# vt-asaplab/vPIN

Hardware: AMD Instinct MI355X
Metric: R1CS constraints/sec, whole Spartan SNARK (sat proof + SPARK evaluation proof; vPIN point-mult + point-add instances) (higher is better)
Workload: dtype u256 (integers mod q and mod p = 2^255-19, 32-bit limbs); 1 GPU; vPIN LeNet trace (layers L1..L7): 12 SNARKs per step; inputs=resident in HBM, parallelism=one trace per rank x 1 rank(s), no collective; 4 stream(s) per rank, table_slot_bytes=128

## Files before the change

include/vpin_hip.h:

```cpp
#ifndef VPIN_HIP_H
#define VPIN_HIP_H
#include <stddef.h>
#include <stdint.h>

#ifdef __cplusplus
extern "C" {
#endif

#define VPIN_OK 0
#define VPIN_EINVAL (-1)
#define VPIN_ENODEV (-2)
#define VPIN_ENOMEM (-3)
#define VPIN_EHIP (-4)
#define VPIN_ESHAPE (-5)
#define VPIN_EVERIFY (-6)

typedef struct vpin_ctx vpin_ctx;
typedef struct vpin_table vpin_table;

const char* vpin_strerror(int code);
const char* vpin_last_error(void);
int vpin_crash_line_set(const char* line, size_t n);
int vpin_abi_version(void);

int vpin_ctx_create(int device, vpin_ctx** out);
int vpin_ctx_create_prio(int device, int priority, vpin_ctx** out);
int vpin_ctx_create_cumask(int device, const uint32_t* cu_mask, uint32_t n_words, vpin_ctx** out);
int vpin_ctx_set_cumask_after_phase1(vpin_ctx* ctx, const uint32_t* cu_mask, uint32_t n_words);
void vpin_ctx_destroy(vpin_ctx* ctx);
void* vpin_ctx_stream(vpin_ctx* ctx);
int vpin_ctx_set_progress_flag(vpin_ctx* ctx, int* flag);
int vpin_ctx_set_shared_device(vpin_ctx* ctx, int on);
unsigned long long vpin_ctx_strip_rows_taken(vpin_ctx* ctx);
unsigned long long vpin_ctx_rlc_shared_sums(vpin_ctx* ctx);
int vpin_ctx_set_rlc_shared_cap(vpin_ctx* ctx, size_t bytes);
int vpin_ctx_set_pool_poison(vpin_ctx* ctx, uint32_t word, int on);
int vpin_ctx_pool_poison_stats(vpin_ctx* ctx, unsigned long long* blocks, unsigned long long* bytes);
unsigned long long vpin_ctx_row_table_rows(vpin_ctx* ctx);
size_t vpin_msm_row_min_scalars(vpin_ctx* ctx, int part_short);
unsigned long long vpin_ctx_pip_row_chunks(vpin_ctx* ctx);
unsigned long long vpin_ctx_witness_redo_ops(vpin_ctx* ctx);
int vpin_ctx_pool_stats(vpin_ctx* ctx, size_t out[3]);
int vpin_driver_alloc_stats(unsigned long long out[2]);
int vpin_ctx_pool_trim(vpin_ctx* ctx);
int vpin_ctx_set_low_memory(vpin_ctx* ctx, int on);
int vpin_ctx_set_expected_proofs(vpin_ctx* ctx, int n);
int vpin_ctx_device_props(vpin_ctx* ctx, int* num_cus, int* clock_khz);
int vpin_ctx_mem_info(vpin_ctx* ctx, size_t* free_bytes, size_t* total_bytes);
int vpin_ctx_sync(vpin_ctx* ctx);

int vpin_host_register(void* p, size_t bytes);
int vpin_host_unregister(void* p);

int vpin_table_upload(vpin_ctx* ctx, const uint8_t* mont32, size_t len, vpin_table** out);
int vpin_table_alloc(vpin_ctx* ctx, size_t len, vpin_table** out);
int vpin_table_wrap(vpin_ctx* ctx, void* device_ptr, size_t len, vpin_table** out);
int vpin_table_clone(vpin_ctx* ctx, const vpin_table* src, vpin_table** out);
void vpin_table_free(vpin_ctx* ctx, vpin_table* t);
size_t vpin_table_len(const vpin_table* t);
void* vpin_table_device_ptr(const vpin_table* t);
int vpin_table_read(vpin_ctx* ctx, const vpin_table* t, size_t off, size_t n, uint8_t* out);
int vpin_table_write(vpin_ctx* ctx, vpin_table* t, size_t off, size_t n, const uint8_t* src);

int vpin_sc_cubic_round(vpin_ctx* ctx, const vpin_table* tau, const vpin_table* Az,
                        const vpin_table* Bz, const vpin_table* Cz, uint8_t out_e0_e2_e3[96]);
int vpin_sc_quad_round(vpin_ctx* ctx, const vpin_table* A, const vpin_table* B,
                       uint8_t out_e0_e2[64]);
int vpin_sc_bind(vpin_ctx* ctx, vpin_table* const* tables, int k, const uint8_t r[32]);
int vpin_sc_cubic_bind_round(vpin_ctx* ctx, vpin_table* tau, vpin_table* Az, vpin_table* Bz,
                             vpin_table* Cz, const uint8_t r[32], uint8_t out_e0_e2_e3[96]);
int vpin_sc_quad_bind_round(vpin_ctx* ctx, vpin_table* A, vpin_table* B, const uint8_t r[32],
                            uint8_t out_e0_e2[64]);

int vpin_eq_table(vpin_ctx* ctx, const uint8_t* r, int ell, vpin_table** out);

int vpin_eq_suffix_tables(vpin_ctx* ctx, const uint8_t* tau, int ell, vpin_table** out);
int vpin_sc_cubic3_round(vpin_ctx* ctx, const vpin_table* pyramid, int ell, int level, vpin_table* Az,
                         vpin_table* Bz, vpin_table* Cz, uint8_t out_S0_S2_S3[96]);
int vpin_sc_cubic3_bind_round(vpin_ctx* ctx, const vpin_table* pyramid, int ell, int level, vpin_table* Az,
                              vpin_table* Bz, vpin_table* Cz, const uint8_t r[32], uint8_t out_S0_S2_S3[96]);
int vpin_sc_cubic3_lead_round(vpin_ctx* ctx, const vpin_table* pyramid, int ell, int level, vpin_table* Az,
                              vpin_table* Bz, vpin_table* Cz, const uint8_t* r, uint8_t out[96]);
int vpin_spark_batched_round(vpin_ctx* ctx, vpin_table* forest, size_t n, int ncirc, int level, size_t len,
                             const vpin_table* E, size_t e_off, const uint8_t* r, int lead, const vpin_table* derefs,
                             const vpin_table* vals, vpin_table* scratch, int first_fold, uint8_t* out);

typedef struct vpin_gens vpin_gens;
int vpin_gens_create(vpin_ctx* ctx, const uint8_t* gens_xyzt, size_t nb, vpin_gens** out);
int vpin_gens_map_stream(vpin_ctx* ctx, const uint8_t* stream64, size_t nb, uint8_t* out_xyzt);
int vpin_gens_shared(vpin_ctx* ctx, const char* label, const uint8_t* gens_xyzt, size_t nb, size_t budget_gb,
                     const vpin_gens** out);
void vpin_gens_shared_clear(void);
size_t vpin_gens_shared_bytes(int device);
void vpin_gens_free(vpin_ctx* ctx, vpin_gens* g);
size_t vpin_gens_count(const vpin_gens* g);
int vpin_gens_layout(const vpin_gens* g, size_t out[6]);
int vpin_gens_row_layout(const vpin_gens* g, size_t out[4]);
int vpin_hyrax_commit_derefs(vpin_ctx* ctx, const vpin_gens* g, const vpin_table* Z, size_t L, size_t N, const uint32_t* col_idx,
                             const uint32_t hot[3], const vpin_table* e_ry, uint8_t* out_compressed);
size_t vpin_gens_entry_bytes(void);
int vpin_hyrax_commit(vpin_ctx* ctx, const vpin_gens* g, const vpin_table* Z, const uint8_t* blinds,
                      size_t L, size_t blind_base, uint8_t* out_compressed );
int vpin_hyrax_commit_rows(vpin_ctx* ctx, const vpin_gens* g, const vpin_table* Z, size_t L, size_t row0, size_t nrows,
                           const uint8_t* blinds, size_t blind_base, uint8_t* out_compressed);
int vpin_hyrax_commit_pippenger(vpin_ctx* ctx, const vpin_gens* g, const vpin_table* Z, const uint8_t* blinds, size_t L,
                                size_t blind_base, int c_bits, uint8_t* out_compressed);
int vpin_hyrax_commit_pair(vpin_ctx* ctx, const vpin_gens* g, const vpin_table* Za, const vpin_table* Zb,
                           const uint8_t* blinds_a, const uint8_t* blinds_b, size_t L, size_t blind_base,
                           uint8_t* out_a, uint8_t* out_b, uint8_t* out_sum);
int vpin_hyrax_commit_pair_split(vpin_ctx* ctx, const vpin_gens* g, const vpin_table* Za, const vpin_table* Zb,
                                 const uint8_t* blinds_a, const uint8_t* blinds_b, size_t L, size_t blind_base,
                                 uint8_t* out_a, uint8_t* out_b, uint8_t* out_sum);
int vpin_gens_msm(vpin_ctx* ctx, const vpin_gens* g, const uint8_t* scalars_mont, size_t rows, size_t ncols,
                  uint8_t* out_compressed , uint8_t* out_xyzt );

int vpin_msm(vpin_ctx* ctx, const uint8_t* scalars_mont, const uint8_t* points_compressed, size_t n, uint8_t* out_compressed,
             uint8_t* out_xyzt);
int vpin_msm_bucket(vpin_ctx* ctx, const uint8_t* scalars_mont, const uint8_t* points_compressed, size_t n, uint8_t* out_compressed,
                    uint8_t* out_xyzt);
int vpin_points_add(vpin_ctx* ctx, const uint8_t* a_compressed, const uint8_t* b_compressed, size_t n, uint8_t* out_compressed);

// ... 511 lines not shown
```

vpin_amd/build.py:

```python
import glob
import os
import shutil
import subprocess
import sys

HERE = os.path.dirname(os.path.abspath(__file__))
CSRC = os.path.join(HERE, "csrc")
LIB_DIR = os.path.join(HERE, "lib")
LIB_PATH = os.path.join(LIB_DIR, "libvpin_hip.so")
ARCH = "gfx950"


def hipcc():
    for cand in (shutil.which("hipcc"), "/opt/rocm/bin/hipcc"):
        if cand and os.path.exists(cand):
            return cand
    raise RuntimeError("hipcc not found: the HIP library cannot be built (no CPU fallback exists)")


def sources():
    return sorted(glob.glob(os.path.join(CSRC, "*.hip")) + glob.glob(os.path.join(CSRC, "*.cpp")))


def deps():
# ... 34 lines not shown
            raise RuntimeError(f"hipcc failed on {src}")
    cmd = [hipcc(), f"--offload-arch={ARCH}", "-shared", "-fPIC", "-fopenmp", "-o", LIB_PATH] + objs
    if verbose:
        print(" ".join(cmd))
    subprocess.check_call(cmd)
    build_cli(verbose)
    build_devtest(force=True, verbose=verbose)
    build_hosttest(force=True, verbose=verbose)
    return LIB_PATH


def build_cli(verbose=False):
    src = os.path.join(CSRC, "cli", "vpin_prove.cpp")
    out_dir = os.path.join(HERE, "bin")
    os.makedirs(out_dir, exist_ok=True)
    out = os.path.join(out_dir, "vpin_prove")
    cmd = [hipcc(), "-O2", "-std=c++17", "-pthread", src, "-o", out, "-L", LIB_DIR, "-lvpin_hip", "-Wl,-rpath,$ORIGIN/../lib"]
    if verbose:
        print(" ".join(cmd))
    subprocess.check_call(cmd)
    return out


DEVTEST_SRC = os.path.join(os.path.dirname(HERE), "tests", "devarith", "devarith.hip")
DEVTEST_LIB = os.path.join(LIB_DIR, "libvpin_devtest.so")


def devtest_up_to_date():
    if not os.path.exists(DEVTEST_LIB):
        return False
    t = os.path.getmtime(DEVTEST_LIB)
    return all(os.path.getmtime(s) <= t for s in [DEVTEST_SRC] + glob.glob(os.path.join(CSRC, "*.h")))


def build_devtest(force=False, verbose=False, out=None, csrc=None):
    if out is None and csrc is None and not force and devtest_up_to_date():
        return DEVTEST_LIB
    if not os.path.exists(LIB_PATH):
        raise RuntimeError("libvpin_hip.so comes first: the harness links to it for make_fq_const")
    os.makedirs(LIB_DIR, exist_ok=True)
    out = out or DEVTEST_LIB
    cmd = [hipcc(), f"--offload-arch={ARCH}", "-O3", "-std=c++17", "-fPIC", "-shared", DEVTEST_SRC, "-o", out,
           "-I", csrc or CSRC, "-L", LIB_DIR, "-lvpin_hip", "-Wl,-rpath,$ORIGIN"]
    cmd += os.environ.get("VPIN_HIPCC_FLAGS", "").split()
    if verbose:
        print(" ".join(cmd))
    subprocess.check_call(cmd)
    return out


HOSTTEST_DIR = os.path.join(os.path.dirname(HERE), "tests", "hostarith")
HOSTTEST_SRC = os.path.join(HOSTTEST_DIR, "hostarith.cpp")
HOSTTEST_MAIN = os.path.join(HOSTTEST_DIR, "hostarith_main.cpp")
HOSTTEST_LIB = os.path.join(LIB_DIR, "libvpin_hosttest.so")
HOSTTEST_FLAGS = ["--offload-host-only", "-O3", "-std=c++17", "-fPIC", "-fopenmp"]


def hosttest_deps():
    return [HOSTTEST_SRC] + glob.glob(os.path.join(CSRC, "*.h")) + glob.glob(os.path.join(CSRC, "host", "*.h"))


def build_hosttest(force=False, verbose=False, out=None, csrc=None):
    if out is None and csrc is None and not force and os.path.exists(HOSTTEST_LIB) and all(
            os.path.getmtime(s) <= os.path.getmtime(HOSTTEST_LIB) for s in hosttest_deps()):
        return HOSTTEST_LIB
    os.makedirs(LIB_DIR, exist_ok=True)
    out = out or HOSTTEST_LIB
    cmd = [hipcc()] + HOSTTEST_FLAGS + ["-shared", HOSTTEST_SRC, "-o", out, "-I", csrc or CSRC]
    if verbose:
        print(" ".join(cmd))
    subprocess.check_call(cmd)
    return out


def build_hosttest_program(out, sanitize="address,undefined", verbose=False):
    cmd = [hipcc()] + HOSTTEST_FLAGS + ["-g", "-fno-omit-frame-pointer", "-Xarch_host", f"-fsanitize={sanitize}", "-fno-sanitize-recover=all",
                                        HOSTTEST_SRC, HOSTTEST_MAIN, "-o", out, "-I", CSRC]
    if verbose:
        print(" ".join(cmd))
    subprocess.check_call(cmd)
    return out


if __name__ == "__main__":
    print(build(force="--force" in sys.argv, verbose=True))
```

vpin_amd/capi.py:

```python
import ctypes as C
import os
import re

import numpy as np

HERE = os.path.dirname(os.path.abspath(__file__))
ROOT = os.path.dirname(HERE)
HEADER = os.path.join(ROOT, "include", "vpin_hip.h")

KERNEL_CLASSES = {
    0: "sc_cubic", 1: "sc_quad", 2: "sc_bind", 3: "sc_cubic_fused", 4: "sc_quad_fused", 5: "eq", 6: "msm", 7: "sc_tail",
    8: "spark_round", 9: "spark_build", 10: "spark_round_big", 11: "msm_rows", 12: "spark_tail",
}
K_COUNT = 16


class VpinError(RuntimeError):
    def __init__(self, code, where):
        self.code = code
        L = lib()
        msg = L.vpin_strerror(code).decode()
        last = L.vpin_last_error().decode()
        super().__init__(f"{where}: {msg} ({code})" + (f" [{last}]" if last else ""))

# ... 713 lines not shown
        cus = sorted(set(int(x) for x in cu_mask))
        words = np.zeros((cus[-1] // 32) + 1, dtype=np.uint32)
        for x in cus:
            words[x // 32] |= np.uint32(1 << (x % 32))
        return words

    def set_cumask_after_phase1(self, cu_mask):
        if cu_mask is None:
            _chk(lib().vpin_ctx_set_cumask_after_phase1(self.h, None, 0), "vpin_ctx_set_cumask_after_phase1")
            return
        words = self._mask_words(cu_mask)
        _chk(lib().vpin_ctx_set_cumask_after_phase1(self.h, words.ctypes.data_as(C.c_void_p), len(words)), "vpin_ctx_set_cumask_after_phase1")

    def close(self):
        if self.h:
            lib().vpin_ctx_destroy(self.h)
            self.h = None

    def __enter__(self):
        return self

    def __exit__(self, *a):
        self.close()

    @property
    def stream(self):
        return lib().vpin_ctx_stream(self.h)

    def sync(self):
        _chk(lib().vpin_ctx_sync(self.h), "vpin_ctx_sync")

    def device_props(self):
        cus, khz = C.c_int(), C.c_int()
        L = lib()
        L.vpin_ctx_device_props.argtypes = [C.c_void_p, C.POINTER(C.c_int), C.POINTER(C.c_int)]
        _chk(L.vpin_ctx_device_props(self.h, C.byref(cus), C.byref(khz)), "vpin_ctx_device_props")
        return cus.value, khz.value * 1e3

    def device_total_bytes(self):
        f, t = C.c_size_t(), C.c_size_t()
        L = lib()
        L.vpin_ctx_mem_info.argtypes = [C.c_void_p, C.POINTER(C.c_size_t), C.POINTER(C.c_size_t)]
        _chk(L.vpin_ctx_mem_info(self.h, C.byref(f), C.byref(t)), "vpin_ctx_mem_info")
        return t.value

    def pool_stats(self):
        L = lib()
        L.vpin_ctx_pool_stats.argtypes = [C.c_void_p, C.POINTER(C.c_size_t * 3)]
        out = (C.c_size_t * 3)()
        _chk(L.vpin_ctx_pool_stats(self.h, C.byref(out)), "vpin_ctx_pool_stats")
        return int(out[0]), int(out[1]), int(out[2])

    @staticmethod
    def crash_line_set(line_bytes):
        L = lib()
        L.vpin_crash_line_set.argtypes = [C.c_char_p, C.c_size_t]
        _chk(L.vpin_crash_line_set(line_bytes if line_bytes else None, len(line_bytes)), "vpin_crash_line_set")

    @staticmethod
    def driver_alloc_stats():
        L = lib()
        L.vpin_driver_alloc_stats.argtypes = [C.POINTER(C.c_ulonglong * 2)]
        out = (C.c_ulonglong * 2)()
        _chk(L.vpin_driver_alloc_stats(C.byref(out)), "vpin_driver_alloc_stats")
        return int(out[0]), int(out[1])

    def pool_trim(self):
        L = lib()
        L.vpin_ctx_pool_trim.argtypes = [C.c_void_p]
        _chk(L.vpin_ctx_pool_trim(self.h), "vpin_ctx_pool_trim")

    def pip_row_chunks(self):
        L = lib()
        L.vpin_ctx_pip_row_chunks.argtypes = [C.c_void_p]
        L.vpin_ctx_pip_row_chunks.restype = C.c_ulonglong
        return int(L.vpin_ctx_pip_row_chunks(self.h))

    def row_table_rows(self):
        L = lib()
        L.vpin_ctx_row_table_rows.argtypes = [C.c_void_p]
        L.vpin_ctx_row_table_rows.restype = C.c_ulonglong
        return int(L.vpin_ctx_row_table_rows(self.h))

    def msm_row_min_scalars(self, part_short=False):
        L = lib()
        L.vpin_msm_row_min_scalars.argtypes = [C.c_void_p, C.c_int]
        L.vpin_msm_row_min_scalars.restype = C.c_size_t
        return int(L.vpin_msm_row_min_scalars(self.h, 1 if part_short else 0))

    def strip_rows_taken(self):
        L = lib()
        L.vpin_ctx_strip_rows_taken.argtypes = [C.c_void_p]
        L.vpin_ctx_strip_rows_taken.restype = C.c_ulonglong
        return int(L.vpin_ctx_strip_rows_taken(self.h))

    def rlc_shared_sums(self):
        L = lib()
        L.vpin_ctx_rlc_shared_sums.argtypes = [C.c_void_p]
        L.vpin_ctx_rlc_shared_sums.restype = C.c_ulonglong
        return int(L.vpin_ctx_rlc_shared_sums(self.h))

    def set_rlc_shared_cap(self, nbytes):
        L = lib()
        L.vpin_ctx_set_rlc_shared_cap.argtypes = [C.c_void_p, C.c_size_t]
        _chk(L.vpin_ctx_set_rlc_shared_cap(self.h, nbytes), "vpin_ctx_set_rlc_shared_cap")

    def set_pool_poison(self, word, on=True):
        L = lib()
        L.vpin_ctx_set_pool_poison.argtypes = [C.c_void_p, C.c_uint32, C.c_int]
        _chk(L.vpin_ctx_set_pool_poison(self.h, word, 1 if on else 0), "vpin_ctx_set_pool_poison")

    def pool_poison_stats(self):
        L = lib()
        L.vpin_ctx_pool_poison_stats.argtypes = [C.c_void_p, C.POINTER(C.c_ulonglong), C.POINTER(C.c_ulonglong)]
        blocks, nbytes = C.c_ulonglong(0), C.c_ulonglong(0)
        _chk(L.vpin_ctx_pool_poison_stats(self.h, C.byref(blocks), C.byref(nbytes)), "vpin_ctx_pool_poison_stats")
        return int(blocks.value), int(nbytes.value)

    def witness_redo_ops(self):
        L = lib()
        L.vpin_ctx_witness_redo_ops.argtypes = [C.c_void_p]
        L.vpin_ctx_witness_redo_ops.restype = C.c_ulonglong
        return int(L.vpin_ctx_witness_redo_ops(self.h))

    def set_shared_device(self, on=True):
        _chk(lib().vpin_ctx_set_shared_device(self.h, 1 if on else 0), "vpin_ctx_set_shared_device")

    def set_low_memory(self, on=True):
        L = lib()
        L.vpin_ctx_set_low_memory.argtypes = [C.c_void_p, C.c_int]
        _chk(L.vpin_ctx_set_low_memory(self.h, 1 if on else 0), "vpin_ctx_set_low_memory")

    def set_expected_proofs(self, n):
        L = lib()
        L.vpin_ctx_set_expected_proofs.argtypes = [C.c_void_p, C.c_int]
        _chk(L.vpin_ctx_set_expected_proofs(self.h, int(n)), "vpin_ctx_set_expected_proofs")

    def gens_map_stream(self, stream):
        L = lib()
        L.vpin_gens_map_stream.argtypes = [C.c_void_p, C.c_void_p, C.c_size_t, C.c_void_p]
        buf = np.frombuffer(bytes(stream), dtype=np.uint8).copy()
        n = buf.size // 64
        out = np.zeros((n, 128), dtype=np.uint8)
        _chk(L.vpin_gens_map_stream(self.h, buf.ctypes.data_as(C.c_void_p), n, out.ctypes.data_as(C.c_void_p)), "vpin_gens_map_stream")
        return out

    def upload(self, arr):
        a = np.ascontiguousarray(arr)
        n = a.nbytes // 32
        h = C.c_void_p()
        _chk(lib().vpin_table_upload(self.h, a.ctypes.data_as(C.c_void_p), n, C.byref(h)), "vpin_table_upload")
        return Table(self, h)

    def alloc(self, n):
        h = C.c_void_p()
        _chk(lib().vpin_table_alloc(self.h, n, C.byref(h)), "vpin_table_alloc")
        return Table(self, h)

    def wrap(self, device_ptr, n):
        h = C.c_void_p()
        _chk(lib().vpin_table_wrap(self.h, C.c_void_p(device_ptr), n, C.byref(h)), "vpin_table_wrap")
        return Table(self, h)

    def eq_table(self, r):
        r = np.ascontiguousarray(r, dtype=np.uint64).reshape(-1, 4)
        h = C.c_void_p()
# ... 749 lines not shown
```

vpin_amd/csrc/capi.hip:

```cpp
#include <chrono>
#include <csignal>
#include <execinfo.h>
#include <fcntl.h>
#include <unistd.h>
#include <cstdio>
#include <cstdlib>
#include <cstring>
#include <thread>

#include "ctx.h"

namespace vpin {

static thread_local std::string g_last_error;

void set_last_error(const char* what, hipError_t e) {
  g_last_error = std::string(what) + ": " + hipGetErrorString(e);
}

void set_last_error_text(const char* text) { g_last_error = text; }

static hipEvent_t get_event(vpin_ctx* c) {
  if (!c->free_events.empty()) {
    hipEvent_t e = c->free_events.back();
    c->free_events.pop_back();
    return e;
  }
  hipEvent_t e = nullptr;
  (void)hipEventCreate(&e);
  return e;
}

static std::mutex g_ctx_mu;
static std::vector<vpin_ctx*> g_live_ctxs;
static void ctx_wait_unpinned(vpin_ctx* c) {
  while (c->pins.load(std::memory_order_acquire) != 0) std::this_thread::yield();
}

void ctx_register(vpin_ctx* c) { std::lock_guard<std::mutex> g(g_ctx_mu); g_live_ctxs.push_back(c); }
void ctx_unregister(vpin_ctx* c) {
  std::lock_guard<std::mutex> g(g_ctx_mu);
  for (size_t i = 0; i < g_live_ctxs.size(); i++)
    if (g_live_ctxs[i] == c) { g_live_ctxs.erase(g_live_ctxs.begin() + (long)i); break; }
}
int live_ctx_count() {
  std::lock_guard<std::mutex> g(g_ctx_mu);
  return (int)g_live_ctxs.size();
}
double host_cpu_quota() {
  static const double q = [] {
    double v = 0.0;
    if (FILE* f = fopen("/sys/fs/cgroup/cpu.max", "r")) {
      char a[32] = {0};
      long per = 0;
      if (fscanf(f, "%31s %ld", a, &per) == 2 && strcmp(a, "max") != 0 && per > 0) v = atof(a) / (double)per;
      fclose(f);
    } else if (FILE* f1 = fopen("/sys/fs/cgroup/cpu/cpu.cfs_quota_us", "r")) {
      long quota = -1, per = 100000;
      if (fscanf(f1, "%ld", &quota) != 1) quota = -1;
      fclose(f1);
      if (FILE* f2 = fopen("/sys/fs/cgroup/cpu/cpu.cfs_period_us", "r")) { if (fscanf(f2, "%ld", &per) != 1) per = 100000; fclose(f2); }
      if (quota > 0 && per > 0) v = (double)quota / (double)per;
    }
    const double hw = (double)std::thread::hardware_concurrency();
    return v > 0.0 && (hw <= 0.0 || v < hw) ? v : (hw > 0.0 ? hw : 1.0);
  }();
  return q;
}
bool ctx_is_live(vpin_ctx* c) {
  std::lock_guard<std::mutex> g(g_ctx_mu);
  for (auto* x : g_live_ctxs) if (x == c) return true;
  return false;
}

static size_t pool_trace_min() {
  static const size_t v = [] { const char* e = getenv("VPIN_POOL_TRACE"); return e ? ((size_t)atol(e) << 20) : (size_t)0; }();
  return v;
}
static double pool_trace_ms() {
  static const auto t0 = std::chrono::steady_clock::now();
  return std::chrono::duration<double, std::milli>(std::chrono::steady_clock::now() - t0).count();
}
static std::atomic<long long> g_in_use{0};
std::atomic<unsigned long long> g_driver_allocs{0}, g_driver_alloc_bytes{0};
void note_driver_alloc(size_t bytes) { g_driver_allocs.fetch_add(1, std::memory_order_relaxed); g_driver_alloc_bytes.fetch_add(bytes, std::memory_order_relaxed); }
static void pool_trace(const char* what, size_t cls, bool fresh, double took_ms = 0.0) {
  if (!pool_trace_min() || cls < pool_trace_min()) return;
  fprintf(stderr, "[pool %10.2f ms] %-7s %9.1f MiB%s  in use %9.1f MiB", pool_trace_ms(), what, (double)cls / 1048576.0,
          fresh ? " (hipMalloc)" : "", (double)g_in_use.load() / 1048576.0);
  if (took_ms > 0.0) fprintf(stderr, "  took %.2f ms", took_ms);
  fputc('\n', stderr);
}

static void pool_release_unlocked(vpin_ctx* c) {
  std::vector<void*> blocks;
  {
    std::lock_guard<std::mutex> g(c->pool_mu);
    for (auto& kv : c->pool_free_lists)
      for (void* p : kv.second) { c->pool_sizes.erase(p); blocks.push_back(p); }
    c->pool_free_lists.clear();
  }
  if (blocks.empty()) return;
  const double t_a = pool_trace_min() ? pool_trace_ms() : 0.0;
  if (c->stream_main) (void)hipStreamSynchronize(c->stream_main);
  if (c->stream_alt) (void)hipStreamSynchronize(c->stream_alt);
  if (!c->stream_main) (void)hipStreamSynchronize(c->stream);
  for (void* p : blocks) (void)hipFree(p);
  if (pool_trace_min())
    fprintf(stderr, "[pool %10.2f ms] release %zu cached blocks of ctx %p to the driver: %.2f ms\n", pool_trace_ms(), blocks.size(), (void*)c,
            pool_trace_ms() - t_a);
}

hipError_t driver_malloc(void** p, size_t bytes) {
  if (bytes >= ((size_t)64 << 20)) {
    size_t free_b = 0, total_b = 0;
    if (hipMemGetInfo(&free_b, &total_b) == hipSuccess && free_b < bytes + ((size_t)256 << 20)) return hipErrorOutOfMemory;
  }
  return hipMalloc(p, bytes);
}

static int pool_poison_fill(vpin_ctx* c, void** out, size_t cls) {
  const hipError_t e = hipMemsetD32Async((hipDeviceptr_t)*out, (int)c->pool_poison_word, cls / 4, c->stream);
  if (e != hipSuccess) {
    set_last_error("pool poison fill", e);
    dev_free(c, *out);
    *out = nullptr;
    return VPIN_EHIP;
  }
  c->pool_poison_blocks++;
  c->pool_poison_bytes += cls;
  return VPIN_OK;
}

int dev_alloc(vpin_ctx* c, size_t bytes, void** out) {
  size_t cls = 256;
  while (cls < bytes) cls <<= 1;
  if (cls > (size_t)1 << 22) cls = (bytes + ((size_t)1 << 20) - 1) & ~(((size_t)1 << 20) - 1);
  size_t hit = 0;
  {
    std::lock_guard<std::mutex> g(c->pool_mu);
    for (auto it = c->pool_free_lists.lower_bound(cls); it != c->pool_free_lists.end(); ++it) {
      if (it->first != cls && (cls < ((size_t)1 << 22) || it->first > 2 * cls)) break;
      if (it->second.empty()) continue;
      *out = it->second.back();
      it->second.pop_back();
      if (pool_trace_min()) { g_in_use += (long long)it->first; pool_trace("alloc", it->first, false); }
      hit = it->first;
      break;
    }
  }
  if (hit) return c->pool_poison ? pool_poison_fill(c, out, hit) : VPIN_OK;
  void* p = nullptr;
  const double t_m = pool_trace_min() ? pool_trace_ms() : 0.0;
  if (driver_malloc(&p, cls) != hipSuccess) {
    (void)hipGetLastError();
    if (pool_trace_min()) fprintf(stderr, "[pool %10.2f ms] hipMalloc of %.1f MiB FAILED: releasing cached blocks\n", pool_trace_ms(), (double)cls / 1048576.0);
    dev_pool_release(c);
    if (driver_malloc(&p, cls) != hipSuccess) {
      (void)hipGetLastError();
      std::vector<vpin_ctx*> others;
      {
        std::lock_guard<std::mutex> g(g_ctx_mu);
        for (auto* x : g_live_ctxs)
          if (x != c && x->device == c->device && x->comm_pub.load(std::memory_order_acquire) == nullptr &&
              x->tail_rounds.load(std::memory_order_acquire) == 0) {
            x->pins.fetch_add(1, std::memory_order_acq_rel);
            others.push_back(x);
          }
      }
      for (auto* x : others) {
        if (x->comm_pub.load(std::memory_order_acquire) == nullptr && x->tail_rounds.load(std::memory_order_acquire) == 0)
          pool_release_unlocked(x);
        x->pins.fetch_sub(1, std::memory_order_acq_rel);
      }
      if (driver_malloc(&p, cls) != hipSuccess) { (void)hipGetLastError(); return VPIN_ENOMEM; }
    }
  }
  note_driver_alloc(cls);
  {
    std::lock_guard<std::mutex> g(c->pool_mu);
    c->pool_sizes[p] = cls;
    *out = p;
    if (pool_trace_min()) { g_in_use += (long long)cls; pool_trace("alloc", cls, true, pool_trace_ms() - t_m); }
  }
  return c->pool_poison ? pool_poison_fill(c, out, cls) : VPIN_OK;
}

void dev_free(vpin_ctx* c, void* p) {
  if (!p) return;
  std::lock_guard<std::mutex> g(c->pool_mu);
  auto it = c->pool_sizes.find(p);
  if (it == c->pool_sizes.end()) { (void)hipFree(p); return; }
  c->pool_free_lists[it->second].push_back(p);
  if (pool_trace_min()) { g_in_use -= (long long)it->second; pool_trace("free", it->second, false); }
}

void dev_pool_release(vpin_ctx* c) { pool_release_unlocked(c); }

void dev_free_owned(vpin_ctx* owner, vpin_ctx* fallback, void* p) {
  if (!p) return;
  vpin_ctx* pool = owner ? owner : fallback;
  bool live = false;
  if (pool) {
    std::lock_guard<std::mutex> g(g_ctx_mu);
    for (auto* x : g_live_ctxs) live = live || x == pool;
    if (live) pool->pins.fetch_add(1, std::memory_order_acq_rel);
  }
  if (live) { dev_free(pool, p); pool->pins.fetch_sub(1, std::memory_order_acq_rel); }
  else if (!owner) (void)hipFree(p);
}

void dev_release_block(vpin_ctx* c, void* p) {
  if (!p) return;
  size_t sz = 0;
  {
    std::lock_guard<std::mutex> g(c->pool_mu);
    auto it = c->pool_sizes.find(p);
    if (it != c->pool_sizes.end()) { sz = it->second; c->pool_sizes.erase(it); }
  }
  const double t_a = pool_trace_min() ? pool_trace_ms() : 0.0;
  (void)hipFree(p);
  if (pool_trace_min()) { g_in_use -= (long long)sz; pool_trace("hipFree", sz, false, pool_trace_ms() - t_a); }
}

static void ctx_switch_stream(vpin_ctx* c, hipStream_t to, int cus, bool masked) {
  if (!to || c->stream == to) return;
  (void)hipEventRecord(c->stream_switch_ev, c->stream);
  (void)hipStreamWaitEvent(to, c->stream_switch_ev, 0);
  c->stream = to;
  c->num_cus = cus;
  c->cu_masked = masked;
}
void ctx_enter_alt(vpin_ctx* c) { if (c && c->stream_alt) ctx_switch_stream(c, c->stream_alt, c->cus_alt, true); }
void ctx_leave_alt(vpin_ctx* c) { if (c && c->stream_alt) ctx_switch_stream(c, c->stream_main, c->cus_main, false); }

ProfScope::ProfScope(vpin_ctx* c, int kclass, double bytes, int also, double units) : ctx(c) {
  if (!c->prof) return;
  ProfRec r;
  r.kclass = kclass;
  r.also = also;
  r.units = units;
  r.bytes = bytes;
  r.start = get_event(c);
  r.stop = get_event(c);
  (void)hipEventRecord(r.start, c->stream);
  c->recs.push_back(r);
  rec = (int)c->recs.size() - 1;
}

ProfScope::~ProfScope() {
  if (rec >= 0) (void)hipEventRecord(ctx->recs[rec].stop, ctx->stream);
}

}

using namespace vpin;

extern "C" {

const char* vpin_strerror(int code) {
  switch (code) {
    case VPIN_OK: return "ok";
    case VPIN_EINVAL: return "invalid argument";
    case VPIN_ENODEV: return "no usable HIP device (this library has no CPU fallback)";
    case VPIN_ENOMEM: return "out of memory";
    case VPIN_EHIP: return "HIP runtime error";
    case VPIN_ESHAPE: return "operand shapes do not match";
    case VPIN_EVERIFY: return "proof rejected by the verifier";
    case VPIN_ECOMM: return "a peer rank failed or timed out";
    default: return "unknown error";
  }
}

const char* vpin_last_error(void) { return g_last_error.c_str(); }

int vpin_abi_version(void) { return 11; }

static int ctx_create(int device, int priority, const uint32_t* cu_mask, uint32_t n_words, vpin_ctx** out);

int vpin_ctx_create(int device, vpin_ctx** out) { return ctx_create(device, 0, nullptr, 0, out); }
int vpin_ctx_create_prio(int device, int priority, vpin_ctx** out) { return ctx_create(device, priority, nullptr, 0, out); }
int vpin_ctx_create_cumask(int device, const uint32_t* cu_mask, uint32_t n_words, vpin_ctx** out) {
  if (!cu_mask || n_words == 0) return VPIN_EINVAL;
  return ctx_create(device, 0, cu_mask, n_words, out);
}

static int ctx_create(int device, int priority, const uint32_t* cu_mask, uint32_t n_words, vpin_ctx** out) {
  if (!out) return VPIN_EINVAL;
  setenv("KMP_BLOCKTIME", "0", 0);
  setenv("OMP_WAIT_POLICY", "PASSIVE", 0);
  setenv("KMP_AFFINITY", "disabled", 0);
  *out = nullptr;
  int n = 0;
  if (hipGetDeviceCount(&n) != hipSuccess || n <= 0) return VPIN_ENODEV;
  if (device < 0 || device >= n) return VPIN_EINVAL;
  VPIN_HIP_TRY(hipSetDevice(device));
  vpin_ctx* c = new (std::nothrow) vpin_ctx();
  if (!c) return VPIN_ENOMEM;
  c->device = device;
  hipDeviceProp_t prop;
  if (hipGetDeviceProperties(&prop, device) == hipSuccess) c->num_cus = prop.multiProcessorCount;
  int lo = 0, hi = 0;
  (void)hipDeviceGetStreamPriorityRange(&lo, &hi);
  int prio = priority < 0 ? hi : priority > 0 ? lo : 0;
  hipError_t e;
  if (cu_mask) {
    int enabled = 0;
    for (uint32_t w = 0; w < n_words; w++) {
      uint32_t bits = cu_mask[w];
      if ((w + 1) * 32 > (uint32_t)c->num_cus) bits &= (w * 32 >= (uint32_t)c->num_cus) ? 0u : ((1u << (c->num_cus - w * 32)) - 1u);
      enabled += __builtin_popcount(bits);
    }
    if (enabled == 0) { delete c; return VPIN_EINVAL; }
    e = hipExtStreamCreateWithCUMask(&c->stream, n_words, cu_mask);
    c->num_cus = enabled;
    c->cu_masked = true;
  } else {
    e = hipStreamCreateWithPriority(&c->stream, hipStreamNonBlocking, prio);
  }
  if (e != hipSuccess) { set_last_error("hipStreamCreate", e); delete c; return VPIN_EHIP; }
  c->stream_main = c->stream;
  c->cus_main = c->num_cus;
  c->partials_cap = (size_t)18 * 4096 * 3;
  if (hipMalloc(&c->d_partials, c->partials_cap * sizeof(fq)) != hipSuccess ||
      hipMalloc(&c->d_out, 8 * sizeof(fq)) != hipSuccess ||
      hipHostMalloc(&c->h_out, 8 * sizeof(fq), hipHostMallocDefault) != hipSuccess) {
    vpin_ctx_destroy(c);
    return VPIN_ENOMEM;
  }
  ctx_register(c);
  *out = c;
  return VPIN_OK;
}

void vpin_ctx_destroy(vpin_ctx* c) {
  if (!c) return;
  (void)hipSetDevice(c->device);
  if (c->stream) (void)hipStreamSynchronize(c->stream);
  ctx_leave_alt(c);
  if (c->prover_cache_free) c->prover_cache_free(c);
  if (c->spark_cache_free) c->spark_cache_free(c);
  if (c->verify_cache_free) c->verify_cache_free(c);
  if (c->h_spark) (void)hipHostFree(c->h_spark);
  if (c->d_spark_cnt) (void)hipFree(c->d_spark_cnt);
  if (c->d_add_count) (void)hipFree(c->d_add_count);
  ctx_unregister(c);
  ctx_wait_unpinned(c);
  dev_pool_release(c);
  if (!c->pool_sizes.empty()) {
    fprintf(stderr, "vpin_ctx_destroy: %zu device block(s) still referenced by live handles are released with the context; "
                    "free tables / instances / decommitments before the context\n", c->pool_sizes.size());
    for (auto& kv : c->pool_sizes) (void)hipFree(kv.first);
    c->pool_sizes.clear();
  }
  for (auto& r : c->recs) { (void)hipEventDestroy(r.start); (void)hipEventDestroy(r.stop); }
  for (auto e : c->free_events) (void)hipEventDestroy(e);
  if (c->d_partials) (void)hipFree(c->d_partials);
  if (c->d_out) (void)hipFree(c->d_out);
  if (c->h_out) (void)hipHostFree(c->h_out);
  if (c->h_bullet) (void)hipHostFree(c->h_bullet);
  if (c->stream_alt) { (void)hipStreamSynchronize(c->stream_alt); (void)hipStreamDestroy(c->stream_alt); }
  if (c->stream_switch_ev) (void)hipEventDestroy(c->stream_switch_ev);
  if (c->stream_main) (void)hipStreamDestroy(c->stream_main);
  delete c;
}

void* vpin_ctx_stream(vpin_ctx* c) { return c ? (void*)c->stream : nullptr; }

int vpin_ctx_set_cumask_after_phase1(vpin_ctx* c, const uint32_t* cu_mask, uint32_t n_words) {
  if (!c || c->cu_masked || c->stream != c->stream_main) return VPIN_EINVAL;
  (void)hipSetDevice(c->device);
  if (c->stream_alt) {
    VPIN_HIP_TRY(hipStreamSynchronize(c->stream_alt));
    (void)hipStreamDestroy(c->stream_alt);
    c->stream_alt = nullptr;
    c->cus_alt = 0;
  }
  if (!cu_mask || n_words == 0) return VPIN_OK;
  int enabled = 0;
  for (uint32_t w = 0; w < n_words; w++) {
    uint32_t bits = cu_mask[w];
    if ((w + 1) * 32 > (uint32_t)c->cus_main) bits &= (w * 32 >= (uint32_t)c->cus_main) ? 0u : ((1u << (c->cus_main - w * 32)) - 1u);
    enabled += __builtin_popcount(bits);
  }
  if (enabled == 0) return VPIN_EINVAL;
  if (!c->stream_switch_ev) VPIN_HIP_TRY(hipEventCreateWithFlags(&c->stream_switch_ev, hipEventDisableTiming));
  VPIN_HIP_TRY(hipExtStreamCreateWithCUMask(&c->stream_alt, n_words, cu_mask));
  c->cus_alt = enabled;
  return VPIN_OK;
}

int vpin_ctx_set_progress_flag(vpin_ctx* c, int* flag) {
  if (!c) return VPIN_EINVAL;
  c->progress_flag = flag;
  return VPIN_OK;
}

unsigned long long vpin_ctx_strip_rows_taken(vpin_ctx* c) { return c ? c->strip_rows_taken : 0ull; }
unsigned long long vpin_ctx_row_table_rows(vpin_ctx* c) { return c ? c->row_table_rows : 0ull; }
unsigned long long vpin_ctx_pip_row_chunks(vpin_ctx* c) { return c ? c->pip_row_chunks : 0ull; }
unsigned long long vpin_ctx_witness_redo_ops(vpin_ctx* c) { return c ? c->witness_redo_ops : 0ull; }

int vpin_ctx_set_pool_poison(vpin_ctx* c, uint32_t word, int on) {
  if (!c) return VPIN_EINVAL;
  c->pool_poison_word = word;
  c->pool_poison = on != 0;
  return VPIN_OK;
}
int vpin_ctx_pool_poison_stats(vpin_ctx* c, unsigned long long* blocks, unsigned long long* bytes) {
  if (!c) return VPIN_EINVAL;
  if (blocks) *blocks = c->pool_poison_blocks;
  if (bytes) *bytes = c->pool_poison_bytes;
  return VPIN_OK;
}

int vpin_host_register(void* p, size_t bytes) {
  if (!p || !bytes) return VPIN_EINVAL;
  VPIN_HIP_TRY(hipHostRegister(p, bytes, hipHostRegisterDefault));
  return VPIN_OK;
}
int vpin_host_unregister(void* p) {
  if (!p) return VPIN_EINVAL;
  VPIN_HIP_TRY(hipHostUnregister(p));
  return VPIN_OK;
}

int vpin_ctx_pool_trim(vpin_ctx* c) {
  if (!c) return VPIN_EINVAL;
  (void)hipSetDevice(c->device);
  dev_pool_release(c);
  return VPIN_OK;
}

int vpin_ctx_pool_stats(vpin_ctx* c, size_t out[3]) {
  if (!c || !out) return VPIN_EINVAL;
  std::lock_guard<std::mutex> g(c->pool_mu);
  size_t total = 0, cached = 0;
  for (auto& kv : c->pool_sizes) total += kv.second;
  for (auto& kv : c->pool_free_lists) cached += kv.first * kv.second.size();
  out[0] = total; out[1] = cached; out[2] = c->pool_sizes.size();
  return VPIN_OK;
}

namespace {
char g_crash_buf[8192];
volatile size_t g_crash_len = 0;
struct sigaction g_crash_old[5];
const int g_crash_sigs[5] = {SIGSEGV, SIGBUS, SIGABRT, SIGFPE, SIGTERM};
void crash_handler(int) {
  const size_t n = g_crash_len;
  size_t off = 0;
  while (off < n) {
    const ssize_t w = write(1, g_crash_buf + off, n - off);
    if (w <= 0) break;
    off += (size_t)w;
  }
  _exit(0);
}
}

namespace {
int g_segv_fd = 2;
void segv_trace_handler(int sig) {
  void* frames[64];
  const int n = backtrace(frames, 64);
  const char msg[] = "[vpin] fatal signal, call stack of the faulting thread:\n";
  (void)!write(g_segv_fd, msg, sizeof msg - 1);
  backtrace_symbols_fd(frames, n, g_segv_fd);
  signal(sig, SIG_DFL);
  raise(sig);
}
struct SegvTraceInit {
  SegvTraceInit() {
    const char* e = getenv("VPIN_SEGV_TRACE");
    if (!e) return;
    if (e[0] == '/' || e[0] == '.' || strchr(e, '/')) {
      const int fd = open(e, O_WRONLY | O_CREAT | O_APPEND, 0644);
      if (fd >= 0) g_segv_fd = fd;
    }
    struct sigaction sa;
    memset(&sa, 0, sizeof sa);
    sa.sa_handler = segv_trace_handler;
// ... 246 lines not shown
```

vpin_amd/csrc/ctx.h:

```cpp
#pragma once
#include <hip/hip_runtime.h>

#include <atomic>
#include <chrono>
#include <cstdio>
#include <cstdlib>
#include <map>
#include <mutex>
#include <string>
#include <unordered_map>
#include <vector>

#include "../../include/vpin_hip.h"
#include "fq_dev.h"

namespace vpin {

void set_last_error(const char* what, hipError_t e);

#define VPIN_HIP_TRY(expr)                         \
  do {                                             \
    hipError_t e_ = (expr);                        \
    if (e_ != hipSuccess) {                        \
      ::vpin::set_last_error(#expr, e_);           \
      return VPIN_EHIP;                            \
    }                                              \
  } while (0)

struct ProfRec {
  int kclass;
  double bytes;
  hipEvent_t start, stop;
  int also = -1;
  double units = 0.0;
};

}

struct vpin_ctx;

struct vpin_table {
  vpin::fq* d = nullptr;
  size_t len = 0;
  size_t cap = 0;
  bool owned = true;
  vpin_ctx* owner = nullptr;
};

struct vpin_gens;

struct vpin_ctx {
  int device = 0;
  hipStream_t stream = nullptr;
  int num_cus = 256;
  bool cu_masked = false;
  hipStream_t stream_main = nullptr, stream_alt = nullptr;
  hipEvent_t stream_switch_ev = nullptr;
  int cus_main = 256, cus_alt = 0;
  vpin::fq* d_partials = nullptr;
  size_t partials_cap = 0;
  vpin::fq* d_out = nullptr;
  vpin::fq* h_out = nullptr;
  bool prof = false;
  bool prof_count_adds = false;
  unsigned long long* d_add_count = nullptr;
  std::vector<vpin::ProfRec> recs;
  std::vector<hipEvent_t> free_events;
  vpin_kstat stats[VPIN_K_COUNT] = {};
  std::mutex pool_mu;
  std::atomic<int> pins{0};
  std::map<size_t, std::vector<void*>> pool_free_lists;
  std::unordered_map<void*, size_t> pool_sizes;
  void* prover_cache = nullptr;
  void (*prover_cache_free)(vpin_ctx*) = nullptr;
  void* spark_cache = nullptr;
  void (*spark_cache_free)(vpin_ctx*) = nullptr;
  void* verify_cache = nullptr;
  void (*verify_cache_free)(vpin_ctx*) = nullptr;
  vpin::fq* h_spark = nullptr;
  uint32_t* d_spark_cnt = nullptr;
  uint32_t spark_seq = 0;
  int round_split = 0, round_split_grid = 0, round_split_ncirc = 0;
  int round_group_ndotp = 0;
  uint32_t tail_seq = 0;
  std::atomic<int> tail_rounds{0};
  vpin::fq tail_sums[3 * 18];
  vpin::fq tail_final[6 * 18];
  unsigned long long pip_row_chunks = 0;
  unsigned long long row_table_rows = 0;
  unsigned long long strip_rows_taken = 0;
  unsigned long long rlc_shared_sums = 0;
  size_t rlc_shared_cap = 0;
  bool pool_poison = false;
  uint32_t pool_poison_word = 0;
  unsigned long long pool_poison_blocks = 0, pool_poison_bytes = 0;
  unsigned long long witness_redo_ops = 0;
  bool low_memory = false;
  bool shared_device = false;
  int expected_proofs = 0;
  double gens_scalars_per_proof = 0.0;
  void* h_bullet = nullptr;
  uint32_t bullet_seq = 0;
  std::atomic<vpin_comm*> comm_pub{nullptr};
  vpin_comm* comm = nullptr;
  volatile int* progress_flag = nullptr;
};

namespace vpin {

struct ProfScope {
  vpin_ctx* ctx;
  int rec = -1;
  ProfScope(vpin_ctx* c, int kclass, double bytes, int also = -1, double units = 0.0);
  ~ProfScope();
};

void ctx_enter_alt(vpin_ctx* c);
void ctx_leave_alt(vpin_ctx* c);
struct AltStreamGuard {
  vpin_ctx* c;
  explicit AltStreamGuard(vpin_ctx* ctx) : c(ctx) {}
  ~AltStreamGuard() { ctx_leave_alt(c); }
};

int dev_alloc(vpin_ctx* c, size_t bytes, void** out);
hipError_t driver_malloc(void** p, size_t bytes);
void note_driver_alloc(size_t bytes);
void dev_free(vpin_ctx* c, void* p);
int live_ctx_count();
double host_cpu_quota();
void dev_free_owned(vpin_ctx* owner, vpin_ctx* fallback, void* p);
void dev_pool_release(vpin_ctx* c);
void dev_release_block(vpin_ctx* c, void* p);

struct DevBuf {
  vpin_ctx* c;
  void* p = nullptr;
  explicit DevBuf(vpin_ctx* ctx) : c(ctx) {}
  ~DevBuf() { if (p) dev_free(c, p); }
  int alloc(size_t bytes) { return dev_alloc(c, bytes, &p); }
  void release() { if (p) { dev_free(c, p); p = nullptr; } }
};

int table_alloc_uninit(vpin_ctx* c, size_t len, vpin_table** out);

struct CommitPairState;
int commit_pair_begin(vpin_ctx* c, const vpin_gens* g, const vpin_table* Za, const vpin_table* Zb, size_t L,
                      CommitPairState** out, size_t row0 = 0, size_t nrows = (size_t)-1, size_t row_step = 1);
int commit_pair_finish(vpin_ctx* c, const vpin_gens* g, CommitPairState* st, const uint8_t* blinds_a, const uint8_t* blinds_b,
                       size_t blind_base, uint8_t* out_a, uint8_t* out_b, uint8_t* out_sum);

int sc_round_launch(vpin_ctx* c, int K, vpin_table* const* tabs, const uint8_t* r);
int sc_round_wait(vpin_ctx* c, int K, uint8_t* out);
int sc_final_claims(vpin_ctx* c, vpin_table* const* tables, int k, const uint8_t r[32], uint8_t* out);
int sc_cubic3_launch(vpin_ctx* c, vpin_table* const* t, const vpin_table* pyramid, int ell, int level, const uint8_t* r,
                     bool lead = false);

int r1cs_multiply_vec_strided(vpin_ctx* c, const vpin_r1cs_dev* d, const vpin_table* z, size_t r0, size_t step, vpin_table** Az,
                              vpin_table** Bz, vpin_table** Cz);
int table_take_strided(vpin_ctx* c, const vpin_table* src, size_t r0, size_t step, vpin_table** out);
int r1cs_eval_table_strided(vpin_ctx* c, const vpin_r1cs_dev* d, const vpin_table* evals_rx, const uint8_t r_abc[96], size_t r0,
                            size_t step, vpin_table** out);

int poly_bound_dist(vpin_ctx* c, const vpin_table* Z, const uint8_t* Lvec, size_t L_size, uint8_t* out_LZ, const fq* z_rows = nullptr);

int slices_bound(vpin_ctx* c, const uint32_t* Z32, int n32, const fq* Z, size_t N, int S, size_t Rs, const uint8_t* Ltop, size_t T,
                 const uint8_t* Rv, fq* d_LZs, uint8_t* ev_out);
int slices_combine(vpin_ctx* c, const fq* d_LZs, int S, size_t Rs, const uint8_t* coef, uint8_t* out_LZ);

inline bool is_pow2(size_t x) { return x && !(x & (x - 1)); }

int hyrax_commit_walk(vpin_ctx* c, const vpin_gens* g, const vpin_table* Z, const uint8_t* blinds, size_t L, size_t blind_base,
                      uint8_t* out_compressed);
int gens_shared_rows(vpin_ctx* c, const char* label, const uint8_t* gens_xyzt, size_t nb, size_t budget_gb, const vpin_gens** out);
int gens_msm_parts_dev(vpin_ctx* c, const vpin_gens* g, const fq* d_scalars, size_t rows, size_t ncols, uint8_t* parts_xyzt);
int hyrax_commit_derefs_hot(vpin_ctx* c, const vpin_gens* g, const vpin_table* Z, size_t L, size_t N, const uint32_t* const col_idx[3],
                            const uint32_t hot[3], const fq* e_ry, uint8_t* out_compressed, size_t row0 = 0, size_t nrows = (size_t)-1,
                            size_t row_step = 1, const fq* z_rows = nullptr);
int hyrax_commit_rows_strided(vpin_ctx* c, const vpin_gens* g, const vpin_table* Z, size_t L, size_t row0, size_t nrows, size_t row_step,
                              uint8_t* out_compressed, const fq* z_rows = nullptr);
size_t gens_msm_parts_scratch_bytes(size_t rows, size_t ncols);
int gens_msm_parts_launch(vpin_ctx* c, const vpin_gens* g, const fq* d_scalars, size_t rows, size_t ncols, void* scratch,
                          uint8_t* parts_xyzt, bool host_mapped = false);

struct ge_niels;
struct ge_ext;
int pip_rows(vpin_ctx* c, const ge_niels* d_gn, const fq* dZ, size_t rows, size_t stride, size_t ncols, const fq* d_extra, int n_extra,
             int cbits, ge_ext* d_points, unsigned long long* d_adds);
int pip_default_bits(size_t n);

struct BulletState;
int bullet_begin(vpin_ctx* c, const uint8_t* x_mont, const uint8_t* a_mont, size_t R, BulletState** out);
int bullet_round_begin(vpin_ctx* c, const vpin_gens* g, BulletState* st, size_t n, uint8_t* parts_xyzt, uint8_t cLR[64]);
int bullet_round_end(vpin_ctx* c);
uint8_t* bullet_pinned(vpin_ctx* c);
int bullet_fold(vpin_ctx* c, BulletState* st, size_t n, const uint8_t u[32], const uint8_t u_inv[32]);
int bullet_finish(vpin_ctx* c, const vpin_gens* g, BulletState* st, uint8_t xhat_ahat[64], uint8_t* parts_xyzt);
void bullet_free(vpin_ctx* c, BulletState* st);
bool bullet_fused(const BulletState* st);
int bullet_step(vpin_ctx* c, const vpin_gens* g, BulletState* st, size_t n, const uint8_t* u_prev, const uint8_t* u_inv_prev,
                uint8_t cLR[64]);
size_t bullet_part_ptrs(vpin_ctx* c, const BulletState* st, size_t n, int row, const uint8_t** out);
int bullet_finish_fused(vpin_ctx* c, const vpin_gens* g, BulletState* st, const uint8_t u[32], const uint8_t u_inv[32],
                        uint8_t xhat_ahat[64]);
int bullet_step_launch(vpin_ctx* c, const vpin_gens* g, const fq* a_prev, const fq* b_prev, fq* a_next, fq* b_next, fq* sj, size_t n,
                       size_t R, bool fold, bool finish, const uint8_t* u, const uint8_t* u_inv, uint8_t* parts_pinned,
                       uint32_t* up_pinned, uint32_t seq, void* dev_parts);

struct TraceLap {
  vpin_ctx* c;
  const char* who;
  bool on;
  std::chrono::steady_clock::time_point t;
  TraceLap(vpin_ctx* ctx, const char* w) : c(ctx), who(w), on(getenv("VPIN_CLI_TRACE") != nullptr), t(std::chrono::steady_clock::now()) {}
  void operator()(const char* what) {
    if (!on) return;
    if (c) (void)hipStreamSynchronize(c->stream);
    auto n = std::chrono::steady_clock::now();
    fprintf(stderr, "[%s] %-22s %9.1f ms\n", who, what, std::chrono::duration<double, std::milli>(n - t).count());
    t = n;
  }
};

}
```

vpin_amd/csrc/host/prover_common.h:

```cpp
#pragma once
#include <omp.h>

#include <chrono>
#include <cstdlib>
#include <cstring>
#include <map>
#include <memory>
#include <mutex>
#include <string>
#include <vector>

#include "../ctx.h"
#include "../comm.h"
#include "curve.h"
#include "transcript.h"

extern "C" {
size_t vpin_gens_msm_parts_count(size_t ncols);
int vpin_gens_msm_parts(vpin_ctx* ctx, const vpin_gens* g, const uint8_t* scalars_mont, size_t rows, size_t ncols,
                        uint8_t* parts_xyzt);
int vpin_poly_bound(vpin_ctx* c, const vpin_table* Z, const uint8_t* Lvec, size_t L_size, uint8_t* out_LZ);
int vpin_gens_map_stream(vpin_ctx* ctx, const uint8_t* stream64, size_t nb, uint8_t* out_xyzt);
void vpin_r1cs_dims(const vpin_r1cs_dev* d, size_t* num_cons, size_t* num_vars, size_t* num_inputs);
}
// ... 374 lines not shown
  };
  size_t n = R;
  static const bool fine = getenv("VPIN_SPARK_TRACE") && atoi(getenv("VPIN_SPARK_TRACE")) >= 3;
  double tb[6] = {0, 0, 0, 0, 0, 0};
  const bool fused = vpin::bullet_fused(bs);
  auto sum_side = [&](int row, size_t nn) {
    const uint8_t* ptrs[256];
    const size_t cnt = vpin::bullet_part_ptrs(c, bs, nn, row, ptrs);
    Point acc = Point::identity();
    for (size_t k = 0; k < cnt; k++) acc = acc + Point::from_xyzt(ptrs[k]);
    return acc;
  };
  Fq u_prev = Fq::zero(), u_inv_prev = Fq::zero();
  for (size_t round = 0; round < lgR; round++) {
    n /= 2;
    Fq cLR[2];
    auto t0 = Clock::now();
    if (fused) rc = vpin::bullet_step(c, pc.dev, bs, n, round ? B(&u_prev) : nullptr, round ? B(&u_inv_prev) : nullptr, B(cLR));
    else rc = vpin::bullet_round_begin(c, pc.dev, bs, n, parts.data(), B(cLR));
    if (rc) return rc;
    auto t1 = Clock::now();
    Point qh[2] = {Point::identity(), Point::identity()};
    pc.fb_gR.mul_acc(qh[0], cLR[0] * r_); pc.fb_h.mul_acc(qh[0], bv1[round]);
    pc.fb_gR.mul_acc(qh[1], cLR[1] * r_); pc.fb_h.mul_acc(qh[1], bv2[round]);
    auto t2 = Clock::now();
    if ((rc = vpin::bullet_round_end(c))) return rc;
    auto t3 = Clock::now();
    Point lr[2] = {(fused ? sum_side(0, n) : sum_parts(parts.data())) + qh[0],
                   (fused ? sum_side(1, n) : sum_parts(parts.data() + np * 128)) + qh[1]};
    auto t4 = Clock::now();
    out.Lvec[round] = compress(lr[0]);
    out.Rvec[round] = compress(lr[1]);
    tr.append_point("L", out.Lvec[round].b);
    tr.append_point("R", out.Rvec[round].b);
    Fq u = tr.challenge_scalar("u"), u_inv = u.invert();
    auto t5 = Clock::now();
    if (fused) { u_prev = u; u_inv_prev = u_inv; }
    else if ((rc = vpin::bullet_fold(c, bs, n, B(&u), B(&u_inv)))) return rc;
    blind_fin = blind_fin + bv1[round] * u * u + bv2[round] * u_inv * u_inv;
    if (fine) {
      auto t6 = Clock::now();
      tb[0] += secs(t0, t1); tb[1] += secs(t1, t2); tb[2] += secs(t2, t3); tb[3] += secs(t3, t4); tb[4] += secs(t4, t5); tb[5] += secs(t5, t6);
    }
  }
  if (fine)
    fprintf(stderr, "[dplog] R=%zu, %zu rounds, us per round: rows+inner products %.1f | host Q,H terms %.1f | wait for the MSM %.1f | "
            "sum %zu parts x2 %.1f | compress x2 + transcript + invert %.1f | fold launch %.1f\n", R, lgR, tb[0] / lgR * 1e6,
            tb[1] / lgR * 1e6, tb[2] / lgR * 1e6, np, tb[3] / lgR * 1e6, tb[4] / lgR * 1e6, tb[5] / lgR * 1e6);
  Fq xa[2];
  if (fused) rc = vpin::bullet_finish_fused(c, pc.dev, bs, B(&u_prev), B(&u_inv_prev), B(xa));
  else rc = vpin::bullet_finish(c, pc.dev, bs, B(xa), parts.data());
  if (rc) return rc;
  const Fq x_hat = xa[0], a_hat = xa[1], y_hat = x_hat * a_hat;
  Point g_hat = fused ? sum_side(0, 0) : sum_parts(parts.data());
  {
    Point p = g_hat.mul(d_);
    pc.fb_h.mul_acc(p, r_delta);
    out.delta = compress(p);
    tr.append_point("delta", out.delta.b);
    Point q = pc.fb_gR.mul(d_ * r_);
    pc.fb_h.mul_acc(q, r_beta);
    out.beta = compress(q);
    tr.append_point("beta", out.beta.b);
  }
  Fq c_ = tr.challenge_scalar("c");
  out.z1 = d_ + c_ * y_hat;
  out.z2 = a_hat * (c_ * blind_fin + r_beta) + r_delta;
  bs_guard.done = true;
  return VPIN_OK;
}

struct TableGuard {
  vpin_ctx* c;
  std::vector<vpin_table*> t;
  explicit TableGuard(vpin_ctx* c_) : c(c_) {}
  ~TableGuard() { for (auto* p : t) vpin_table_free(c, p); }
  vpin_table* add(vpin_table* p) { t.push_back(p); return p; }
};

#if defined(__clang__)
#pragma clang diagnostic pop
#endif

int sat_prove_core(vpin_ctx* c, const vpin_r1cs_dev* dinst, size_t nv, size_t ncons, size_t ni,
                   const vpin_table* d_para, const vpin_table* d_input, const vpin_table* d_vars, const uint8_t* inputs,
                   const uint8_t seed_commit64[64], const uint8_t seed_proof64[64], uint8_t* proof_out, size_t proof_cap,
                   size_t* proof_len, uint8_t* comm_para_out, uint8_t* comm_input_out, uint8_t inst_evals_out[96],
                   uint8_t* rx_out, uint8_t* ry_out, vpin_host::Transcript* tr_out, vpin_host::Transcript* tape_out);

}
```

vpin_amd/csrc/msm.hip:

```cpp
#include <algorithm>
#include <atomic>
#include <cstdlib>
#include <condition_variable>
#include <cstring>
#include <memory>
#include <mutex>
#include <string>
#include <vector>

#include "ctx.h"
#include "fp_dev.h"
#include "fp10_dev.h"
#include "ge_tree_dev.h"
#include "mailbox_dev.h"

#ifndef VPIN_NIELS_SLOT
#define VPIN_NIELS_SLOT 96
#endif
static_assert(VPIN_NIELS_SLOT == 96 || VPIN_NIELS_SLOT == 128, "table entry size");

struct vpin_gens {
  vpin::fp* table = nullptr;
  vpin::fp* table_hi = nullptr;
  int s32 = VPIN_NIELS_SLOT / 32;
// ... 1175 lines not shown
}

static int msm_rows_win(vpin_ctx* c, const vpin_gens* g, const RowArgs& ra, size_t rows, const HotRows& hr, ge_ext* d_points) {
  const RowTable rt = row_view(g);
  const int segn = row_segment(rt.W);
  c->row_table_rows += rows;
  const size_t total = ra.ncols + (size_t)ra.n_extra;
  const size_t most = std::max<size_t>(1, total / ((size_t)segn * 2));
  size_t want = rows >= 768 ? 1 : (768 + rows - 1) / rows;
  if (rows >= 768 && total > (size_t)kSeg) want = std::min<size_t>(8, (total + kSeg - 1) / kSeg);
  const char* ec = getenv("VPIN_MSM_ROW_WIN_CHUNKS");
  const int chunks = ec && atoi(ec) > 0 ? std::min(atoi(ec), 64) : (int)std::max<size_t>(1, std::min<size_t>(64, std::min(want, most)));
  DevBuf parts(c);
  if (parts.alloc(rows * (size_t)chunks * (size_t)rt.W * sizeof(ge_ext))) return VPIN_ENOMEM;
  hipLaunchKernelGGL(msm_rows_win_kernel, dim3((unsigned)rows, (unsigned)chunks), dim3(kMsmBlock), msm_lds_pad(c), c->stream, ra, view(g),
                     rt, hr, segn, (ge_ext*)parts.p);
  hipLaunchKernelGGL(msm_rows_finish_kernel, dim3((unsigned)((rows + 63) / 64)), dim3(64), 0, c->stream, (ge_ext*)parts.p, rows, chunks,
                     rt.W, rt.c, d_points);
  VPIN_HIP_TRY(hipGetLastError());
  return VPIN_OK;
}

static int row_chunks(size_t rows, size_t total, bool hot_kernel) {
  if (hot_kernel) {
    static const int env_chunks = [] { const char* e = getenv("VPIN_MSM_HOT_CHUNKS"); return e ? atoi(e) : 0; }();
    return env_chunks > 0 ? env_chunks : (int)std::max<size_t>(1, std::min<size_t>(8, total / kSeg));
  }
  if (rows < 128) {
    size_t want = (total + kMsmBlock - 1) / kMsmBlock * 4;
    return (int)(want < 1 ? 1 : want > 64 ? 64 : want);
  }
  if (rows >= 768 && total > (size_t)kSeg) {
    static const int env_chunks = [] { const char* e = getenv("VPIN_MSM_ROW_CHUNKS"); return e ? atoi(e) : 0; }();
    return env_chunks > 0 ? env_chunks : (int)std::min<size_t>(8, (total + kSeg - 1) / kSeg);
  }
  if (rows < 768 && total >= 2 * (size_t)kMsmBlock) {
    size_t want = (768 + rows - 1) / rows, most = total / kMsmBlock;
    return std::max(1, (int)(want < most ? want : most));
  }
  return 1;
}

struct StripShape { size_t groups; int strips; uint32_t rows_used; };
static StripShape strip_shape(size_t R, uint32_t eligible, size_t slots, bool cu_masked, size_t min_list) {
  const size_t G = ((size_t)eligible + kMsmBlock - 1) / kMsmBlock;
  size_t bestG = 0;
  int bestS = 0;
  for (int cand = 8; cand <= 64 && (size_t)cand * 128 <= R; cand += 8)
    if (G * (size_t)cand <= slots) { bestG = G; bestS = cand; }
  if (cu_masked)
    for (int cand = 8; cand <= 64 && (size_t)cand * 128 <= R; cand += 8) {
      const size_t g2 = std::min(G, slots / (size_t)cand);
      if (g2 * kMsmBlock >= min_list && g2 * (size_t)cand > bestG * (size_t)bestS) { bestG = g2; bestS = cand; }
    }
  if (const char* eshape = getenv("VPIN_MSM_STRIP_SHAPE")) {
    int eg = 0, esn = 0;
    if (sscanf(eshape, "%d,%d", &eg, &esn) == 2 && eg > 0 && esn > 0 && esn % 8 == 0 && (size_t)esn <= R / 8) {
      if (std::min(G, (size_t)eg) * (size_t)esn <= slots) { bestG = std::min(G, (size_t)eg); bestS = esn; }
      else if (getenv("VPIN_MSM_STRIP_TRACE")) fprintf(stderr, "[strip] VPIN_MSM_STRIP_SHAPE=%d,%d refused: %zu workgroups on %zu slots\n", eg, esn, std::min(G, (size_t)eg) * (size_t)esn, slots);
    }
  }
  return StripShape{bestG, bestS, bestG ? (uint32_t)std::min<size_t>(eligible, bestG * kMsmBlock) : 0u};
}

struct StripTake {
  DevBuf flag, list, parts, sync;
  size_t nrows = 0;
  uint32_t n = 0;
  int S = 16;
  bool uniform_shape = false;
  explicit StripTake(vpin_ctx* c) : flag(c), list(c), parts(c), sync(c) {}
  const uint32_t* d_list() const { return (const uint32_t*)list.p; }
  const uint32_t* d_count() const { return (const uint32_t*)list.p + nrows; }
};

static int strip_take(vpin_ctx* c, const vpin_gens* g, const RowArgs& ra, size_t nrows, const HotRows& hr, StripTake& st) {
  const char* es = getenv("VPIN_MSM_STRIP");
  const char* em = getenv("VPIN_MSM_STRIP_MIN");
  const size_t R = ra.ncols;
  const int env_strip = es ? atoi(es) : -1;
  const size_t min_rows = em ? (size_t)atol(em) : 8192, min_list = em ? (size_t)1 : 4096, min_R = em ? (size_t)64 : 4096;
  st.S = env_strip > 0 ? env_strip : 16;
  st.nrows = nrows;
  if (!(env_strip != 0 && (env_strip > 0 || (!c->shared_device && c->comm == nullptr)) && nrows >= min_rows && R >= min_R && R <= g->split &&
        st.S % 8 == 0 && (size_t)st.S <= R / 8))
    return VPIN_OK;
  if (st.flag.alloc(nrows) || st.list.alloc((nrows + 1) * sizeof(uint32_t))) return VPIN_ENOMEM;
  uint32_t* d_list = (uint32_t*)st.list.p;
  uint32_t* d_count = d_list + nrows;
  uint32_t n_strip = 0;
  hipLaunchKernelGGL(strip_classify_kernel, dim3((unsigned)nrows), dim3(kMsmBlock), 0, c->stream, ra, hr, (uint8_t*)st.flag.p);
  hipLaunchKernelGGL(strip_list_kernel, dim3(1), dim3(1024), 0, c->stream, (const uint8_t*)st.flag.p, nrows, d_list, d_count);
  VPIN_HIP_TRY(hipMemcpyAsync(&n_strip, d_count, sizeof n_strip, hipMemcpyDeviceToHost, c->stream));
  VPIN_HIP_TRY(hipStreamSynchronize(c->stream));
  if (n_strip < min_list) n_strip = 0;
  if (n_strip && env_strip < 0) {
    const size_t slots = (size_t)c->num_cus * (c->shared_device ? 1 : 3);
    const StripShape shape = strip_shape(R, n_strip, slots, c->cu_masked, min_list);
    if (shape.rows_used && shape.rows_used < n_strip)
      hipLaunchKernelGGL(strip_trim_kernel, dim3((n_strip - shape.rows_used + 255) / 256), dim3(256), 0, c->stream, (const uint32_t*)d_list,
                         d_count, shape.rows_used, n_strip, (uint8_t*)st.flag.p);
    if (getenv("VPIN_MSM_STRIP_TRACE")) fprintf(stderr, "[strip] %zu rows: %u eligible, %u taken as %zu groups x %d strips on %zu slots\n", nrows, n_strip, shape.rows_used, shape.groups, shape.strips, slots);
    n_strip = shape.rows_used;
    if (n_strip) {
      st.S = shape.strips;
      st.uniform_shape = true;
    }
  }
  if (n_strip && st.parts.alloc((size_t)n_strip * (size_t)st.S * sizeof(ge_ext))) return VPIN_ENOMEM;
  st.n = n_strip;
  return VPIN_OK;
}
static int strip_launch(vpin_ctx* c, const vpin_gens* g, const RowArgs& ra, const HotRows& hr, StripTake& st, unsigned pad) {
  c->strip_rows_taken += st.n;
  const unsigned groups = (unsigned)((st.n + kMsmBlock - 1) / kMsmBlock);
  const size_t per = (ra.ncols + (size_t)st.S - 1) / (size_t)st.S;
  const char* el = getenv("VPIN_MSM_STRIP_LAG");
  const int lag = el ? atoi(el) : 1;
  uint32_t* d_sync = nullptr;
  if (lag > 0 && st.uniform_shape) {
    if (st.sync.alloc((size_t)st.S * (per + 1) * sizeof(uint32_t))) return VPIN_ENOMEM;
    d_sync = (uint32_t*)st.sync.p;
    VPIN_HIP_TRY(hipMemsetAsync(d_sync, 0, (size_t)st.S * (per + 1) * sizeof(uint32_t), c->stream));
  }
  hipLaunchKernelGGL(msm_strip_kernel, dim3(groups * (unsigned)st.S), dim3(kMsmBlock), pad, c->stream, ra, view(g), hr, st.d_list(),
                     st.d_count(), st.S, (ge_ext*)st.parts.p, d_sync, lag);
  return VPIN_OK;
}

struct RowPolicy {
  bool walk_only = false;
  bool part_short = false;
  bool may_strip = false;
};

static int msm_rows_launch(vpin_ctx* c, const vpin_gens* g, const RowArgs& ra, size_t rows, const HotRows& hr, const RowPolicy& pol,
                           ge_ext* d_points) {
  const size_t total = ra.ncols + (size_t)ra.n_extra;
  const int chunks = row_chunks(rows, total, pol.may_strip);
  const bool strip_asked = pol.may_strip && (getenv("VPIN_MSM_STRIP") || getenv("VPIN_MSM_STRIP_MIN"));
  const bool use_row = !pol.walk_only && !strip_asked && row_table_use(c, g, rows, ra.ncols, ra.n_extra, ra.extra_base0, pol.part_short);
  const bool as_rows = pol.may_strip || rows >= 128;
  if (c->prof_count_adds && c->d_add_count && as_rows)
    hipLaunchKernelGGL(msm_count_adds_kernel, dim3((unsigned)rows), dim3(kMsmBlock), 0, c->stream, ra, view(g), hr, use_row ? g->c_row : 0,
                       use_row ? g->W_row : 0, c->d_add_count);
  const double bytes = 32.0 * (double)rows * (double)total;
  if (use_row) {
    ProfScope ps(c, VPIN_K_MSM, bytes, as_rows ? VPIN_K_MSM_ROWS : -1);
    return msm_rows_win(c, g, ra, rows, hr, d_points);
  }
  DevBuf parts(c);
  ge_ext* dst = d_points;
  if (chunks > 1) {
    if (parts.alloc(rows * (size_t)chunks * sizeof(ge_ext))) return VPIN_ENOMEM;
    dst = (ge_ext*)parts.p;
  }
  StripTake st(c);
  if (pol.may_strip)
    if (const int rc = strip_take(c, g, ra, rows, hr, st)) return rc;
  {
    ProfScope ps(c, VPIN_K_MSM, bytes, as_rows ? VPIN_K_MSM_ROWS : -1);
    const unsigned pad = msm_lds_pad(c);
    const dim3 grid((unsigned)rows, (unsigned)chunks);
    if (st.n)
      if (const int rc = strip_launch(c, g, ra, hr, st, pad)) return rc;
    if (pol.may_strip)
      hipLaunchKernelGGL(msm_rows_hot_kernel, grid, dim3(kMsmBlock), pad, c->stream, ra, view(g), hr, dst,
                         st.n ? (const uint8_t*)st.flag.p : (const uint8_t*)nullptr);
    else
      hipLaunchKernelGGL(msm_rows_kernel, grid, dim3(kMsmBlock), pad, c->stream, ra, view(g), dst);
    if (chunks > 1)
      hipLaunchKernelGGL(ge_sum_chunks_kernel, dim3((unsigned)((rows + 63) / 64)), dim3(64), 0, c->stream, (const ge_ext*)dst, rows, chunks,
                         d_points);
    if (st.n)
      hipLaunchKernelGGL(strip_combine_kernel, dim3((st.n + 63) / 64), dim3(64), 0, c->stream, (const ge_ext*)st.parts.p, st.d_list(),
                         st.d_count(), st.S, d_points);
  }
  VPIN_HIP_TRY(hipGetLastError());
  return VPIN_OK;
}

static int msm_rows(vpin_ctx* c, const vpin_gens* g, const fq* dZ, size_t rows, size_t stride, size_t ncols,
                    const fq* d_extra, int n_extra, size_t extra_base0, ge_ext* d_points, bool walk_only = false,
                    bool part_short = false) {
  if (const int pm = pip_mode())
    if (n_extra <= 1 && ncols + (size_t)n_extra <= 32768)
      return msm_rows_pip(c, g, dZ, rows, stride, ncols, d_extra, n_extra, extra_base0, pm < 0 ? 0 : pm, d_points);
  return msm_rows_launch(c, g, RowArgs{dZ, stride, ncols, d_extra, n_extra, extra_base0, 0, 1, 0}, rows, HotRows{},
                         RowPolicy{walk_only, part_short, false}, d_points);
}

static int compress_to_host(vpin_ctx* c, const ge_ext* d_pts, size_t n, uint8_t* out0, uint8_t* out1 = nullptr, uint8_t* out2 = nullptr) {
  uint8_t* const outs[3] = {out0, out1, out2};
  const size_t k = out2 ? 3 : out1 ? 2 : 1, per = n / k * 32;
  DevBuf dout(c);
  if (dout.alloc(n * 32)) return VPIN_ENOMEM;
  hipLaunchKernelGGL(ge_compress_kernel, dim3((unsigned)((n + 63) / 64)), dim3(64), 0, c->stream, d_pts, n, (fp*)dout.p, (fp*)nullptr);
  VPIN_HIP_TRY(hipGetLastError());
  for (size_t i = 0; i < k; i++) VPIN_HIP_TRY(hipMemcpyAsync(outs[i], (uint8_t*)dout.p + i * per, per, hipMemcpyDeviceToHost, c->stream));
  VPIN_HIP_TRY(hipStreamSynchronize(c->stream));
  return VPIN_OK;
}

static int commit_rows(vpin_ctx* c, const vpin_gens* g, const fq* z, size_t rows, size_t stride, size_t R, const uint8_t* blinds,
                       size_t blind_base, bool buckets, int c_bits, uint8_t* out_compressed, bool walk_only = false) {
  (void)hipSetDevice(c->device);
  const int n_extra = blinds ? 1 : 0;
  DevBuf dbl(c), dpts(c);
  if ((blinds && dbl.alloc(rows * 32)) || dpts.alloc(rows * sizeof(ge_ext))) return VPIN_ENOMEM;
  if (blinds) VPIN_HIP_TRY(hipMemcpyAsync(dbl.p, blinds, rows * 32, hipMemcpyHostToDevice, c->stream));
  const int rc = buckets ? msm_rows_pip(c, g, z, rows, stride, R, (const fq*)dbl.p, n_extra, blind_base, c_bits, (ge_ext*)dpts.p)
                         : msm_rows(c, g, z, rows, stride, R, (const fq*)dbl.p, n_extra, blind_base, (ge_ext*)dpts.p, walk_only);
  if (rc) return rc;
  return compress_to_host(c, (const ge_ext*)dpts.p, rows, out_compressed);
}

int vpin_hyrax_commit(vpin_ctx* c, const vpin_gens* g, const vpin_table* Z, const uint8_t* blinds, size_t L,
                      size_t blind_base, uint8_t* out_compressed) {
  if (!c || !g || !Z || !Z->d || !blinds || !out_compressed || L == 0) return VPIN_EINVAL;
  if (Z->len % L != 0) return VPIN_ESHAPE;
  const size_t R = Z->len / L;
  if (R > g->nb || blind_base >= g->nb) return VPIN_ESHAPE;
  return commit_rows(c, g, Z->d, L, R, R, blinds, blind_base, false, 0, out_compressed);
}

int vpin_hyrax_commit_pippenger(vpin_ctx* c, const vpin_gens* g, const vpin_table* Z, const uint8_t* blinds, size_t L,
                                size_t blind_base, int c_bits, uint8_t* out_compressed) {
  if (!c || !g || !Z || !Z->d || !out_compressed || L == 0) return VPIN_EINVAL;
  if (Z->len % L != 0) return VPIN_ESHAPE;
  const size_t R = Z->len / L;
  if (R > g->nb || (blinds && blind_base >= g->nb)) return VPIN_ESHAPE;
  return commit_rows(c, g, Z->d, L, R, R, blinds, blind_base, true, c_bits, out_compressed);
}

int vpin_hyrax_commit_rows(vpin_ctx* c, const vpin_gens* g, const vpin_table* Z, size_t L, size_t row0, size_t nrows,
                           const uint8_t* blinds, size_t blind_base, uint8_t* out_compressed) {
  if (!c || !g || !Z || !Z->d || !out_compressed || L == 0 || nrows == 0) return VPIN_EINVAL;
  if (Z->len % L != 0 || row0 + nrows > L) return VPIN_ESHAPE;
  const size_t R = Z->len / L;
  if (R > g->nb || (blinds && blind_base >= g->nb)) return VPIN_ESHAPE;
  return commit_rows(c, g, Z->d + row0 * R, nrows, R, R, blinds, blind_base, false, 0, out_compressed);
}

}

namespace vpin {

int hyrax_commit_derefs_hot(vpin_ctx* c, const vpin_gens* g, const vpin_table* Z, size_t L, size_t N, const uint32_t* const col_idx[3],
                            const uint32_t hot[3], const fq* e_ry, uint8_t* out_compressed, size_t row0, size_t nrows, size_t row_step,
                            const fq* z_rows) {
  if (!c || !g || !Z || (!Z->d && !z_rows) || !col_idx || !hot || !e_ry || !out_compressed || L == 0 || Z->len % L) return VPIN_EINVAL;
  const size_t R = Z->len / L;
  if (R > g->nb || N % R || Z->len < 6 * N) return VPIN_ESHAPE;
  const fq* zbase = z_rows ? z_rows : (const fq*)Z->d;
  const int z_compact = z_rows ? 1 : 0;
  if (nrows == (size_t)-1) { row0 = 0; nrows = L; row_step = 1; }
  if (row_step == 0 || (nrows && row0 + (nrows - 1) * row_step >= L)) return VPIN_ESHAPE;
  if (nrows == 0) return VPIN_OK;
  if (pip_mode()) return hyrax_commit_rows_strided(c, g, Z, L, row0, nrows, row_step, out_compressed, z_rows);
  (void)hipSetDevice(c->device);
  DevBuf dpts(c), dT(c);
  if (dpts.alloc(nrows * sizeof(ge_ext))) return VPIN_ENOMEM;
  HotRows hr{};
  hr.row0 = 3 * (N / R);
  hr.rows_per_vec = N / R;
  uint32_t distinct[3];
  int nd = 0;
  for (int m = 0; m < 3; m++) {
    hr.idx[m] = col_idx[m];
    hr.hot[m] = hot[m];
    if (hot[m] == 0xffffffffu) continue;
    bool seen = false;
    for (int k = 0; k < nd; k++) seen = seen || distinct[k] == hot[m];
    if (!seen) distinct[nd++] = hot[m];
  }
  if (nd && dT.alloc((size_t)nd * R * sizeof(ge_cached))) return VPIN_ENOMEM;
  for (int k = 0; k < nd; k++) {
    ge_cached* Tk = (ge_cached*)dT.p + (size_t)k * R;
    hipLaunchKernelGGL(scalar_times_bases_kernel, dim3((unsigned)((R + 63) / 64)), dim3(64), 0, c->stream, e_ry + distinct[k], R, view(g), Tk);
    for (int m = 0; m < 3; m++)
      if (hot[m] == distinct[k]) hr.T[m] = Tk;
  }
  if (const int rc = msm_rows_launch(c, g, RowArgs{zbase, R, R, nullptr, 0, 0, row0, row_step, z_compact}, nrows, hr,
                                     RowPolicy{false, false, true}, (ge_ext*)dpts.p))
    return rc;
  return compress_to_host(c, (const ge_ext*)dpts.p, nrows, out_compressed);
}

int hyrax_commit_walk(vpin_ctx* c, const vpin_gens* g, const vpin_table* Z, const uint8_t* blinds, size_t L, size_t blind_base,
                      uint8_t* out_compressed) {
  if (!c || !g || !Z || !Z->d || !blinds || !out_compressed || L == 0) return VPIN_EINVAL;
  if (Z->len % L != 0) return VPIN_ESHAPE;
  const size_t R = Z->len / L;
  if (R > g->nb || blind_base >= g->nb) return VPIN_ESHAPE;
  return commit_rows(c, g, Z->d, L, R, R, blinds, blind_base, false, 0, out_compressed, true);
}

int gens_shared_rows(vpin_ctx* c, const char* label, const uint8_t* gens_xyzt, size_t nb, size_t budget_gb, const vpin_gens** out) {
  return gens_shared_impl(c, label, gens_xyzt, nb, budget_gb, true, out);
}

int hyrax_commit_rows_strided(vpin_ctx* c, const vpin_gens* g, const vpin_table* Z, size_t L, size_t row0, size_t nrows, size_t row_step,
                              uint8_t* out_compressed, const fq* z_rows) {
  if (!c || !g || !Z || (!Z->d && !z_rows) || !out_compressed || L == 0 || row_step == 0) return VPIN_EINVAL;
  if (nrows == 0) return VPIN_OK;
  if (Z->len % L != 0 || row0 + (nrows - 1) * row_step >= L) return VPIN_ESHAPE;
  const size_t R = Z->len / L;
  if (R > g->nb) return VPIN_ESHAPE;
  if (z_rows) return commit_rows(c, g, z_rows, nrows, R, R, nullptr, 0, false, 0, out_compressed);
  return commit_rows(c, g, Z->d + row0 * R, nrows, row_step * R, R, nullptr, 0, false, 0, out_compressed);
}

}

extern "C" {

int vpin_hyrax_commit_derefs(vpin_ctx* c, const vpin_gens* g, const vpin_table* Z, size_t L, size_t N, const uint32_t* col_idx,
                             const uint32_t hot[3], const vpin_table* e_ry, uint8_t* out_compressed) {
  if (!c || !g || !Z || !Z->d || !col_idx || !hot || !e_ry || !e_ry->d || !out_compressed || L == 0 || N == 0) return VPIN_EINVAL;
  for (size_t i = 0; i < 3 * N; i++)
    if (col_idx[i] >= e_ry->len) return VPIN_ESHAPE;
  for (int m = 0; m < 3; m++)
    if (hot[m] != 0xffffffffu && hot[m] >= e_ry->len) return VPIN_ESHAPE;
  (void)hipSetDevice(c->device);
  DevBuf didx(c);
  if (didx.alloc(3 * N * sizeof(uint32_t))) return VPIN_ENOMEM;
  VPIN_HIP_TRY(hipMemcpyAsync(didx.p, col_idx, 3 * N * sizeof(uint32_t), hipMemcpyHostToDevice, c->stream));
  const uint32_t* const idx[3] = {(const uint32_t*)didx.p, (const uint32_t*)didx.p + N, (const uint32_t*)didx.p + 2 * N};
  return vpin::hyrax_commit_derefs_hot(c, g, Z, L, N, idx, hot, (const fq*)e_ry->d, out_compressed);
}

int vpin_hyrax_commit_pair(vpin_ctx* c, const vpin_gens* g, const vpin_table* Za, const vpin_table* Zb,
                           const uint8_t* blinds_a, const uint8_t* blinds_b, size_t L, size_t blind_base,
                           uint8_t* out_a, uint8_t* out_b, uint8_t* out_sum) {
  if (!c || !g || !Za || !Zb || !blinds_a || !blinds_b || !out_a || !out_b || !out_sum || L == 0) return VPIN_EINVAL;
  if (Za->len != Zb->len || Za->len % L != 0) return VPIN_ESHAPE;
  size_t R = Za->len / L;
  if (R > g->nb || blind_base >= g->nb) return VPIN_ESHAPE;
  (void)hipSetDevice(c->device);
  DevBuf dbl(c), dpts(c);
  if (dbl.alloc(2 * L * 32) || dpts.alloc(3 * L * sizeof(ge_ext))) return VPIN_ENOMEM;
  VPIN_HIP_TRY(hipMemcpyAsync(dbl.p, blinds_a, L * 32, hipMemcpyHostToDevice, c->stream));
  VPIN_HIP_TRY(hipMemcpyAsync((uint8_t*)dbl.p + L * 32, blinds_b, L * 32, hipMemcpyHostToDevice, c->stream));
  ge_ext* pts = (ge_ext*)dpts.p;
  int rc = msm_rows(c, g, Za->d, L, R, R, (const fq*)dbl.p, 1, blind_base, pts);
  if (rc) return rc;
  rc = msm_rows(c, g, Zb->d, L, R, R, (const fq*)dbl.p + L, 1, blind_base, pts + L);
  if (rc) return rc;
  hipLaunchKernelGGL(ge_add_rows_kernel, dim3((unsigned)((L + 63) / 64)), dim3(64), 0, c->stream, pts, pts + L, L, pts + 2 * L);
  return compress_to_host(c, pts, 3 * L, out_a, out_b, out_sum);
}

constexpr size_t kMaxParts = 128;
static inline int wide_q(size_t ncols) { return ncols >= 8192 ? 4 : 1; }
static inline size_t raw_parts(size_t ncols) { const size_t per = (size_t)kWideScalars * wide_q(ncols); return (ncols + per - 1) / per; }
size_t vpin_gens_msm_parts_count(size_t ncols) { size_t n = raw_parts(ncols); return n < kMaxParts ? n : kMaxParts; }

int vpin_gens_msm_parts(vpin_ctx* c, const vpin_gens* g, const uint8_t* scalars_mont, size_t rows, size_t ncols,
                        uint8_t* parts_xyzt) {
  if (!c || !g || !scalars_mont || !parts_xyzt || rows == 0 || ncols == 0) return VPIN_EINVAL;
  if (ncols > g->nb) return VPIN_ESHAPE;
  (void)hipSetDevice(c->device);
  DevBuf ds(c);
  if (ds.alloc(rows * ncols * 32)) return VPIN_ENOMEM;
  VPIN_HIP_TRY(hipMemcpyAsync(ds.p, scalars_mont, rows * ncols * 32, hipMemcpyHostToDevice, c->stream));
  return vpin::gens_msm_parts_dev(c, g, (const fq*)ds.p, rows, ncols, parts_xyzt);
}

}

namespace vpin {
struct CommitPairState {
  DevBuf pts;
  size_t L = 0;
  explicit CommitPairState(vpin_ctx* c) : pts(c) {}
};

int commit_pair_begin(vpin_ctx* c, const vpin_gens* g, const vpin_table* Za, const vpin_table* Zb, size_t L_all,
                      CommitPairState** out, size_t row0, size_t nrows, size_t row_step) {
  if (!c || !g || !Za || !Zb || !out || L_all == 0) return VPIN_EINVAL;
  if (Za->len != Zb->len || Za->len % L_all != 0) return VPIN_ESHAPE;
  size_t R = Za->len / L_all;
  if (R > g->nb) return VPIN_ESHAPE;
  if (nrows == (size_t)-1) { row0 = 0; nrows = L_all; row_step = 1; }
  if (nrows == 0 || row_step == 0 || row0 + (nrows - 1) * row_step >= L_all) return VPIN_ESHAPE;
  const size_t L = nrows;
  (void)hipSetDevice(c->device);
  CommitPairState* st = new (std::nothrow) CommitPairState(c);
  if (!st) return VPIN_ENOMEM;
  st->L = L;
  if (st->pts.alloc(5 * L * sizeof(ge_ext))) { delete st; return VPIN_ENOMEM; }
  ge_ext* pts = (ge_ext*)st->pts.p;
  int rc = msm_rows(c, g, Za->d + row0 * R, L, row_step * R, R, nullptr, 0, 0, pts, false, true);
// ... 135 lines not shown
```

vpin_amd/csrc/prover.cpp:

```cpp
#include "host/proof_sizes.h"
#include "host/prover_common.h"

namespace {

using namespace vpin_host;
using namespace vpin_prover;


struct SatGens {
  size_t ell = 0, L = 0, R = 0, nb = 0;
  std::vector<Point> g;
  FixedBase fb[5];
  const vpin_gens* dev = nullptr;
  PcGens pc;
  Mcg gens_1, gens_3, gens_4;
};

struct ProverCache {
  std::map<size_t, std::unique_ptr<SatGens>> by_nv;
};

static void cache_free(vpin_ctx* c) {
  auto* pc = static_cast<ProverCache*>(c->prover_cache);
  if (!pc) return;
// ... 369 lines not shown
  if (rc) return rc;
  struct Guard { vpin_ctx* c; vpin::BulletState* s; ~Guard() { (void)hipStreamSynchronize(c->stream); vpin::bullet_free(c, s); } } guard{c, bs};
  const bool fused = !classic && vpin::bullet_fused(bs);
  if (!classic && !fused) return VPIN_ESHAPE;
  const size_t lgR = log2z(R), np = vpin_gens_msm_parts_count(R);
  auto sum_side = [&](int row, size_t nn) {
    const uint8_t* ptrs[256];
    const size_t cnt = vpin::bullet_part_ptrs(c, bs, nn, row, ptrs);
    Point acc = Point::identity();
    for (size_t k = 0; k < cnt; k++) acc = acc + Point::from_xyzt(ptrs[k]);
    return acc;
  };
  std::vector<uint8_t> parts(2 * np * 128);
  const Fq* u = reinterpret_cast<const Fq*>(u_mont);
  Fq u_prev = Fq::zero(), ui_prev = Fq::zero();
  size_t n = R;
  for (size_t k = 0; k < lgR; k++) {
    n /= 2;
    if (fused) rc = vpin::bullet_step(c, g, bs, n, k ? B(&u_prev) : nullptr, k ? B(&ui_prev) : nullptr, cLR_out + 64 * k);
    else rc = vpin::bullet_round_begin(c, g, bs, n, parts.data(), cLR_out + 64 * k);
    if (rc) return rc;
    if ((rc = vpin::bullet_round_end(c))) return rc;
    for (int row = 0; row < 2; row++) {
      Point acc = Point::identity();
      if (fused) acc = sum_side(row, n);
      else
        for (size_t p = 0; p < np; p++) acc = acc + Point::from_xyzt(parts.data() + ((size_t)row * np + p) * 128);
      acc.compress(LR_out + 64 * k + 32 * row);
    }
    u_prev = u[k];
    ui_prev = u[k].invert();
    if (!fused && (rc = vpin::bullet_fold(c, bs, n, B(&u_prev), B(&ui_prev)))) return rc;
  }
  Point ghat = Point::identity();
  if (fused) {
    if ((rc = vpin::bullet_finish_fused(c, g, bs, B(&u_prev), B(&ui_prev), xhat_ahat_out))) return rc;
    ghat = sum_side(0, 0);
  } else {
    if ((rc = vpin::bullet_finish(c, g, bs, xhat_ahat_out, parts.data()))) return rc;
    for (size_t p = 0; p < np; p++) ghat = ghat + Point::from_xyzt(parts.data() + p * 128);
  }
  ghat.compress(ghat_out);
  return VPIN_OK;
}

void vpin_sat_last_timings(double out[8]) { memcpy(out, g_timings, sizeof g_timings); }

size_t vpin_sat_proof_max_bytes(size_t num_cons, size_t num_vars) { return vpin_sizes::sat_proof_max_bytes(num_cons, num_vars); }

}

namespace vpin_prover {

static int dist_fingerprint_check(vpin_ctx* c, size_t nv, size_t ncons, size_t ni, const uint8_t seed_commit64[64],
                                  const uint8_t seed_proof64[64]) {
  vpin_comm* cm = c->comm;
  auto fnv = [](const uint8_t* p, size_t n) { uint64_t h = 0xcbf29ce484222325ull; for (size_t i = 0; i < n; i++) { h ^= p[i]; h *= 0x100000001b3ull; } return h; };
  auto env_num = [](const char* name, long dflt) { const char* e = getenv(name); return e ? atol(e) : dflt; };
  uint64_t fp[9] = {
      (uint64_t)nv, (uint64_t)ncons, (uint64_t)ni, fnv(seed_commit64, 64), fnv(seed_proof64, 64),
      (uint64_t)(getenv("VPIN_DIST_NO_SAT_SPLIT") != nullptr), (uint64_t)(getenv("VPIN_DIST_BY_CIRCUIT") != nullptr),
      (uint64_t)env_num("VPIN_SPARK_TAIL_PAIRS", 1024), (uint64_t)(getenv("VPIN_BULLET_CLASSIC") != nullptr)};
  std::vector<uint64_t> all((size_t)cm->world * 9);
  int rc = vpin::comm_allgather_ctx(c, fp, all.data(), sizeof fp, "fingerprint");
  if (rc) return rc;
  static const char* what[9] = {"num_vars", "num_cons", "num_inputs", "seed_commit", "seed_proof", "VPIN_DIST_NO_SAT_SPLIT",
                                "VPIN_DIST_BY_CIRCUIT", "VPIN_SPARK_TAIL_PAIRS", "VPIN_BULLET_CLASSIC"};
  for (int r = 0; r < cm->world; r++)
    for (int k = 0; k < 9; k++)
      if (all[(size_t)r * 9 + k] != fp[k]) {
        char msg[200];
        snprintf(msg, sizeof msg, "collective proof: rank %d and rank %d differ in %s (%llu vs %llu)", cm->rank, r, what[k],
                 (unsigned long long)fp[k], (unsigned long long)all[(size_t)r * 9 + k]);
        vpin::set_last_error(msg, hipErrorUnknown);
        return VPIN_ECOMM;
      }
  return VPIN_OK;
}

int sat_prove_core(vpin_ctx* c, const vpin_r1cs_dev* dinst, size_t nv, size_t ncons, size_t ni,
                   const vpin_table* d_para, const vpin_table* d_input, const vpin_table* d_vars, const uint8_t* inputs,
                   const uint8_t seed_commit64[64], const uint8_t seed_proof64[64], uint8_t* proof_out, size_t proof_cap,
                   size_t* proof_len, uint8_t* comm_para_out, uint8_t* comm_input_out, uint8_t inst_evals_out[96],
                   uint8_t* rx_out, uint8_t* ry_out, vpin_host::Transcript* tr_out, vpin_host::Transcript* tape_out) {
  auto t_begin = Clock::now();
  memset(g_timings, 0, sizeof g_timings);
  (void)hipSetDevice(c->device);

  SatGens* sg = nullptr;
  auto t0 = Clock::now();
  int rc = get_gens(c, nv, &sg);
  if (rc) return rc;
  g_timings[5] = secs(t0, Clock::now());
  const size_t L = sg->L, R = sg->R;
  TableGuard tg(c);

  t0 = Clock::now();
  vpin_comm* cm = (c->comm && c->comm->world > 1) ? c->comm : nullptr;
  if (cm && (rc = dist_fingerprint_check(c, nv, ncons, ni, seed_commit64, seed_proof64))) return rc;
  const size_t nrows = cm ? vpin::comm_strided_count(L, cm->rank, cm->world) : L;
  vpin::CommitPairState* cps = nullptr;
  if (nrows && (rc = vpin::commit_pair_begin(c, sg->dev, d_para, d_input, L, &cps, cm ? (size_t)cm->rank : 0, nrows, cm ? (size_t)cm->world : 1)))
    return rc;
  const uint8_t two = 2;
  Transcript tape1 = make_tape(&two, 1, seed_commit64);
  std::vector<Fq> blind_para = tape1.challenge_vector("poly_blinds", L);
  std::vector<Fq> blind_input = tape1.challenge_vector("poly_blinds", L);
  std::vector<Fq> blind_vars(L);
  for (size_t i = 0; i < L; i++) blind_vars[i] = blind_para[i] + blind_input[i];
  std::vector<CG> comm_vars(L);
  if (!cm) {
    rc = vpin::commit_pair_finish(c, sg->dev, cps, B(blind_para.data()), B(blind_input.data()), R + 1, comm_para_out,
                                  comm_input_out, comm_vars[0].b);
    if (rc) return rc;
  } else {
    const size_t pmax = vpin::comm_block_max(L, cm->world);
    std::vector<uint8_t> mine(3 * pmax * 32, 0), all((size_t)cm->world * 3 * pmax * 32);
    if (nrows) {
      std::vector<Fq> bp(nrows), bi(nrows);
      for (size_t k = 0; k < nrows; k++) { bp[k] = blind_para[cm->rank + k * cm->world]; bi[k] = blind_input[cm->rank + k * cm->world]; }
      if ((rc = vpin::commit_pair_finish(c, sg->dev, cps, B(bp.data()), B(bi.data()), R + 1, mine.data(), mine.data() + pmax * 32,
                                         mine.data() + 2 * pmax * 32)))
        return rc;
    }
    if ((rc = vpin::comm_allgather_ctx(c, mine.data(), all.data(), mine.size(), "witness_commit"))) return rc;
    for (int r = 0; r < cm->world; r++) {
      const size_t n = vpin::comm_strided_count(L, r, cm->world);
      const uint8_t* blk = all.data() + (size_t)r * 3 * pmax * 32;
      for (size_t k = 0; k < n; k++) {
        const size_t row = (size_t)r + k * (size_t)cm->world;
        memcpy(comm_para_out + row * 32, blk + k * 32, 32);
        memcpy(comm_input_out + row * 32, blk + pmax * 32 + k * 32, 32);
        memcpy(comm_vars[row].b, blk + 2 * pmax * 32 + k * 32, 32);
      }
    }
  }
  g_timings[0] = secs(t0, Clock::now());

  Transcript tr("snark_example");
  Transcript tape = make_tape(reinterpret_cast<const uint8_t*>("proof"), 5, seed_proof64);
  tr.append_protocol_name("Spartan SNARK proof");
  tr.append_protocol_name("R1CS proof");
  tr.append_message("poly_commitment", "poly_commitment_begin");
  for (size_t i = 0; i < L; i++) tr.append_point("poly_commitment_share", comm_vars[i].b);
  tr.append_message("poly_commitment", "poly_commitment_end");

  t0 = Clock::now();
  const size_t zl = 2 * nv;
  vpin_table* d_z = nullptr;
  if ((rc = vpin_r1cs_build_z(c, dinst, d_vars, inputs, &d_z))) return rc;
  tg.add(d_z);
  const int nrx = (int)log2z(ncons), nry = (int)log2z(zl);
  std::vector<Fq> tau = tr.challenge_vector("challenge_tau", nrx);
  int lw = 0;
  if (cm && (cm->world & (cm->world - 1)) == 0) {
    const int l = (int)log2z((size_t)cm->world);
    static const bool off = getenv("VPIN_DIST_NO_SAT_SPLIT") != nullptr;
    if (!off && nrx - l >= 12 && nry - l >= 12) lw = l;
  }
  const size_t wstep = (size_t)1 << lw, wrank = lw ? (size_t)cm->rank : 0;
  vpin_table* d_pyr = nullptr;
  if ((rc = vpin_eq_suffix_tables(c, B(tau.data()), nrx - lw, &d_pyr))) return rc;
  tg.add(d_pyr);
  const Fq one = Fq::one();
  vpin_table* d_abc[3] = {nullptr, nullptr, nullptr};
  auto t_spmv = Clock::now();
  if (lw) rc = vpin::r1cs_multiply_vec_strided(c, dinst, d_z, wrank, wstep, &d_abc[0], &d_abc[1], &d_abc[2]);
  else rc = vpin_r1cs_multiply_vec(c, dinst, d_z, &d_abc[0], &d_abc[1], &d_abc[2]);
  if (rc) return rc;
  for (int m = 0; m < 3; m++) tg.add(d_abc[m]);
  g_timings[6] += secs(t_spmv, Clock::now());
  ZkSc sc1, sc2;
  std::vector<Fq> rx, ry;
  Fq claims1[4], blind_post1;
  vpin_table* tabs1[3] = {d_abc[0], d_abc[1], d_abc[2]};
  rc = zk_sumcheck(c, 4, tabs1, Fq::zero(), Fq::zero(), nrx, sg->gens_1, sg->gens_4, tr, tape, sc1, rx, claims1, blind_post1,
                   &tau, d_pyr, lw);
  if (rc) return rc;
  if ((rc = vpin::comm_mark(c, "sat_phase1_rest"))) return rc;
  vpin::ctx_enter_alt(c);
  if (c->progress_flag) *c->progress_flag = 1;
  g_timings[1] = secs(t0, Clock::now());

  const Fq tau_claim = claims1[0], Az_claim = claims1[1], Bz_claim = claims1[2], Cz_claim = claims1[3];
  Fq Az_blind = tape.challenge_scalar("Az_blind"), Bz_blind = tape.challenge_scalar("Bz_blind"),
     Cz_blind = tape.challenge_scalar("Cz_blind"), prod_blind = tape.challenge_scalar("prod_Az_Bz_blind");
  KnowProof pok_Cz;
  CG comm_Cz = knowledge_prove(pok_Cz, sg->gens_1, tr, tape, Cz_claim, Cz_blind);
  ProdProof pprod;
  CG comm_Az, comm_Bz, comm_prod;
  product_prove(pprod, sg->gens_1, tr, tape, Az_claim, Az_blind, Bz_claim, Bz_blind, Az_claim * Bz_claim, prod_blind, comm_Az,
                comm_Bz, comm_prod);
  tr.append_point("comm_Az_claim", comm_Az.b);
  tr.append_point("comm_Bz_claim", comm_Bz.b);
  tr.append_point("comm_Cz_claim", comm_Cz.b);
  tr.append_point("comm_prod_Az_Bz_claims", comm_prod.b);
  Fq blind_expected1 = tau_claim * (prod_blind - Cz_blind);
  Fq claim_post1 = (Az_claim * Bz_claim - Cz_claim) * tau_claim;
  EqProof eq1;
  equality_prove(eq1, sg->gens_1, tr, tape, claim_post1, blind_expected1, claim_post1, blind_post1);

  t0 = Clock::now();
  Fq r_A = tr.challenge_scalar("challenege_Az"), r_B = tr.challenge_scalar("challenege_Bz"),
     r_C = tr.challenge_scalar("challenege_Cz");
  Fq claim2 = r_A * Az_claim + r_B * Bz_claim + r_C * Cz_claim;
  Fq blind_claim2 = r_A * Az_blind + r_B * Bz_blind + r_C * Cz_blind;
  vpin_table *d_eq_rx = nullptr, *d_eabc = nullptr;
  if ((rc = vpin_eq_table(c, B(rx.data()), nrx, &d_eq_rx))) return rc;
  tg.add(d_eq_rx);
  t_spmv = Clock::now();
  {
    Fq rabc[3] = {r_A, r_B, r_C};
    if (lw) rc = vpin::r1cs_eval_table_strided(c, dinst, d_eq_rx, B(rabc), wrank, wstep, &d_eabc);
    else rc = vpin_r1cs_eval_table(c, dinst, d_eq_rx, B(rabc), &d_eabc);
    if (rc) return rc;
    tg.add(d_eabc);
  }
  g_timings[6] += secs(t_spmv, Clock::now());
  Fq claims2[2], blind_post2;
  vpin_table* d_z2 = d_z;
  if (lw) {
    if ((rc = vpin::table_take_strided(c, d_z, wrank, wstep, &d_z2))) return rc;
    tg.add(d_z2);
  }
  vpin_table* tabs2[2] = {d_z2, d_eabc};
  rc = zk_sumcheck(c, 2, tabs2, claim2, blind_claim2, nry, sg->gens_1, sg->gens_3, tr, tape, sc2, ry, claims2, blind_post2, nullptr,
                   nullptr, lw);
  if (rc) return rc;
  if ((rc = vpin::comm_mark(c, "sat_phase2_rest"))) return rc;
  g_timings[2] = secs(t0, Clock::now());

  t0 = Clock::now();
  const size_t left = sg->ell / 2, right = sg->ell - left;
  std::vector<Fq> Lv(L), Rv(R), LZ(R);
  host_eq(ry.data() + 1, left, Lv.data());
  host_eq(ry.data() + 1 + left, right, Rv.data());
  if (cm) rc = vpin::poly_bound_dist(c, d_vars, B(Lv.data()), L, B(LZ.data()));
  else rc = vpin_poly_bound(c, d_vars, B(Lv.data()), L, B(LZ.data()));
  if (rc) return rc;
  Fq eval_vars_at_ry = Fq::zero();
  for (size_t i = 0; i < R; i++) eval_vars_at_ry = eval_vars_at_ry + LZ[i] * Rv[i];
  Fq blind_eval = tape.challenge_scalar("blind_eval");
  tr.append_protocol_name("polynomial evaluation proof");
  Fq LZ_blind = Fq::zero();
  for (size_t i = 0; i < L; i++) LZ_blind = LZ_blind + blind_vars[i] * Lv[i];

  DpLog pe;
  if ((rc = dplog_prove(c, sg->pc, tr, tape, LZ, LZ_blind, Rv, eval_vars_at_ry, blind_eval, pe))) return rc;
  g_timings[3] = secs(t0, Clock::now());

  Fq blind_eval_Z = (one - ry[0]) * blind_eval;
  Fq blind_expected2 = claims2[1] * blind_eval_Z;
  Fq claim_post2 = claims2[0] * claims2[1];
  EqProof eq2;
  equality_prove(eq2, sg->gens_1, tr, tape, claim_post2, blind_expected2, claim_post2, blind_post2);

  t0 = Clock::now();
  Fq ie[3];
  {
    vpin_table* d_eq_ry = nullptr;
    if ((rc = vpin_eq_table(c, B(ry.data()), nry, &d_eq_ry))) return rc;
    tg.add(d_eq_ry);
    if ((rc = vpin_r1cs_evaluate(c, dinst, d_eq_rx, d_eq_ry, B(ie)))) return rc;
  }
  tr.append_scalar("Ar_claim", ie[0]);
  tr.append_scalar("Br_claim", ie[1]);
  tr.append_scalar("Cr_claim", ie[2]);
  memcpy(inst_evals_out, ie, 96);
  g_timings[7] = secs(t0, Clock::now());

  Writer w;
  w.u64(L);
  for (auto& cg : comm_vars) w.point(cg);
  write_zksc(w, sc1);
  w.point(comm_Az); w.point(comm_Bz); w.point(comm_Cz); w.point(comm_prod);
  w.point(pok_Cz.alpha); w.scalar(pok_Cz.z1); w.scalar(pok_Cz.z2);
  w.point(pprod.alpha); w.point(pprod.beta); w.point(pprod.delta);
  for (int i = 0; i < 5; i++) w.scalar(pprod.z[i]);
  w.point(eq1.alpha); w.scalar(eq1.z);
  write_zksc(w, sc2);
  w.point(pe.Cy);
  write_dplog(w, pe);
  w.point(eq2.alpha); w.scalar(eq2.z);
  if (w.buf.size() > proof_cap) return VPIN_ESHAPE;
  memcpy(proof_out, w.buf.data(), w.buf.size());
  *proof_len = w.buf.size();
  if (rx_out) memcpy(rx_out, rx.data(), rx.size() * 32);
  if (ry_out) memcpy(ry_out, ry.data(), ry.size() * 32);
  if ((rc = vpin::comm_mark(c, "sat_replicated"))) return rc;
  if (tr_out) *tr_out = tr;
  if (tape_out) *tape_out = tape;
  g_timings[4] = secs(t_begin, Clock::now());
  static const bool trace_on = getenv("VPIN_SPARK_TRACE") && atoi(getenv("VPIN_SPARK_TRACE")) >= 2;
  if (trace_on)
    fprintf(stderr, "[sat] 2^%d: polycommit %.3f  phase 1 %.3f  phase 2 %.3f  polyeval %.3f  inst.evaluate %.3f  (sparse products %.3f)  total %.3f ms\n",
            nrx, 1e3 * g_timings[0], 1e3 * g_timings[1], 1e3 * g_timings[2], 1e3 * g_timings[3], 1e3 * g_timings[7],
            1e3 * g_timings[6], 1e3 * g_timings[4]);
  return VPIN_OK;
}

}

extern "C" {

int vpin_sat_prepare(vpin_ctx* c, size_t num_vars) {
  if (!c || !vpin::is_pow2(num_vars)) return VPIN_EINVAL;
  SatGens* sg = nullptr;
  return get_gens(c, num_vars, &sg);
}

int vpin_sat_prove_resident(vpin_ctx* c, const vpin_r1cs_dev* dinst, const vpin_table* vars_para, const vpin_table* vars_input,
                            const vpin_table* vars, const uint8_t* inputs, const uint8_t seed_commit64[64],
// ... 63 lines not shown
```

vpin_amd/csrc/spark.cpp:

```cpp
#include <cstdio>

#include "host/proof_sizes.h"
#include "host/prover_common.h"
#include "gadget_dev.h"
#include "spark_dev.h"

namespace {

using namespace vpin_host;
using namespace vpin_prover;

static bool spark_trace() { static const bool on = getenv("VPIN_SPARK_TRACE") != nullptr; return on; }
struct TraceSpan {
  const char* name; Clock::time_point t0;
  explicit TraceSpan(const char* n) : name(n), t0(Clock::now()) {}
  ~TraceSpan() { if (spark_trace()) fprintf(stderr, "[spark] %-28s %8.3f ms\n", name, secs(t0, Clock::now()) * 1e3); }
};


struct SparkGens {
  std::vector<Point> g;
  std::map<size_t, std::unique_ptr<PcGens>> views;
};

static void spark_cache_free(vpin_ctx* c) {
  auto* sg = static_cast<SparkGens*>(c->spark_cache);
  if (!sg) return;
  delete sg;
  c->spark_cache = nullptr;
}

static size_t spark_budget_gb(vpin_ctx* c) {
  if (c->expected_proofs > 0) return (size_t)24;
  static const size_t gb = [c] {
    const char* e = getenv("VPIN_SPARK_GENS_BUDGET_GB");
    if (e && atoi(e) > 0) return (size_t)atoi(e);
    size_t free_b = 0, total_b = 0;
    (void)hipSetDevice(c->device);
    if (hipMemGetInfo(&free_b, &total_b) != hipSuccess) return (size_t)24;
    return free_b >= ((size_t)200 << 30) ? (size_t)80 : (size_t)24;
  }();
  return gb;
}

static int get_view(vpin_ctx* c, size_t ell, const PcGens** out) {
  if (!c->spark_cache) { c->spark_cache = new SparkGens(); c->spark_cache_free = spark_cache_free; }
  auto* sg = static_cast<SparkGens*>(c->spark_cache);
  auto it = sg->views.find(ell);
  if (it == sg->views.end()) {
    const size_t left = ell / 2, R = (size_t)1 << (ell - left), nb = R + 2;
    vpin::TraceLap lap(nullptr, "spark get_view");
    if (sg->g.size() < nb) derive_gens(sg->g, nb, "gens_r1cs_eval", c);
    lap("derive_gens (host)");
    std::unique_ptr<PcGens> v(new PcGens());
    v->ell = ell; v->L = (size_t)1 << left; v->R = R;
    int rc = vpin::gens_shared_rows(c, "gens_r1cs_eval", nullptr, nb, 0, &v->dev);
    if (rc == VPIN_EINVAL) {
      std::vector<uint8_t> xyzt(128 * nb);
#pragma omp parallel for schedule(static) num_threads(host_threads())
      for (long i = 0; i < (long)nb; i++) sg->g[i].to_xyzt(xyzt.data() + 128 * (size_t)i);
      c->gens_scalars_per_proof = (double)((size_t)1 << ell) * 0.375;
      rc = vpin::gens_shared_rows(c, "gens_r1cs_eval", xyzt.data(), nb, spark_budget_gb(c), &v->dev);
    }
    if (rc) return rc;
    lap("device table");
#pragma omp parallel for schedule(static, 1) num_threads(2)
    for (int k = 0; k < 2; k++) {
      if (k == 0) v->fb_gR = FixedBase(sg->g[R]);
      else v->fb_h = FixedBase(sg->g[R + 1]);
    }
    lap("fixed bases (host)");
    v->bind_views();
    it = sg->views.emplace(ell, std::move(v)).first;
  }
  *out = it->second.get();
  return VPIN_OK;
}

using Shape = vpin_sizes::SparkShape;

static Shape shape_of(size_t num_cons, size_t num_vars, const size_t nnz[3]) { return vpin_sizes::spark_shape(num_cons, num_vars, nnz); }

static int commit_noblind(vpin_ctx* c, const PcGens* pc, const vpin_table* Z, std::vector<CG>& out, bool short_scalars = false) {
  std::vector<uint8_t> zeros(pc->L * 32, 0);
  out.resize(pc->L);
  if (short_scalars) return vpin::hyrax_commit_walk(c, pc->dev, Z, zeros.data(), pc->L, pc->R + 1, out[0].b);
  return vpin_hyrax_commit(c, pc->dev, Z, zeros.data(), pc->L, pc->R + 1, out[0].b);
}

static void append_polycomm(Transcript& tr, const char* label, const std::vector<CG>& C) {
  tr.append_message(label, "poly_commitment_begin");
  for (auto& p : C) tr.append_point("poly_commitment_share", p.b);
  tr.append_message(label, "poly_commitment_end");
}

static void w_scalars(Writer& w, const Fq* v, size_t n) { w.u64(n); for (size_t i = 0; i < n; i++) w.scalar(v[i]); }

static int polyeval_prove_plain(vpin_ctx* c, const PcGens& pc, const vpin_table* Z, const std::vector<Fq>& r, const Fq& Zr,
                                Transcript& tr, Transcript& tape, DpLog& out, const vpin::fq* z_rows = nullptr,
                                const std::vector<Fq>* lz_pre = nullptr, const std::vector<Fq>* rv_pre = nullptr) {
  if (r.size() != pc.ell || (!(lz_pre && rv_pre) && (!Z || Z->len != ((size_t)1 << pc.ell)))) return VPIN_ESHAPE;
  tr.append_protocol_name("polynomial evaluation proof");
  const size_t left = pc.ell / 2, right = pc.ell - left;
  if (lz_pre && rv_pre) {
    if (lz_pre->size() != pc.R || rv_pre->size() != pc.R) return VPIN_ESHAPE;
    TraceSpan ts("  dplog");
    return dplog_prove(c, pc, tr, tape, *lz_pre, Fq::zero(), *rv_pre, Zr, Fq::zero(), out);
  }
  std::vector<Fq> Lv(pc.L), Rv(pc.R), LZ(pc.R);
  host_eq(r.data(), left, Lv.data());
  host_eq(r.data() + left, right, Rv.data());
  int rc;
  {
    TraceSpan ts("  poly_bound");
    if (c->comm && c->comm->world > 1) rc = vpin::poly_bound_dist(c, Z, B(Lv.data()), pc.L, B(LZ.data()), z_rows);
    else rc = vpin_poly_bound(c, Z, B(Lv.data()), pc.L, B(LZ.data()));
  }
  if (rc) return rc;
  if ((rc = vpin::comm_mark(c, "hash_poly_bound"))) return rc;
  TraceSpan ts("  dplog");
  return dplog_prove(c, pc, tr, tape, LZ, Fq::zero(), Rv, Zr, Fq::zero(), out);
}

struct SlicePass {
  vpin::DevBuf lzs;
  std::vector<Fq> Rv;
  int used = 0, nbits = 0;
  bool on = false;
  explicit SlicePass(vpin_ctx* c) : lzs(c) {}
  static bool fits(const PcGens& pc, int nbits, const std::vector<Fq>& rand) {
    const bool off = getenv("VPIN_HASH_TWO_PASS") != nullptr;
    return !off && pc.ell / 2 >= (size_t)nbits && rand.size() + (size_t)nbits == pc.ell;
  }
  int run(vpin_ctx* c, const PcGens& pc, const uint32_t* table32, int n32, const vpin::fq* table, int nbits_, int used_,
          const std::vector<Fq>& rand, Fq* ev) {
    nbits = nbits_; used = used_;
    const size_t left = pc.ell / 2, T = pc.L >> nbits, N = (size_t)1 << rand.size();
    std::vector<Fq> Ltop(T);
    host_eq(rand.data(), left - (size_t)nbits, Ltop.data());
    Rv.resize(pc.R);
    host_eq(rand.data() + (left - (size_t)nbits), pc.ell - left, Rv.data());
    if (lzs.alloc((size_t)used * pc.R * 32)) return VPIN_ENOMEM;
    int rc = vpin::slices_bound(c, table32, n32, table, N, used, pc.R, B(Ltop.data()), T, B(Rv.data()), (vpin::fq*)lzs.p, B(ev));
    on = rc == VPIN_OK;
    return rc;
  }
  int combine(vpin_ctx* c, const PcGens& pc, const std::vector<Fq>& ch, std::vector<Fq>& LZ) {
    std::vector<Fq> coef((size_t)1 << nbits);
    host_eq(ch.data(), (size_t)nbits, coef.data());
    LZ.resize(pc.R);
    return vpin::slices_combine(c, (const vpin::fq*)lzs.p, used, pc.R, B(coef.data()), B(LZ.data()));
  }
};

struct DistPlan {
  vpin_comm* cm = nullptr;
  int rank = 0, world = 1;
  int owner_ops[12], owner_dotp[6], owner_mem[4];
  std::vector<std::vector<int>> ops_of, dotp_of, mem_of;
  int max_ops_inst = 0, max_mem_inst = 0;
  int lw = 0;
};

static void make_plan(int world, int owner_ops[12], int owner_dotp[6], int owner_mem[4]) {
  std::vector<long> load(world, 0);
  auto least = [&](const std::vector<long>& key2) {
    int best = 0;
    for (int r = 1; r < world; r++)
      if (load[r] < load[best] || (load[r] == load[best] && key2[r] < key2[best])) best = r;
    return best;
  };
// ... 397 lines not shown
        const Fq* res = reinterpret_cast<const Fq*>(c->h_spark);
        for (int t = 0; t < npc; t++) {
          cl[t] = res[4 * t] + rl * (res[4 * t + 1] - res[4 * t]);
          cr[t] = res[4 * t + 2] + rl * (res[4 * t + 3] - res[4 * t + 2]);
        }
        if (with_dotp) {
          const Fq* q = reinterpret_cast<const Fq*>(c->h_spark) + 64;
          for (int i = 0; i < 6; i++)
            for (int t = 0; t < 3; t++) dp[3 * i + t] = q[6 * i + 2 * t] + rl * (q[6 * i + 2 * t + 1] - q[6 * i + 2 * t]);
        }
      }
    }

    for (int t = 0; t < npc; t++) {
      tr.append_scalar("claim_prod_left", cl[t]);
      tr.append_scalar("claim_prod_right", cr[t]);
    }
    if (with_dotp) {
      for (int t = 0; t < 3; t++) out.dotp[t].resize(6);
      for (int i = 0; i < 6; i++) {
        for (int t = 0; t < 3; t++) out.dotp[t][i] = dp[3 * i + t];
        tr.append_scalar("claim_dotp_left", out.dotp[0][i]);
        tr.append_scalar("claim_dotp_right", out.dotp[1][i]);
        tr.append_scalar("claim_dotp_weight", out.dotp[2][i]);
      }
    }
    Fq r_layer = tr.challenge_scalar("challenge_r_layer");
    for (int t = 0; t < npc; t++) claims[t] = cl[t] + r_layer * (cr[t] - cl[t]);
    out.claims_left[o] = cl;
    out.claims_right[o] = cr;
    std::vector<Fq> ext;
    ext.reserve(k + 1);
    ext.push_back(r_layer);
    ext.insert(ext.end(), r.begin(), r.end());
    rand.swap(ext);
    if (fine) { auto t = Clock::now(); t_epi += secs(tl0, t); tl0 = t; }
  }
  if (fine)
    fprintf(stderr, "[spark]   forest of %d x 2^%d: setup %.3f  first result %.3f  later results %.3f  host per-round math %.3f  epilogue %.3f ms\n",
            npc, num_layers, t_setup * 1e3, t_first * 1e3, t_rounds * 1e3, t_host * 1e3, t_epi * 1e3);
  return VPIN_OK;
}

static thread_local double g_spark_timings[8];

static int dist_pick(vpin_ctx* c, const DistPlan& pl, const Fq* mine, size_t cnt, const int* owner, Fq* out, const char* tag) {
  std::vector<Fq> all(cnt * (size_t)pl.world);
  int rc = vpin::comm_allgather_ctx(c, mine, all.data(), cnt * 32, tag);
  if (rc) return rc;
  for (size_t i = 0; i < cnt; i++) out[i] = all[cnt * (size_t)owner[i] + i];
  return VPIN_OK;
}

struct SparkProof {
  vpin_ctx* c;
  const vpin_spark_decomm* d;
  const std::vector<Fq>&rx, &ry;
  const Fq* evals;
  Transcript &tr, &tape;
  const size_t N, M, lgN, lgM;
  const PcGens *g_ops = nullptr, *g_mem = nullptr, *g_derefs = nullptr;
  TableGuard tg;
  DistPlan plan;
  const DistPlan* dz = nullptr;
  bool st = false;
  vpin::SparkLeaves leaves;
  size_t Nf = 0, Mf = 0;
  bool defer_mem = false;
  vpin_table *mem_rx = nullptr, *mem_ry = nullptr, *comb = nullptr;
  vpin_table comb_shape;
  vpin::DevBuf b_cloc, b_crows, b_vloc, b_ops, b_mem, b_scr;
  vpin::fq* comb_rows = nullptr;
  const vpin::fq *derefs = nullptr, *vals = nullptr;
  std::vector<CG> comm_derefs;
  vpin::HashParams hash;
  vpin::SparkForest f_ops, f_mem;
  Fq pl[2][8];
  DotpCtx dotp;
  Fq dotp_left[3], dotp_right[3];
  Batched pf_ops, pf_mem;
  std::vector<Fq> rand_ops, rand_mem;
  Fq ev_derefs[6], ev_ops[15], ev_mem[2];
  DpLog pe_derefs, pe_ops, pe_mem;

  SparkProof(vpin_ctx* c_, const vpin_spark_decomm* d_, const std::vector<Fq>& rx_, const std::vector<Fq>& ry_, const Fq* evals_,
             Transcript& tr_, Transcript& tape_)
      : c(c_), d(d_), rx(rx_), ry(ry_), evals(evals_), tr(tr_), tape(tape_), N(d_->N), M(d_->M), lgN(log2z(d_->N)), lgM(log2z(d_->M)),
        tg(c_), b_cloc(c_), b_crows(c_), b_vloc(c_), b_ops(c_), b_mem(c_), b_scr(c_) {}
  bool by_circuit() const { return dz && !st; }
};

static int split_plan(SparkProof& S) {
  vpin_ctx* c = S.c;
  if (!(c->comm && c->comm->world > 1)) return VPIN_OK;
  if (c->comm->world > 12) return VPIN_EINVAL;
  plan_init(S.plan, c->comm);
  S.dz = &S.plan;
  static const bool by_circuit = getenv("VPIN_DIST_BY_CIRCUIT") != nullptr;
  const size_t Wz = (size_t)S.plan.world;
  if (!by_circuit && (Wz & (Wz - 1)) == 0 && Wz <= 16 && S.N / Wz >= 4096 && S.M / Wz >= 4096 && S.g_derefs->L >= Wz)
    S.plan.lw = (int)log2z(Wz);
  S.st = S.plan.lw > 0;
  if (S.st) { S.leaves.r0 = (size_t)S.plan.rank; S.leaves.step = Wz; }
  return VPIN_OK;
}

static int stage_derefs(SparkProof& S) {
  vpin_ctx* c = S.c;
  const vpin_spark_decomm* d = S.d;
  const DistPlan* dz = S.dz;
  const PcGens* g_derefs = S.g_derefs;
  const size_t N = S.N;
  int rc;
  S.tr.append_protocol_name("Sparse polynomial evaluation proof");
  const size_t nm = std::max(d->nx, d->ny);
  std::vector<Fq> rx_ext(nm, Fq::zero()), ry_ext(nm, Fq::zero());
  std::copy(S.rx.begin(), S.rx.end(), rx_ext.begin() + (nm - d->nx));
  std::copy(S.ry.begin(), S.ry.end(), ry_ext.begin() + (nm - d->ny));
  if ((rc = vpin_eq_table(c, B(rx_ext.data()), (int)nm, &S.mem_rx))) return rc;
  S.tg.add(S.mem_rx);
  if ((rc = vpin_eq_table(c, B(ry_ext.data()), (int)nm, &S.mem_ry))) return rc;
  S.tg.add(S.mem_ry);
  const vpin::fq *mem_rx = S.mem_rx->d, *mem_ry = S.mem_ry->d;
  S.Nf = N / S.leaves.step; S.Mf = S.M / S.leaves.step;
  if (S.st) {
    S.comb_shape.d = nullptr; S.comb_shape.len = S.comb_shape.cap = 8 * N; S.comb_shape.owned = false;
    S.comb = &S.comb_shape;
    const size_t Nl = S.Nf, nrows_loc = vpin::comm_strided_count(g_derefs->L, dz->rank, dz->world);
    if (S.b_cloc.alloc(6 * Nl * 32) || S.b_crows.alloc(std::max<size_t>(1, nrows_loc) * g_derefs->R * 32) || S.b_vloc.alloc(3 * Nl * 32)) return VPIN_ENOMEM;
    S.comb_rows = (vpin::fq*)S.b_crows.p;
    if ((rc = vpin::spark_gather_derefs(c, d, S.leaves, mem_rx, mem_ry, (vpin::fq*)S.b_cloc.p, S.comb_rows, g_derefs->R, nrows_loc))) return rc;
    for (int m = 0; m < 3; m++)
      if ((rc = vpin::spark_take_strided(c, d->vals + (size_t)m * N, Nl, S.leaves.r0, S.leaves.step, (vpin::fq*)S.b_vloc.p + (size_t)m * Nl))) return rc;
    S.derefs = (const vpin::fq*)S.b_cloc.p; S.vals = (const vpin::fq*)S.b_vloc.p;
  } else {
    if ((rc = vpin::table_alloc_uninit(c, 8 * N, &S.comb))) return rc;
    S.tg.add(S.comb);
    if ((rc = vpin::spark_gather_derefs(c, d, S.leaves, mem_rx, mem_ry, S.comb->d))) return rc;
    S.derefs = S.comb->d; S.vals = d->vals;
  }
  if ((rc = vpin::comm_mark(c, "derefs_gather"))) return rc;
  std::vector<CG>& comm_derefs = S.comm_derefs;
  const bool hot = d->hot_col[0] != 0xffffffffu || d->hot_col[1] != 0xffffffffu || d->hot_col[2] != 0xffffffffu;
  const uint32_t* col_idx[3] = {d->idx + 6 * N, d->idx + 7 * N, d->idx + 8 * N};
  if (dz) {
    const size_t L = g_derefs->L, pmax = vpin::comm_block_max(L, dz->world);
    const size_t nrows = vpin::comm_strided_count(L, dz->rank, dz->world);
    std::vector<uint8_t> mine(pmax * 32, 0), all(pmax * 32 * (size_t)dz->world);
    if (nrows) {
      if (hot)
        rc = vpin::hyrax_commit_derefs_hot(c, g_derefs->dev, S.comb, L, N, col_idx, d->hot_col, mem_ry, mine.data(), (size_t)dz->rank,
                                           nrows, (size_t)dz->world, S.comb_rows);
      else
        rc = vpin::hyrax_commit_rows_strided(c, g_derefs->dev, S.comb, L, (size_t)dz->rank, nrows, (size_t)dz->world, mine.data(), S.comb_rows);
      if (rc) return rc;
    }
    if ((rc = vpin::comm_allgather_ctx(c, mine.data(), all.data(), mine.size(), "derefs_commit"))) return rc;
    comm_derefs.resize(L);
    for (int r = 0; r < dz->world; r++) {
      const size_t n = vpin::comm_strided_count(L, r, dz->world);
      for (size_t k = 0; k < n; k++) memcpy(comm_derefs[(size_t)r + k * (size_t)dz->world].b, all.data() + ((size_t)r * pmax + k) * 32, 32);
    }
  } else if (hot) {
    comm_derefs.resize(g_derefs->L);
    if ((rc = vpin::hyrax_commit_derefs_hot(c, g_derefs->dev, S.comb, g_derefs->L, N, col_idx, d->hot_col, mem_ry, comm_derefs[0].b))) return rc;
  } else if ((rc = commit_noblind(c, g_derefs, S.comb, comm_derefs))) {
    return rc;
  }
  S.tr.append_message("derefs_commitment", "begin_derefs_commitment");
  append_polycomm(S.tr, "comm_poly_row_col_ops_val", comm_derefs);
  S.tr.append_message("derefs_commitment", "end_derefs_commitment");
  return VPIN_OK;
}

static vpin::HashParams make_hash(const Fq& r_hash, const Fq& gamma) {
  const Fq r2 = r_hash * r_hash, r2_boost = r2 * Fq::r2();
  vpin::HashParams hp;
  memcpy(hp.r.v, B(&r_hash), 32); memcpy(hp.r2.v, B(&r2), 32); memcpy(hp.r2_boost.v, B(&r2_boost), 32); memcpy(hp.gamma.v, B(&gamma), 32);
  return hp;
}

static int stage_network(SparkProof& S) {
  vpin_ctx* c = S.c;
  const DistPlan* dz = S.dz;
  int rc;
  std::vector<Fq> r_mem_check = S.tr.challenge_vector("challenge_r_hash", 2);
  S.hash = make_hash(r_mem_check[0], r_mem_check[1]);
  vpin::SparkLeaves lv_ops = S.leaves, lv_mem = S.leaves;
  int nl_ops = 12, nl_mem = 4;
  size_t nl_dotp = 6;
  if (S.by_circuit()) {
    const auto &ops = dz->ops_of[dz->rank], &mem = dz->mem_of[dz->rank];
    lv_ops.ncirc = nl_ops = (int)ops.size(); lv_mem.ncirc = nl_mem = (int)mem.size();
    std::copy(ops.begin(), ops.end(), lv_ops.ids);
    std::copy(mem.begin(), mem.end(), lv_mem.ids);
    nl_dotp = dz->dotp_of[dz->rank].size();
  }
// ... 202 lines not shown
  const size_t N = S.N, M = S.M;
  const std::vector<Fq>&rand_ops = S.rand_ops, &rand_mem = S.rand_mem;
  int rc;
  S.tr.append_protocol_name("Sparse polynomial hash layer proof");
  vpin_table *eq_ops = nullptr, *eq_mem = nullptr;
  const bool one_pass = !dz && SlicePass::fits(*S.g_derefs, 3, rand_ops) && SlicePass::fits(*S.g_ops, 4, rand_ops) &&
                        SlicePass::fits(*S.g_mem, 1, rand_mem);
  SlicePass sp_derefs(c), sp_ops(c), sp_mem(c);
  vpin_table *comb_ops = nullptr, *comb_mem = nullptr;
  if (!one_pass && dz) {
    auto* dm = const_cast<vpin_spark_decomm*>(d);
    dm->comb_unpooled = true;
    if ((rc = vpin::spark_comb_tables(c, dm))) return rc;
    comb_ops = dm->comb_ops; comb_mem = dm->comb_mem;
  } else if (!one_pass) {
    if ((rc = vpin::spark_comb_make(c, d, &comb_ops, &comb_mem))) return rc;
    S.tg.add(comb_ops); S.tg.add(comb_mem);
  }
  if (!one_pass) {
    TraceSpan ts("hash: eq tables");
    const int lwz = S.st ? dz->lw : 0;
    if ((rc = vpin_eq_table(c, B(rand_ops.data()), (int)S.lgN - lwz, &eq_ops))) return rc;
    S.tg.add(eq_ops);
    if ((rc = vpin_eq_table(c, B(rand_mem.data()), (int)S.lgM - lwz, &eq_mem))) return rc;
    S.tg.add(eq_mem);
  }
  if ((rc = vpin::comm_mark(c, "hash_eq_tables"))) return rc;
  const Fq* hs = reinterpret_cast<const Fq*>(c->h_spark);
  if (dz) {
    if ((rc = hash_slice_evals_dist(S, comb_ops, comb_mem, eq_ops, eq_mem))) return rc;
  } else if (one_pass) {
    TraceSpan ts("hash: derefs slices (one pass)");
    if ((rc = sp_derefs.run(c, *S.g_derefs, nullptr, 0, S.derefs, 3, 6, rand_ops, S.ev_derefs))) return rc;
  } else {
    TraceSpan ts("hash: derefs slice evals");
    if ((rc = vpin::spark_slice_evals(c, S.derefs, N, 6, eq_ops->d))) return rc;
    for (int i = 0; i < 6; i++) S.ev_derefs[i] = hs[3 * i];
  }
  S.tr.append_protocol_name("Derefs evaluation proof");
  std::vector<Fq> e8(8, Fq::zero());
  std::copy(S.ev_derefs, S.ev_derefs + 6, e8.begin());
  if ((rc = prove_joint(S, *S.g_derefs, S.comb, sp_derefs, e8, 3, rand_ops,
                        {"evals_ops_val", "challenge_combine_n_to_one", "joint_claim_eval", "hash: polyeval derefs"}, S.comb_rows, S.pe_derefs)))
    return rc;
  if (one_pass) {
    TraceSpan ts("hash: ops+mem slices (one pass)");
    if ((rc = sp_ops.run(c, *S.g_ops, d->idx, 12, d->vals, 4, 15, rand_ops, S.ev_ops))) return rc;
    if ((rc = sp_mem.run(c, *S.g_mem, d->idx + 12 * N, 2, nullptr, 1, 2, rand_mem, S.ev_mem))) return rc;
  } else if (!dz) {
    TraceSpan ts("hash: ops+mem slice evals");
    if ((rc = vpin::spark_slice_evals(c, comb_ops->d, N, 15, eq_ops->d))) return rc;
    for (int i = 0; i < 15; i++) S.ev_ops[i] = hs[3 * i];
    if ((rc = vpin::spark_slice_evals(c, comb_mem->d, M, 2, eq_mem->d))) return rc;
    for (int i = 0; i < 2; i++) S.ev_mem[i] = hs[3 * i];
  }
  std::vector<Fq> e16(16, Fq::zero());
  std::copy(S.ev_ops, S.ev_ops + 15, e16.begin());
  if ((rc = prove_joint(S, *S.g_ops, comb_ops, sp_ops, e16, 4, rand_ops,
                        {"claim_evals_ops", "challenge_combine_n_to_one", "joint_claim_eval_ops", "hash: polyeval ops"}, nullptr, S.pe_ops)))
    return rc;
  return prove_joint(S, *S.g_mem, comb_mem, sp_mem, {S.ev_mem[0], S.ev_mem[1]}, 1, rand_mem,
                     {"claim_evals_mem", "challenge_combine_two_to_one", "joint_claim_eval_mem", "hash: polyeval mem"}, nullptr, S.pe_mem);
}

static void write_proof(const SparkProof& S, Writer& w) {
  const auto& pl = S.pl;
  w.u64(S.comm_derefs.size());
  for (auto& p : S.comm_derefs) w.point(p);
  for (int s = 0; s < 2; s++) { w.scalar(pl[s][0]); w_scalars(w, &pl[s][1], 3); w_scalars(w, &pl[s][4], 3); w.scalar(pl[s][7]); }
  w_scalars(w, S.dotp_left, 3);
  w_scalars(w, S.dotp_right, 3);
  write_batched(w, S.pf_mem);
  write_batched(w, S.pf_ops);
  w_scalars(w, &S.ev_ops[0], 3); w_scalars(w, &S.ev_ops[3], 3); w.scalar(S.ev_mem[0]);
  w_scalars(w, &S.ev_ops[6], 3); w_scalars(w, &S.ev_ops[9], 3); w.scalar(S.ev_mem[1]);
  w_scalars(w, &S.ev_ops[12], 3);
  w_scalars(w, &S.ev_derefs[0], 3); w_scalars(w, &S.ev_derefs[3], 3);
  write_dplog(w, S.pe_ops);
  write_dplog(w, S.pe_mem);
  write_dplog(w, S.pe_derefs);
}

static int spark_prove(vpin_ctx* c, const vpin_spark_decomm* d, const std::vector<Fq>& rx, const std::vector<Fq>& ry,
                       const Fq evals[3], Transcript& tr, Transcript& tape, Writer& w) {
  if (d->N < 4 || d->M < 4 || rx.size() != d->nx || ry.size() != d->ny) return VPIN_ESHAPE;
  int rc;
  SparkProof S(c, d, rx, ry, evals, tr, tape);
  const Shape sh{d->nx, d->ny, S.N, S.M, S.lgN + 4, std::max(d->nx, d->ny) + 1, S.lgN + 3};
  if ((rc = get_view(c, std::max(sh.v_ops, sh.v_mem), &S.g_ops)) || (rc = get_view(c, sh.v_ops, &S.g_ops)) ||
      (rc = get_view(c, sh.v_mem, &S.g_mem)) || (rc = get_view(c, sh.v_derefs, &S.g_derefs)))
    return rc;
  auto t0 = Clock::now();
  auto lap = [&](int slot) { g_spark_timings[slot] = secs(t0, Clock::now()); t0 = Clock::now(); };
  if ((rc = split_plan(S)) || (rc = stage_derefs(S))) return rc;
  lap(1);
  if (c->progress_flag) *c->progress_flag = 2;
  if ((rc = stage_network(S))) return rc;
  lap(2);
  if ((rc = stage_product(S))) return rc;
  lap(3);
  if ((rc = stage_hash(S))) return rc;
  lap(4);
  write_proof(S, w);
  return VPIN_OK;
}

}

extern "C" {

size_t vpin_spark_comm_bytes(const vpin_r1cs* inst) {
  return inst ? vpin_sizes::spark_comm_bytes(inst->num_cons, inst->num_vars, inst->nnz) : 0;
}

size_t vpin_snark_proof_max_bytes(const vpin_r1cs* inst) {
  return inst ? vpin_sizes::snark_proof_max_bytes(inst->num_cons, inst->num_vars, inst->nnz) : 0;
}

int vpin_spark_prepare(vpin_ctx* c, size_t num_cons, size_t num_vars, size_t max_nnz) {
  if (!c || !vpin::is_pow2(num_cons) || !vpin::is_pow2(num_vars) || max_nnz == 0) return VPIN_EINVAL;
  (void)hipSetDevice(c->device);
  const size_t nnz[3] = {max_nnz, max_nnz, max_nnz};
  const Shape s = shape_of(num_cons, num_vars, nnz);
  const PcGens* g = nullptr;
  int rc = get_view(c, std::max(s.v_ops, s.v_mem), &g);
  if (!rc) {
    auto* sg = static_cast<SparkGens*>(c->spark_cache);
    std::vector<size_t> idx;
    for (size_t ell : {s.v_ops, s.v_mem, s.v_derefs}) {
      const size_t R = (size_t)1 << (ell - ell / 2);
      if (R + 1 < sg->g.size()) { idx.push_back(R); idx.push_back(R + 1); }
    }
#pragma omp parallel for schedule(dynamic, 1) num_threads(host_threads())
    for (long k = 0; k < (long)idx.size(); k++) { FixedBase warm(sg->g[idx[(size_t)k]]); (void)warm; }
  }
  if (!rc) rc = get_view(c, s.v_ops, &g);
  if (!rc) rc = get_view(c, s.v_mem, &g);
  if (!rc) rc = get_view(c, s.v_derefs, &g);
  return rc;
}

int vpin_spark_gens_view(vpin_ctx* c, size_t ell, const vpin_gens** out, size_t* L, size_t* R) {
  if (!c || !out || !L || !R || ell < 2 || ell > 40) return VPIN_EINVAL;
  (void)hipSetDevice(c->device);
  const PcGens* g = nullptr;
  int rc = get_view(c, ell, &g);
  if (rc) return rc;
  *out = g->dev; *L = g->L; *R = g->R;
  return VPIN_OK;
}

int vpin_dist_plan(int world, int owner_ops[12], int owner_dotp[6], int owner_mem[4]) {
  if (world < 1 || world > 12 || !owner_ops || !owner_dotp || !owner_mem) return VPIN_EINVAL;
  make_plan(world, owner_ops, owner_dotp, owner_mem);
  return VPIN_OK;
}

void vpin_spark_decomm_hot_cols(const vpin_spark_decomm* d, uint32_t out[3]) {
  for (int m = 0; m < 3; m++) out[m] = d ? d->hot_col[m] : 0xffffffffu;
}

void vpin_spark_decomm_free(vpin_ctx* c, vpin_spark_decomm* d) {
  if (!d) return;
  if (c) {
    (void)hipSetDevice(c->device);
    if (d->idx) vpin::dev_free(c, d->idx);
    if (d->vals) vpin::dev_free(c, d->vals);
    if (d->comb_ops) vpin_table_free(c, d->comb_ops);
    if (d->comb_mem) vpin_table_free(c, d->comb_mem);
  }
  delete d;
}

static int encode_commit(vpin_ctx* c, const Shape& s, std::unique_ptr<vpin_spark_decomm>& d, vpin::TraceLap& lap, size_t num_cons,
// ... 111 lines not shown
  if (!g || !g->r1cs) return 0;
  vpin_r1cs r{};
  r.num_cons = g->r1cs->num_cons; r.num_vars = g->r1cs->num_vars; r.num_inputs = g->num_inputs;
  for (int m = 0; m < 3; m++) r.nnz[m] = g->nnz[m];
  return vpin_spark_comm_bytes(&r);
}

size_t vpin_dev_instance_proof_max_bytes(const vpin_dev_instance* g) {
  if (!g || !g->r1cs) return 0;
  vpin_r1cs r{};
  r.num_cons = g->r1cs->num_cons; r.num_vars = g->r1cs->num_vars; r.num_inputs = g->num_inputs;
  for (int m = 0; m < 3; m++) r.nnz[m] = g->nnz[m];
  return vpin_snark_proof_max_bytes(&r);
}

int vpin_poly_slices_bound(vpin_ctx* c, const vpin_table* Z, int nbits, int used, const uint8_t* r, size_t r_len, const uint8_t* ch,
                           uint8_t* evals_out, uint8_t* LZ_out) {
  if (!c || !Z || !Z->d || nbits < 0 || nbits > 4 || used < 1 || used > (1 << nbits) || !r || !evals_out) return VPIN_EINVAL;
  const size_t ell = r_len + (size_t)nbits;
  if (Z->len != ((size_t)1 << ell) || ell / 2 < (size_t)nbits) return VPIN_ESHAPE;
  PcGens pc;
  pc.ell = ell; pc.L = (size_t)1 << (ell / 2); pc.R = (size_t)1 << (ell - ell / 2);
  std::vector<Fq> rand(r_len);
  memcpy(rand.data(), r, r_len * 32);
  SlicePass sp(c);
  std::vector<Fq> ev((size_t)used);
  int rc = sp.run(c, pc, nullptr, 0, Z->d, nbits, used, rand, ev.data());
  if (rc) return rc;
  memcpy(evals_out, ev.data(), (size_t)used * 32);
  if (ch && LZ_out) {
    std::vector<Fq> chv((size_t)nbits), LZ;
    memcpy(chv.data(), ch, (size_t)nbits * 32);
    if ((rc = sp.combine(c, pc, chv, LZ))) return rc;
    memcpy(LZ_out, LZ.data(), pc.R * 32);
  }
  return VPIN_OK;
}

int vpin_poly_slices_bound_u32(vpin_ctx* c, const uint32_t* slices_u32, int n32, const vpin_table* Zfq, int nbits, int used,
                               const uint8_t* r, size_t r_len, const uint8_t* ch, uint8_t* evals_out, uint8_t* LZ_out) {
  if (!c || !slices_u32 || n32 < 1 || nbits < 0 || nbits > 4 || used < n32 || used > (1 << nbits) || !r || !evals_out) return VPIN_EINVAL;
  const size_t ell = r_len + (size_t)nbits, N = (size_t)1 << r_len;
  if (ell / 2 < (size_t)nbits || (used > n32 && (!Zfq || !Zfq->d || Zfq->len < (size_t)(used - n32) * N))) return VPIN_ESHAPE;
  PcGens pc;
  pc.ell = ell; pc.L = (size_t)1 << (ell / 2); pc.R = (size_t)1 << (ell - ell / 2);
  (void)hipSetDevice(c->device);
  vpin::DevBuf b32(c);
  if (b32.alloc((size_t)n32 * N * 4)) return VPIN_ENOMEM;
  if (hipMemcpyAsync(b32.p, slices_u32, (size_t)n32 * N * 4, hipMemcpyHostToDevice, c->stream) != hipSuccess) return VPIN_EHIP;
  std::vector<Fq> rand(r_len);
  memcpy(rand.data(), r, r_len * 32);
  SlicePass sp(c);
  std::vector<Fq> ev((size_t)used);
  int rc = sp.run(c, pc, (const uint32_t*)b32.p, n32, used > n32 ? Zfq->d : nullptr, nbits, used, rand, ev.data());
  if (rc) return rc;
  memcpy(evals_out, ev.data(), (size_t)used * 32);
  if (ch && LZ_out) {
    std::vector<Fq> chv((size_t)nbits), LZ;
    memcpy(chv.data(), ch, (size_t)nbits * 32);
    if ((rc = sp.combine(c, pc, chv, LZ))) return rc;
    memcpy(LZ_out, LZ.data(), pc.R * 32);
  }
  return VPIN_OK;
}

int vpin_snark_prove_resident(vpin_ctx* c, const vpin_r1cs_dev* dinst, const vpin_spark_decomm* decomm,
                              const vpin_table* vars_para, const vpin_table* vars_input, const vpin_table* vars,
                              const uint8_t* inputs, const uint8_t seed_commit64[64], const uint8_t seed_proof64[64],
                              uint8_t* proof_out, size_t proof_cap, size_t* proof_len, uint8_t* comm_para_out,
                              uint8_t* comm_input_out) {
  if (!c || !dinst || !decomm || !vars_para || !vars_input || !vars || !seed_commit64 || !seed_proof64 || !proof_out ||
      !proof_len || !comm_para_out || !comm_input_out)
    return VPIN_EINVAL;
  size_t nv, ncons, ni;
  vpin_r1cs_dims(dinst, &ncons, &nv, &ni);
  if (vars_para->len != nv || vars_input->len != nv || vars->len != nv || (ni && !inputs)) return VPIN_ESHAPE;
  if (decomm->num_cons != ncons || decomm->num_vars != nv || decomm->num_inputs != ni) return VPIN_ESHAPE;
  auto t0 = Clock::now();
  vpin::AltStreamGuard alt_guard(c);
  Transcript tr("snark_example"), tape("snark_example");
  uint8_t ie[96];
  std::vector<Fq> rx(log2z(ncons)), ry(log2z(2 * nv));
  size_t sat_len = 0;
  int rc = sat_prove_core(c, dinst, nv, ncons, ni, vars_para, vars_input, vars, inputs, seed_commit64, seed_proof64, proof_out,
                          proof_cap, &sat_len, comm_para_out, comm_input_out, ie, B(rx.data()), B(ry.data()), &tr, &tape);
  if (rc) return vpin::comm_leave(c->comm, rc);
  if (c->progress_flag) *c->progress_flag = 1;
  g_spark_timings[5] = secs(t0, Clock::now());
  Writer w;
  w.bytes(ie, 96);
  Fq evals[3];
  memcpy(evals, ie, 96);
  if ((rc = spark_prove(c, decomm, rx, ry, evals, tr, tape, w))) return vpin::comm_leave(c->comm, rc);
  if (sat_len + w.buf.size() > proof_cap) return VPIN_ESHAPE;
  memcpy(proof_out + sat_len, w.buf.data(), w.buf.size());
  *proof_len = sat_len + w.buf.size();
  g_spark_timings[6] = secs(t0, Clock::now());
  return VPIN_OK;
}

int vpin_snark_prove(vpin_ctx* c, const vpin_r1cs* inst, const uint8_t* vars_para, const uint8_t* vars_input,
                     const uint8_t* vars, const uint8_t* inputs, const uint8_t seed_commit64[64], const uint8_t seed_proof64[64],
                     uint8_t* proof_out, size_t proof_cap, size_t* proof_len, uint8_t* comm_out, size_t comm_cap, size_t* comm_len,
                     uint8_t* comm_para_out, uint8_t* comm_input_out) {
  if (!c || !inst || !vars_para || !vars_input || !vars) return VPIN_EINVAL;
  const size_t nv = inst->num_vars;
  if (!vpin::is_pow2(nv) || !vpin::is_pow2(inst->num_cons) || inst->num_inputs >= nv) return VPIN_ESHAPE;
  vpin_r1cs_dev* dinst = nullptr;
  vpin_spark_decomm* decomm = nullptr;
  const bool trace = getenv("VPIN_CLI_TRACE") != nullptr;
  auto t0 = std::chrono::steady_clock::now();
  auto lap = [&](const char* what) {
    if (!trace) return;
    (void)hipStreamSynchronize(c->stream);
    auto t1 = std::chrono::steady_clock::now();
    fprintf(stderr, "[vpin_snark_prove] %-18s %9.1f ms\n", what, std::chrono::duration<double, std::milli>(t1 - t0).count());
    t0 = t1;
  };
  int rc = vpin_r1cs_upload(c, inst, &dinst);
  if (rc) return rc;
  lap("r1cs_upload");
  TableGuard tg(c);
  vpin_table *d_para = nullptr, *d_input = nullptr, *d_vars = nullptr;
  rc = vpin_spark_encode(c, inst, &decomm, comm_out, comm_cap, comm_len);
  lap("spark_encode");
  if (!rc) rc = vpin_table_upload(c, vars_para, nv, &d_para);
  if (!rc) { tg.add(d_para); rc = vpin_table_upload(c, vars_input, nv, &d_input); }
  if (!rc) { tg.add(d_input); rc = vpin_table_upload(c, vars, nv, &d_vars); }
  lap("witness_upload");
  if (!rc) {
    tg.add(d_vars);
    rc = vpin_snark_prove_resident(c, dinst, decomm, d_para, d_input, d_vars, inputs, seed_commit64, seed_proof64, proof_out,
                                   proof_cap, proof_len, comm_para_out, comm_input_out);
  }
  lap("prove_resident");
  vpin_spark_decomm_free(c, decomm);
  vpin_r1cs_free(c, dinst);
  return rc;
}

int vpin_snark_prove_dev(vpin_ctx* c, const vpin_dev_instance* g, const uint8_t seed_commit64[64], const uint8_t seed_proof64[64],
                         uint8_t* proof_out, size_t proof_cap, size_t* proof_len, uint8_t* comm_out, size_t comm_cap,
                         size_t* comm_len, uint8_t* comm_para_out, uint8_t* comm_input_out) {
  if (!c || !g || !g->r1cs) return VPIN_EINVAL;
  vpin_spark_decomm* decomm = nullptr;
  vpin::TraceLap lap(c, "vpin_snark_prove_dev");
  int rc = vpin_spark_encode_dev(c, g, &decomm, comm_out, comm_cap, comm_len);
  lap("spark_encode_dev");
  if (!rc)
    rc = vpin_snark_prove_resident(c, g->r1cs, decomm, g->vars_para, g->vars_input, g->vars, g->num_inputs ? g->inputs : nullptr,
                                   seed_commit64, seed_proof64, proof_out, proof_cap, proof_len, comm_para_out, comm_input_out);
  lap("prove_resident");
  vpin_spark_decomm_free(c, decomm);
  return rc;
}

void vpin_spark_last_timings(double out[8]) { memcpy(out, g_spark_timings, sizeof g_spark_timings); }

}
```

vpin_amd/csrc/spark.hip:

```cpp
#include <chrono>
#include <cstdlib>

#include "mailbox_dev.h"
#include "sc_dev.h"
#include "spark_dev.h"

namespace vpin {

__device__ __forceinline__ fq fq_r2() {
  fq r;
  r.v[0] = 0x449c0f01u; r.v[1] = 0xa40611e3u; r.v[2] = 0x68859347u; r.v[3] = 0xd00e1ba7u;
  r.v[4] = 0x17f5be65u; r.v[5] = 0xceec73d2u; r.v[6] = 0x7c309a3du; r.v[7] = 0x0399411bu;
  return r;
}
__device__ __forceinline__ fq fq_raw_u32(uint32_t x) {
  fq r = fq_zero();
  r.v[0] = x;
  return r;
}

__global__ __launch_bounds__(kBlock) void u32_to_fq_kernel(const uint32_t* __restrict__ src, fq* __restrict__ dst, size_t n) {
  const fq r2 = fq_r2();
  for (size_t i = (size_t)blockIdx.x * kBlock + threadIdx.x; i < n; i += (size_t)gridDim.x * kBlock) {
    uint32_t x = src[i];
    fq_store(dst + i, x ? fq_mul(fq_raw_u32(x), r2) : fq_zero());
  }
}

template <bool kStrided>
__device__ __forceinline__ size_t leaf_index(const SparkLeaves& lv, size_t k) {
  if constexpr (kStrided) return lv.r0 + k * lv.step;
  return k;
}

template <bool kStrided>
__global__ __launch_bounds__(kBlock) void gather_derefs_kernel(const uint32_t* __restrict__ idx, size_t N,
                                                               const fq* __restrict__ mem_rx, const fq* __restrict__ mem_ry,
                                                               fq* __restrict__ comb, SparkLeaves lv) {
  const int s = blockIdx.y;
  const size_t n = kStrided ? N / lv.step : N;
  fq* dst = comb + (size_t)s * n;
  if (!kStrided && s >= 6) {
    for (size_t i = (size_t)blockIdx.x * kBlock + threadIdx.x; i < n; i += (size_t)gridDim.x * kBlock) fq_store(dst + i, fq_zero());
    return;
  }
  const uint32_t* a = idx + (size_t)(s < 3 ? s : 3 + s) * N;
  const fq* mem = s < 3 ? mem_rx : mem_ry;
  for (size_t k = (size_t)blockIdx.x * kBlock + threadIdx.x; k < n; k += (size_t)gridDim.x * kBlock)
    fq_store(dst + k, fq_load(mem + a[leaf_index<kStrided>(lv, k)]));
}

__device__ __forceinline__ fq ops_leaf(const HashParams& hp, const fq& val, uint32_t addr, uint32_t ts) {
  fq h = fq_sub(fq_mul(val, hp.r), hp.gamma);
  if (addr) h = fq_add(h, fq_mul(fq_raw_u32(addr), fq_r2()));
  if (ts) h = fq_add(h, fq_mul(fq_raw_u32(ts), hp.r2_boost));
  return h;
}
__device__ __forceinline__ fq ops_leaf_write(const HashParams& hp, const fq& read) { return fq_add(read, hp.r2); }
__device__ __forceinline__ fq mem_leaf_init(const HashParams& hp, const fq& val, size_t addr) {
  fq h = fq_sub(fq_mul(val, hp.r), hp.gamma);
  if (addr) h = fq_add(h, fq_mul(fq_raw_u32((uint32_t)addr), fq_r2()));
  return h;
}
__device__ __forceinline__ fq mem_leaf_audit(const HashParams& hp, fq init, uint32_t ts) {
  if (ts) init = fq_add(init, fq_mul(fq_raw_u32(ts), hp.r2_boost));
  return init;
}

template <bool kStrided>
__global__ __launch_bounds__(kBlock) void hash_ops_kernel(const uint32_t* __restrict__ idx, const fq* __restrict__ derefs, size_t N,
                                                          HashParams hp, fq* __restrict__ forest, SparkLeaves lv) {
  const int side = blockIdx.y / 3, m = blockIdx.y % 3;
  const size_t n = kStrided ? N / lv.step : N;
  const uint32_t* addr = idx + (size_t)(side * 6 + m) * N;
  const uint32_t* ts = idx + (size_t)(side * 6 + 3 + m) * N;
  const fq* val = derefs + (size_t)(side * 3 + m) * n;
  fq* rd = forest + (size_t)(side * 6 + m) * 2 * n;
  fq* wr = forest + (size_t)(side * 6 + 3 + m) * 2 * n;
  for (size_t k = (size_t)blockIdx.x * kBlock + threadIdx.x; k < n; k += (size_t)gridDim.x * kBlock) {
    const size_t i = leaf_index<kStrided>(lv, k);
    const fq h = ops_leaf(hp, fq_load(val + k), addr[i], ts[i]);
    fq_store(rd + k, h);
    fq_store(wr + k, ops_leaf_write(hp, h));
  }
}

template <bool kStrided>
__global__ __launch_bounds__(kBlock) void hash_mem_kernel(const uint32_t* __restrict__ audit_ts, const fq* __restrict__ mem_rx,
                                                          const fq* __restrict__ mem_ry, size_t M, HashParams hp,
                                                          fq* __restrict__ forest, SparkLeaves lv) {
  const int side = blockIdx.y;
  const size_t n = kStrided ? M / lv.step : M;
  const fq* mem = side ? mem_ry : mem_rx;
  const uint32_t* ts = audit_ts + (size_t)side * M;
  fq* init = forest + (size_t)(2 * side) * 2 * n;
  fq* audit = forest + (size_t)(2 * side + 1) * 2 * n;
  for (size_t k = (size_t)blockIdx.x * kBlock + threadIdx.x; k < n; k += (size_t)gridDim.x * kBlock) {
    const size_t i = leaf_index<kStrided>(lv, k);
    const fq h = mem_leaf_init(hp, fq_load(mem + i), i);
    fq_store(init + k, h);
    fq_store(audit + k, mem_leaf_audit(hp, h, ts[i]));
  }
}

__global__ __launch_bounds__(kBlock) void hash_ops_sub_kernel(const uint32_t* __restrict__ idx, const fq* __restrict__ derefs, size_t N,
                                                              HashParams hp, fq* __restrict__ forest, SparkLeaves lv) {
  const int g = lv.ids[blockIdx.y], side = g / 6, kind = (g % 6) / 3, m = g % 3;
  const uint32_t* addr = idx + (size_t)(side * 6 + m) * N;
  const uint32_t* ts = idx + (size_t)(side * 6 + 3 + m) * N;
  const fq* val = derefs + (size_t)(side * 3 + m) * N;
  fq* leaf = forest + (size_t)blockIdx.y * 2 * N;
  for (size_t i = (size_t)blockIdx.x * kBlock + threadIdx.x; i < N; i += (size_t)gridDim.x * kBlock) {
    const fq h = ops_leaf(hp, fq_load(val + i), addr[i], ts[i]);
    fq_store(leaf + i, kind ? ops_leaf_write(hp, h) : h);
  }
}

__global__ __launch_bounds__(kBlock) void hash_mem_sub_kernel(const uint32_t* __restrict__ audit_ts, const fq* __restrict__ mem_rx,
                                                              const fq* __restrict__ mem_ry, size_t M, HashParams hp,
                                                              fq* __restrict__ forest, SparkLeaves lv) {
  const int g = lv.ids[blockIdx.y], side = g / 2, kind = g % 2;
  const fq* mem = side ? mem_ry : mem_rx;
// ... 417 lines not shown
  return VPIN_OK;
}

int spark_comb_tables(vpin_ctx* c, vpin_spark_decomm* d) {
  if (!d) return VPIN_EINVAL;
  std::lock_guard<std::mutex> g(d->comb_mu);
  if (d->comb_ops && d->comb_mem) return VPIN_OK;
  spark_comb_release(c, d, false);
  int rc = spark_comb_make(c, d, &d->comb_ops, &d->comb_mem, !d->comb_unpooled);
  if (!rc && hipStreamSynchronize(c->stream) != hipSuccess) rc = VPIN_EHIP;
  if (rc) spark_comb_release(c, d, false);
  return rc;
}

void spark_comb_release(vpin_ctx* c, vpin_spark_decomm* d, bool to_driver) {
  if (!d) return;
  for (vpin_table** t : {&d->comb_ops, &d->comb_mem}) {
    if (!*t) continue;
    if (to_driver && (*t)->owned && (*t)->owner == c) {
      dev_release_block(c, (*t)->d);
      delete *t;
    } else {
      vpin_table_free(c, *t);
    }
    *t = nullptr;
  }
}

__global__ __launch_bounds__(kBlock) void count_cols_kernel(const uint32_t* __restrict__ idx, size_t N, uint32_t v0, uint32_t v1,
                                                            unsigned long long* __restrict__ cnt) {
  const int m = blockIdx.y;
  const uint32_t* a = idx + (size_t)(6 + m) * N;
  unsigned n0 = 0, n1 = 0;
  for (size_t i = (size_t)blockIdx.x * kBlock + threadIdx.x; i < N; i += (size_t)gridDim.x * kBlock) {
    const uint32_t x = a[i];
    n0 += x == v0;
    n1 += x == v1;
  }
  __shared__ unsigned sh[2][kBlock];
  sh[0][threadIdx.x] = n0;
  sh[1][threadIdx.x] = n1;
  __syncthreads();
  for (int st = kBlock / 2; st >= 1; st >>= 1) {
    if ((int)threadIdx.x < st) { sh[0][threadIdx.x] += sh[0][threadIdx.x + st]; sh[1][threadIdx.x] += sh[1][threadIdx.x + st]; }
    __syncthreads();
  }
  if (threadIdx.x == 0) {
    if (sh[0][0]) atomicAdd(&cnt[2 * m], (unsigned long long)sh[0][0]);
    if (sh[1][0]) atomicAdd(&cnt[2 * m + 1], (unsigned long long)sh[1][0]);
  }
}

int spark_find_hot_cols(vpin_ctx* c, vpin_spark_decomm* d) {
  if (!c || !d || !d->idx || d->N == 0) return VPIN_EINVAL;
  for (int m = 0; m < 3; m++) d->hot_col[m] = 0xffffffffu;
  if (d->N < ((size_t)1 << 20)) return VPIN_OK;
  (void)hipSetDevice(c->device);
  DevBuf cnt(c);
  if (cnt.alloc(6 * sizeof(unsigned long long))) return VPIN_ENOMEM;
  VPIN_HIP_TRY(hipMemsetAsync(cnt.p, 0, 6 * sizeof(unsigned long long), c->stream));
  const uint32_t v0 = (uint32_t)d->num_vars, v1 = (uint32_t)d->num_vars + 1;
  hipLaunchKernelGGL(count_cols_kernel, dim3(grid_for(d->N), 3), dim3(kBlock), 0, c->stream, (const uint32_t*)d->idx, d->N, v0, v1,
                     (unsigned long long*)cnt.p);
  VPIN_HIP_TRY(hipGetLastError());
  unsigned long long h[6];
  VPIN_HIP_TRY(hipMemcpyAsync(h, cnt.p, sizeof h, hipMemcpyDeviceToHost, c->stream));
  VPIN_HIP_TRY(hipStreamSynchronize(c->stream));
  for (int m = 0; m < 3; m++) {
    const int k = h[2 * m + 1] > h[2 * m] ? 1 : 0;
    if (h[2 * m + k] >= d->N / 64) d->hot_col[m] = k ? v1 : v0;
  }
  return VPIN_OK;
}

int spark_gather_derefs(vpin_ctx* c, const vpin_spark_decomm* d, const SparkLeaves& lv, const fq* mem_rx, const fq* mem_ry, fq* comb,
                        fq* comb_rows, size_t R, size_t nrows_loc) {
  const bool strided = lv.step > 1;
  if (!c || !d || !mem_rx || !mem_ry || !comb || lv.ncirc || lv.step == 0 || lv.r0 >= lv.step || d->N % lv.step) return VPIN_EINVAL;
  if (strided && (!comb_rows || R == 0 || d->N % R)) return VPIN_EINVAL;
  (void)hipSetDevice(c->device);
  ProfScope ps(c, VPIN_K_SPARK_BUILD, strided ? (double)d->N * 6 * 68.0 + (double)nrows_loc * R * 68.0 : (double)d->N * (6 * 68.0 + 2 * 32.0));
  const dim3 grid(grid_for(d->N / lv.step), strided ? 6 : 8);
  if (strided)
    hipLaunchKernelGGL(gather_derefs_kernel<true>, grid, dim3(kBlock), 0, c->stream, (const uint32_t*)d->idx, d->N, mem_rx, mem_ry, comb, lv);
  else
    hipLaunchKernelGGL(gather_derefs_kernel<false>, grid, dim3(kBlock), 0, c->stream, (const uint32_t*)d->idx, d->N, mem_rx, mem_ry, comb, lv);
  if (strided && nrows_loc)
    hipLaunchKernelGGL(gather_derefs_rows_kernel, dim3(grid_for(nrows_loc * R)), dim3(kBlock), 0, c->stream, (const uint32_t*)d->idx, d->N,
                       R, mem_rx, mem_ry, comb_rows, lv.r0, lv.step, nrows_loc);
  VPIN_HIP_TRY(hipGetLastError());
  return VPIN_OK;
}

static int build_levels(vpin_ctx* c, SparkForest* f) {
  const size_t n2 = 2 * f->n;
  size_t h = f->n / 2;
  int l = 0;
  while (h > (size_t)kTopBlock) {
    if (h / 4 > (size_t)kTopBlock) {
      hipLaunchKernelGGL(tree_level3_kernel, dim3(grid_for(h / 4), f->ncirc), dim3(kBlock), 0, c->stream, f->base, f->stride(),
                         f->level_off(l), f->level_off(l + 1), f->level_off(l + 2), f->level_off(l + 3), h);
      h >>= 3;
      l += 3;
      continue;
    }
    hipLaunchKernelGGL(tree_level_kernel, dim3(grid_for(h), f->ncirc), dim3(kBlock), 0, c->stream, f->base, f->stride(),
                       f->level_off(l), f->level_off(l + 1), h);
    h >>= 1;
    l++;
  }
  if (h >= 1) hipLaunchKernelGGL(tree_top_kernel, dim3(f->ncirc), dim3(kTopBlock), 0, c->stream, f->base, f->stride(), n2, h);
  VPIN_HIP_TRY(hipGetLastError());
  return VPIN_OK;
}

static int check_forest(const vpin_ctx* c, const vpin_spark_decomm* d, const SparkLeaves& lv, const SparkInputs& in, const SparkForest* f,
                        bool is_mem) {
  const int all = is_mem ? 4 : 12;
  if (!c || !d || !f || !f->base || lv.step == 0 || lv.r0 >= lv.step || (lv.ncirc && lv.step > 1)) return VPIN_EINVAL;
  if (is_mem ? (!in.mem_rx || !in.mem_ry) : !in.derefs) return VPIN_EINVAL;
  if (lv.ncirc < 0 || lv.ncirc > all) return VPIN_EINVAL;
  for (int j = 0; j < lv.ncirc; j++)
    if (lv.ids[j] < 0 || lv.ids[j] >= all) return VPIN_EINVAL;
  if (f->n * lv.step != (is_mem ? d->M : d->N) || f->ncirc != (lv.ncirc ? lv.ncirc : all) || f->n < 2) return VPIN_ESHAPE;
  return VPIN_OK;
}

static double forest_bytes(const SparkLeaves& lv, const SparkForest* f, bool is_mem) {
  if (lv.ncirc) return (double)f->n * f->ncirc * (is_mem ? (36.0 + 32.0 + 64.0) : (8.0 + 32.0 + 32.0 + 64.0));
  return (double)f->n * (is_mem ? (2 * 36.0 + 4 * 32.0 + 4 * 64.0) : (6 * (8.0 + 32.0) + 12 * 32.0 + 12 * 64.0));
}

static void launch_leaves(vpin_ctx* c, const vpin_spark_decomm* d, const HashParams& hp, const SparkLeaves& lv, const SparkInputs& in,
                          SparkForest* f, bool is_mem) {
  const uint32_t* idx = d->idx;
  const uint32_t* audit_ts = d->idx + 12 * d->N;
  const dim3 paired(grid_for(f->n), is_mem ? 2 : 6), each(grid_for(f->n), f->ncirc), block(kBlock);
  if (is_mem) {
    if (lv.ncirc) hipLaunchKernelGGL(hash_mem_sub_kernel, each, block, 0, c->stream, audit_ts, in.mem_rx, in.mem_ry, d->M, hp, f->base, lv);
    else if (lv.step > 1) hipLaunchKernelGGL(hash_mem_kernel<true>, paired, block, 0, c->stream, audit_ts, in.mem_rx, in.mem_ry, d->M, hp, f->base, lv);
    else hipLaunchKernelGGL(hash_mem_kernel<false>, paired, block, 0, c->stream, audit_ts, in.mem_rx, in.mem_ry, d->M, hp, f->base, lv);
  } else {
    if (lv.ncirc) hipLaunchKernelGGL(hash_ops_sub_kernel, each, block, 0, c->stream, idx, in.derefs, d->N, hp, f->base, lv);
    else if (lv.step > 1) hipLaunchKernelGGL(hash_ops_kernel<true>, paired, block, 0, c->stream, idx, in.derefs, d->N, hp, f->base, lv);
    else hipLaunchKernelGGL(hash_ops_kernel<false>, paired, block, 0, c->stream, idx, in.derefs, d->N, hp, f->base, lv);
  }
}

int spark_build_forest(vpin_ctx* c, const vpin_spark_decomm* d, const HashParams& hp, const SparkLeaves& lv, const SparkInputs& in,
                       SparkForest* f, bool is_mem) {
  int rc = check_forest(c, d, lv, in, f, is_mem);
  if (rc) return rc;
  (void)hipSetDevice(c->device);
  ProfScope ps(c, VPIN_K_SPARK_BUILD, forest_bytes(lv, f, is_mem));
  launch_leaves(c, d, hp, lv, in, f, is_mem);
  VPIN_HIP_TRY(hipGetLastError());
  return build_levels(c, f);
}

int spark_build_forests(vpin_ctx* c, const vpin_spark_decomm* d, const HashParams& hp, const SparkLeaves& lv, const SparkInputs& in,
                        SparkForest* ops, SparkForest* mem) {
  int rc = check_forest(c, d, lv, in, ops, false);
  if (!rc) rc = check_forest(c, d, lv, in, mem, true);
  if (rc) return rc;
  (void)hipSetDevice(c->device);
  ProfScope ps(c, VPIN_K_SPARK_BUILD, forest_bytes(lv, ops, false) + forest_bytes(lv, mem, true));
  launch_leaves(c, d, hp, lv, in, ops, false);
  launch_leaves(c, d, hp, lv, in, mem, true);
  VPIN_HIP_TRY(hipGetLastError());
  rc = build_levels(c, ops);
  if (!rc) rc = build_levels(c, mem);
  return rc;
// ... 627 lines not shown
```

vpin_amd/csrc/spark_dev.h:

```cpp
#pragma once
#include <mutex>

#include "ctx.h"

struct vpin_spark_decomm {
  size_t num_cons = 0, num_vars = 0, num_inputs = 0;
  size_t nx = 0, ny = 0, N = 0, M = 0;
  uint32_t* idx = nullptr;
  vpin::fq* vals = nullptr;
  vpin_table* comb_ops = nullptr;
  vpin_table* comb_mem = nullptr;
  std::mutex comb_mu;
  bool comb_unpooled = false;
  uint32_t hot_col[3] = {0xffffffffu, 0xffffffffu, 0xffffffffu};
};

namespace vpin {

constexpr size_t kSparkPinned = 8192;
constexpr int kSparkMaxInst = 18;
constexpr size_t kSparkHostTop = 32;

int spark_pinned(vpin_ctx* c);

int spark_trace_timestamps(vpin_ctx* c, const uint32_t* addr, size_t n, size_t M, uint32_t* ts, uint32_t* audit);
int spark_check_bounds(vpin_ctx* c, const uint32_t* a, size_t nnz, uint32_t limit, uint32_t* d_bad);

int spark_u32_to_fq(vpin_ctx* c, const uint32_t* src, fq* dst, size_t n);
int spark_comb_tables(vpin_ctx* c, vpin_spark_decomm* d);
int spark_comb_make(vpin_ctx* c, const vpin_spark_decomm* d, vpin_table** ops, vpin_table** mem, bool pooled = true);
void spark_comb_release(vpin_ctx* c, vpin_spark_decomm* d, bool to_driver = false);

struct SparkLeaves {
  size_t r0 = 0, step = 1;
  int ncirc = 0;
  int ids[12] = {};
};

int spark_gather_derefs(vpin_ctx* c, const vpin_spark_decomm* d, const SparkLeaves& lv, const fq* mem_rx, const fq* mem_ry, fq* comb,
                        fq* comb_rows = nullptr, size_t R = 0, size_t nrows_loc = 0);
int spark_find_hot_cols(vpin_ctx* c, vpin_spark_decomm* d);

struct SparkForest {
  fq* base = nullptr;
  size_t n = 0;
  int ncirc = 0;
  size_t stride() const { return 2 * n; }
  size_t level_off(int l) const { return 2 * n - ((2 * n) >> l); }
};

struct HashParams { fq r, r2, r2_boost, gamma; };
struct SparkInputs { const fq* derefs; const fq* mem_rx; const fq* mem_ry; };

int spark_build_forest(vpin_ctx* c, const vpin_spark_decomm* d, const HashParams& hp, const SparkLeaves& lv, const SparkInputs& in,
                       SparkForest* f, bool is_mem);
int spark_build_forests(vpin_ctx* c, const vpin_spark_decomm* d, const HashParams& hp, const SparkLeaves& lv, const SparkInputs& in,
                        SparkForest* ops, SparkForest* mem);
int spark_mem_roots(vpin_ctx* c, const vpin_spark_decomm* d, const HashParams& hp, const fq* mem_rx, const fq* mem_ry);

int spark_fetch_tops(vpin_ctx* c, const SparkForest* f, size_t cnt);

int spark_prod_round(vpin_ctx* c, const SparkForest* f, int level, size_t len, const fq* E, const uint8_t* r, int ndotp,
                     bool lead = false);

int spark_dotp_round(vpin_ctx* c, size_t N, const fq* vals, const fq* comb_derefs, fq* scratch, size_t len, bool first_fold,
                     const uint8_t* r, const int* halves = nullptr, int ndotp = 6);

int spark_wait_flag(vpin_ctx* c);

int spark_collect(vpin_ctx* c, const SparkForest* f, int level, const vpin_spark_decomm* d, const fq* comb_derefs,
                  const fq* scratch, bool with_dotp, bool folded);

int spark_triple_sums(vpin_ctx* c, const fq* comb_derefs, const fq* vals, size_t N, const int* halves = nullptr, int nh = 6);

size_t spark_tail_pairs();
int spark_tail_launch(vpin_ctx* c, const SparkForest* f, int level, int k, int j0, size_t len0, const fq* pyr, const uint8_t* r_prev,
                      size_t N, const fq* vals, const fq* comb_derefs, fq* scratch, const int* halves = nullptr, int ndotp = 6);
int spark_tail_wait(vpin_ctx* c, int idx, int ninst, int ncirc);
void spark_tail_reply(vpin_ctx* c, int idx, const uint8_t r[32]);
void spark_tail_end(vpin_ctx* c);
void spark_tail_abort(vpin_ctx* c);
const fq* spark_tail_sums(vpin_ctx* c);
const fq* spark_tail_final(vpin_ctx* c);

int spark_wait(vpin_ctx* c);

int spark_slice_evals(vpin_ctx* c, const fq* table, size_t len, int nslices, const fq* eq, size_t r0 = 0, size_t step = 1);

int spark_take_strided(vpin_ctx* c, const fq* src, size_t nloc, size_t r0, size_t step, fq* dst);

}
```

Before: 80.22 million constraints/s.

## Overlap SPARK derefs gather and commitment with sat sumcheck via side stream

Adds hooks into the satisfiability prover so that once rx is known, the SPARK derefs for the row slices are gathered and their Hyrax commitment launched on a separate side stream. The ry slices follow when ry is known. Device frees issued on the side stream are parked in a deferred-free list until the side stream is joined, and the commitment path skips its host sync. The SPARK prover then reuses these precomputed derefs and commitments instead of recomputing them serially. The cost is extra streams, pinned buffers and deferred memory release, and the side work now competes with the sat sumcheck for CUs.

Result: slower. 79.31 million constraints/s (-1.1%).

```diff
diff --git a/include/vpin_hip.h b/include/vpin_hip.h
--- a/include/vpin_hip.h
+++ b/include/vpin_hip.h
@@ -37,6 +37,8 @@
 int vpin_ctx_set_pool_poison(vpin_ctx* ctx, uint32_t word, int on);
 int vpin_ctx_pool_poison_stats(vpin_ctx* ctx, unsigned long long* blocks, unsigned long long* bytes);
 unsigned long long vpin_ctx_row_table_rows(vpin_ctx* ctx);
+unsigned long long vpin_ctx_early_derefs_rows(vpin_ctx* ctx);
+int vpin_ctx_stream_mask(vpin_ctx* ctx, int which, uint32_t* words, uint32_t cap);
 size_t vpin_msm_row_min_scalars(vpin_ctx* ctx, int part_short);
 unsigned long long vpin_ctx_pip_row_chunks(vpin_ctx* ctx);
 unsigned long long vpin_ctx_witness_redo_ops(vpin_ctx* ctx);
diff --git a/vpin_amd/build.py b/vpin_amd/build.py
--- a/vpin_amd/build.py
+++ b/vpin_amd/build.py
@@ -140,5 +140,17 @@
     return out
 
 
+DEFERRED_FREE_MAIN = os.path.join(os.path.dirname(HERE), "tests", "deferred_free", "deferred_free_main.cpp")
+
+
+def build_deferred_free_program(out, sanitize="address,undefined", verbose=False):
+    cmd = [hipcc(), "--offload-host-only", "-O1", "-std=c++17", "-g", "-fno-omit-frame-pointer", "-pthread", "-Xarch_host",
+           f"-fsanitize={sanitize}", "-fno-sanitize-recover=all", DEFERRED_FREE_MAIN, "-o", out, "-I", CSRC]
+    if verbose:
+        print(" ".join(cmd))
+    subprocess.check_call(cmd)
+    return out
+
+
 if __name__ == "__main__":
     print(build(force="--force" in sys.argv, verbose=True))
diff --git a/vpin_amd/capi.py b/vpin_amd/capi.py
--- a/vpin_amd/capi.py
+++ b/vpin_amd/capi.py
@@ -819,6 +819,22 @@
         L.vpin_ctx_row_table_rows.restype = C.c_ulonglong
         return int(L.vpin_ctx_row_table_rows(self.h))
 
+    def early_derefs_rows(self):
+        L = lib()
+        L.vpin_ctx_early_derefs_rows.argtypes = [C.c_void_p]
+        L.vpin_ctx_early_derefs_rows.restype = C.c_ulonglong
+        return int(L.vpin_ctx_early_derefs_rows(self.h))
+
+    def stream_mask(self, which):
+        L = lib()
+        L.vpin_ctx_stream_mask.argtypes = [C.c_void_p, C.c_int, C.POINTER(C.c_uint32), C.c_uint32]
+        L.vpin_ctx_stream_mask.restype = C.c_int
+        buf = (C.c_uint32 * 32)()
+        n = int(L.vpin_ctx_stream_mask(self.h, int(which), buf, 32))
+        if n < 0 and n != -100:
+            raise VpinError(n, "vpin_ctx_stream_mask")
+        return None if n < 0 else [int(buf[i]) for i in range(min(n, 32))]
+
     def msm_row_min_scalars(self, part_short=False):
         L = lib()
         L.vpin_msm_row_min_scalars.argtypes = [C.c_void_p, C.c_int]
diff --git a/vpin_amd/csrc/capi.hip b/vpin_amd/csrc/capi.hip
--- a/vpin_amd/csrc/capi.hip
+++ b/vpin_amd/csrc/capi.hip
@@ -104,6 +104,7 @@
   const double t_a = pool_trace_min() ? pool_trace_ms() : 0.0;
   if (c->stream_main) (void)hipStreamSynchronize(c->stream_main);
   if (c->stream_alt) (void)hipStreamSynchronize(c->stream_alt);
+  if (c->stream_side) (void)hipStreamSynchronize(c->stream_side);
   if (!c->stream_main) (void)hipStreamSynchronize(c->stream);
   for (void* p : blocks) (void)hipFree(p);
   if (pool_trace_min())
@@ -186,8 +187,13 @@
   return c->pool_poison ? pool_poison_fill(c, out, cls) : VPIN_OK;
 }
 
+static void dev_free_now(vpin_ctx* c, void* p);
 void dev_free(vpin_ctx* c, void* p) {
   if (!p) return;
+  if (c->defer_free) { c->defer_free->park(p); return; }
+  dev_free_now(c, p);
+}
+static void dev_free_now(vpin_ctx* c, void* p) {
   std::lock_guard<std::mutex> g(c->pool_mu);
   auto it = c->pool_sizes.find(p);
   if (it == c->pool_sizes.end()) { (void)hipFree(p); return; }
@@ -233,6 +239,55 @@
 }
 void ctx_enter_alt(vpin_ctx* c) { if (c && c->stream_alt) ctx_switch_stream(c, c->stream_alt, c->cus_alt, true); }
 void ctx_leave_alt(vpin_ctx* c) { if (c && c->stream_alt) ctx_switch_stream(c, c->stream_main, c->cus_main, false); }
+
+int side_stream_get(vpin_ctx* c) {
+  const std::vector<uint32_t>& want = (c->stream_alt && c->stream == c->stream_alt) ? c->mask_alt : c->mask_main;
+  if (c->side_made && c->side_mask == want) return VPIN_OK;
+  (void)hipSetDevice(c->device);
+  if (c->side_made) {
+    VPIN_HIP_TRY(hipStreamSynchronize(c->stream_side));
+    (void)hipStreamDestroy(c->stream_side);
+    c->stream_side = nullptr;
+    c->side_made = false;
+  }
+  if (!c->side_ev) VPIN_HIP_TRY(hipEventCreateWithFlags(&c->side_ev, hipEventDisableTiming));
+  if (want.empty()) VPIN_HIP_TRY(hipStreamCreateWithPriority(&c->stream_side, hipStreamNonBlocking, c->stream_prio));
+  else VPIN_HIP_TRY(hipExtStreamCreateWithCUMask(&c->stream_side, (uint32_t)want.size(), want.data()));
+  c->side_mask = want;
+  c->side_made = true;
+  return VPIN_OK;
+}
+
+void* side_pinned(vpin_ctx* c, size_t bytes) {
+  if (bytes <= c->h_side_cap) return c->h_side;
+  (void)hipSetDevice(c->device);
+  if (c->h_side) { (void)hipHostFree(c->h_side); c->h_side = nullptr; c->h_side_cap = 0; }
+  size_t cap = 4096;
+  while (cap < bytes) cap <<= 1;
+  if (hipHostMalloc(&c->h_side, cap, hipHostMallocDefault) != hipSuccess) { (void)hipGetLastError(); c->h_side = nullptr; return nullptr; }
+  c->h_side_cap = cap;
+  return c->h_side;
+}
+
+SideScope::SideScope(vpin_ctx* ctx, DeferredFree* list) : c(ctx), rc(VPIN_EHIP) {
+  if (c->defer_free || (rc = side_stream_get(c))) { if (rc == VPIN_OK) rc = VPIN_EINVAL; return; }
+  if (hipEventRecord(c->side_ev, c->stream) != hipSuccess || hipStreamWaitEvent(c->stream_side, c->side_ev, 0) != hipSuccess) {
+    set_last_error("side stream: event", hipGetLastError());
+    rc = VPIN_EHIP;
+    return;
+  }
+  back = c->stream;
+  c->stream = c->stream_side;
+  c->defer_free = list;
+}
+SideScope::~SideScope() {
+  if (!back) return;
+  c->stream = back;
+  c->defer_free = nullptr;
+}
+void side_wait(vpin_ctx* c) {
+  if (c && c->side_made) { (void)hipSetDevice(c->device); (void)hipStreamSynchronize(c->stream_side); }
+}
 
 ProfScope::ProfScope(vpin_ctx* c, int kclass, double bytes, int also, double units) : ctx(c) {
   if (!c->prof) return;
@@ -315,8 +370,10 @@
     e = hipExtStreamCreateWithCUMask(&c->stream, n_words, cu_mask);
     c->num_cus = enabled;
     c->cu_masked = true;
+    c->mask_main.assign(cu_mask, cu_mask + n_words);
   } else {
     e = hipStreamCreateWithPriority(&c->stream, hipStreamNonBlocking, prio);
+    c->stream_prio = prio;
   }
   if (e != hipSuccess) { set_last_error("hipStreamCreate", e); delete c; return VPIN_EHIP; }
   c->stream_main = c->stream;
@@ -360,6 +417,9 @@
   if (c->h_out) (void)hipHostFree(c->h_out);
   if (c->h_bullet) (void)hipHostFree(c->h_bullet);
   if (c->stream_alt) { (void)hipStreamSynchronize(c->stream_alt); (void)hipStreamDestroy(c->stream_alt); }
+  if (c->stream_side) { (void)hipStreamSynchronize(c->stream_side); (void)hipStreamDestroy(c->stream_side); }
+  if (c->side_ev) (void)hipEventDestroy(c->side_ev);
+  if (c->h_side) (void)hipHostFree(c->h_side);
   if (c->stream_switch_ev) (void)hipEventDestroy(c->stream_switch_ev);
   if (c->stream_main) (void)hipStreamDestroy(c->stream_main);
   delete c;
@@ -375,6 +435,7 @@
     (void)hipStreamDestroy(c->stream_alt);
     c->stream_alt = nullptr;
     c->cus_alt = 0;
+    c->mask_alt.clear();
   }
   if (!cu_mask || n_words == 0) return VPIN_OK;
   int enabled = 0;
@@ -387,6 +448,7 @@
   if (!c->stream_switch_ev) VPIN_HIP_TRY(hipEventCreateWithFlags(&c->stream_switch_ev, hipEventDisableTiming));
   VPIN_HIP_TRY(hipExtStreamCreateWithCUMask(&c->stream_alt, n_words, cu_mask));
   c->cus_alt = enabled;
+  c->mask_alt.assign(cu_mask, cu_mask + n_words);
   return VPIN_OK;
 }
 
@@ -398,6 +460,15 @@
 
 unsigned long long vpin_ctx_strip_rows_taken(vpin_ctx* c) { return c ? c->strip_rows_taken : 0ull; }
 unsigned long long vpin_ctx_row_table_rows(vpin_ctx* c) { return c ? c->row_table_rows : 0ull; }
+unsigned long long vpin_ctx_early_derefs_rows(vpin_ctx* c) { return c ? c->early_derefs_rows : 0ull; }
+int vpin_ctx_stream_mask(vpin_ctx* c, int which, uint32_t* words, uint32_t cap) {
+  if (!c || which < 0 || which > 2 || (cap && !words)) return VPIN_EINVAL;
+  if (which == 0 && !c->side_made) return -100;
+  if (which == 2 && !c->stream_alt) return -100;
+  const std::vector<uint32_t>& m = which == 0 ? c->side_mask : which == 1 ? c->mask_main : c->mask_alt;
+  for (size_t i = 0; i < m.size() && i < cap; i++) words[i] = m[i];
+  return (int)m.size();
+}
 unsigned long long vpin_ctx_pip_row_chunks(vpin_ctx* c) { return c ? c->pip_row_chunks : 0ull; }
 unsigned long long vpin_ctx_witness_redo_ops(vpin_ctx* c) { return c ? c->witness_redo_ops : 0ull; }
 
diff --git a/vpin_amd/csrc/ctx.h b/vpin_amd/csrc/ctx.h
--- a/vpin_amd/csrc/ctx.h
+++ b/vpin_amd/csrc/ctx.h
@@ -13,6 +13,7 @@
 
 #include "../../include/vpin_hip.h"
 #include "fq_dev.h"
+#include "host/deferred_free.h"
 
 namespace vpin {
 
@@ -57,6 +58,15 @@
   hipStream_t stream_main = nullptr, stream_alt = nullptr;
   hipEvent_t stream_switch_ev = nullptr;
   int cus_main = 256, cus_alt = 0;
+  hipStream_t stream_side = nullptr;
+  hipEvent_t side_ev = nullptr;
+  bool side_made = false;
+  int stream_prio = 0;
+  std::vector<uint32_t> mask_main, mask_alt, side_mask;
+  vpin::DeferredFree* defer_free = nullptr;
+  void* h_side = nullptr;
+  size_t h_side_cap = 0;
+  unsigned long long early_derefs_rows = 0;
   vpin::fq* d_partials = nullptr;
   size_t partials_cap = 0;
   vpin::fq* d_out = nullptr;
@@ -123,6 +133,20 @@
   ~AltStreamGuard() { ctx_leave_alt(c); }
 };
 
+int side_stream_get(vpin_ctx* c);
+void* side_pinned(vpin_ctx* c, size_t bytes);
+struct SideScope {
+  vpin_ctx* c;
+  hipStream_t back = nullptr;
+  int rc;
+  SideScope(vpin_ctx* ctx, DeferredFree* list);
+  ~SideScope();
+  SideScope(const SideScope&) = delete;
+  SideScope& operator=(const SideScope&) = delete;
+  bool ok() const { return rc == VPIN_OK; }
+};
+void side_wait(vpin_ctx* c);
+
 int dev_alloc(vpin_ctx* c, size_t bytes, void** out);
 hipError_t driver_malloc(void** p, size_t bytes);
 void note_driver_alloc(size_t bytes);
@@ -176,9 +200,9 @@
 int gens_msm_parts_dev(vpin_ctx* c, const vpin_gens* g, const fq* d_scalars, size_t rows, size_t ncols, uint8_t* parts_xyzt);
 int hyrax_commit_derefs_hot(vpin_ctx* c, const vpin_gens* g, const vpin_table* Z, size_t L, size_t N, const uint32_t* const col_idx[3],
                             const uint32_t hot[3], const fq* e_ry, uint8_t* out_compressed, size_t row0 = 0, size_t nrows = (size_t)-1,
-                            size_t row_step = 1, const fq* z_rows = nullptr);
+                            size_t row_step = 1, const fq* z_rows = nullptr, bool no_wait = false);
 int hyrax_commit_rows_strided(vpin_ctx* c, const vpin_gens* g, const vpin_table* Z, size_t L, size_t row0, size_t nrows, size_t row_step,
-                              uint8_t* out_compressed, const fq* z_rows = nullptr);
+                              uint8_t* out_compressed, const fq* z_rows = nullptr, bool no_wait = false);
 size_t gens_msm_parts_scratch_bytes(size_t rows, size_t ncols);
 int gens_msm_parts_launch(vpin_ctx* c, const vpin_gens* g, const fq* d_scalars, size_t rows, size_t ncols, void* scratch,
                           uint8_t* parts_xyzt, bool host_mapped = false);
diff --git a/vpin_amd/csrc/host/deferred_free.h b/vpin_amd/csrc/host/deferred_free.h
--- /dev/null
+++ b/vpin_amd/csrc/host/deferred_free.h
@@ -0,0 +1,51 @@
+#pragma once
+#include <cstddef>
+#include <mutex>
+#include <vector>
+
+namespace vpin {
+
+struct DeferredFree {
+  std::vector<void*> blocks;
+  void (*release)(void* owner, void* block) = nullptr;
+  void* owner = nullptr;
+  size_t parked = 0, released = 0;
+  std::mutex mu;
+
+  void park(void* p) {
+    if (!p) return;
+    std::lock_guard<std::mutex> g(mu);
+    blocks.push_back(p);
+    parked++;
+  }
+  void release_all() {
+    std::vector<void*> out;
+    {
+      std::lock_guard<std::mutex> g(mu);
+      out.swap(blocks);
+    }
+    for (void* p : out) {
+      if (release) release(owner, p);
+      released++;
+    }
+  }
+};
+
+struct DeferredJoin {
+  DeferredFree* list;
+  void (*wait)(void* arg);
+  void* arg;
+  bool joined = false;
+  DeferredJoin(DeferredFree* l, void (*w)(void*), void* a) : list(l), wait(w), arg(a) {}
+  DeferredJoin(const DeferredJoin&) = delete;
+  DeferredJoin& operator=(const DeferredJoin&) = delete;
+  void join() {
+    if (joined) return;
+    joined = true;
+    if (wait) wait(arg);
+    if (list) list->release_all();
+  }
+  ~DeferredJoin() { join(); }
+};
+
+}
diff --git a/vpin_amd/csrc/host/prover_common.h b/vpin_amd/csrc/host/prover_common.h
--- a/vpin_amd/csrc/host/prover_common.h
+++ b/vpin_amd/csrc/host/prover_common.h
@@ -480,10 +480,17 @@
 #pragma clang diagnostic pop
 #endif
 
+struct SatHooks {
+  virtual int on_rx(const std::vector<Fq>& rx) = 0;
+  virtual int on_ry(const std::vector<Fq>& ry) = 0;
+  virtual ~SatHooks() {}
+};
+
 int sat_prove_core(vpin_ctx* c, const vpin_r1cs_dev* dinst, size_t nv, size_t ncons, size_t ni,
                    const vpin_table* d_para, const vpin_table* d_input, const vpin_table* d_vars, const uint8_t* inputs,
                    const uint8_t seed_commit64[64], const uint8_t seed_proof64[64], uint8_t* proof_out, size_t proof_cap,
                    size_t* proof_len, uint8_t* comm_para_out, uint8_t* comm_input_out, uint8_t inst_evals_out[96],
-                   uint8_t* rx_out, uint8_t* ry_out, vpin_host::Transcript* tr_out, vpin_host::Transcript* tape_out);
-
-}
+                   uint8_t* rx_out, uint8_t* ry_out, vpin_host::Transcript* tr_out, vpin_host::Transcript* tape_out,
+                   SatHooks* hooks = nullptr);
+
+}
diff --git a/vpin_amd/csrc/msm.hip b/vpin_amd/csrc/msm.hip
--- a/vpin_amd/csrc/msm.hip
+++ b/vpin_amd/csrc/msm.hip
@@ -1281,7 +1281,7 @@
   const size_t min_rows = em ? (size_t)atol(em) : 8192, min_list = em ? (size_t)1 : 4096, min_R = em ? (size_t)64 : 4096;
   st.S = env_strip > 0 ? env_strip : 16;
   st.nrows = nrows;
-  if (!(env_strip != 0 && (env_strip > 0 || (!c->shared_device && c->comm == nullptr)) && nrows >= min_rows && R >= min_R && R <= g->split &&
+  if (!(env_strip != 0 && !c->defer_free && (env_strip > 0 || (!c->shared_device && c->comm == nullptr)) && nrows >= min_rows && R >= min_R && R <= g->split &&
         st.S % 8 == 0 && (size_t)st.S <= R / 8))
     return VPIN_OK;
   if (st.flag.alloc(nrows) || st.list.alloc((nrows + 1) * sizeof(uint32_t))) return VPIN_ENOMEM;
@@ -1389,7 +1389,8 @@
                          RowPolicy{walk_only, part_short, false}, d_points);
 }
 
-static int compress_to_host(vpin_ctx* c, const ge_ext* d_pts, size_t n, uint8_t* out0, uint8_t* out1 = nullptr, uint8_t* out2 = nullptr) {
+static int compress_to_host(vpin_ctx* c, const ge_ext* d_pts, size_t n, uint8_t* out0, uint8_t* out1 = nullptr, uint8_t* out2 = nullptr,
+                            bool no_wait = false) {
   uint8_t* const outs[3] = {out0, out1, out2};
   const size_t k = out2 ? 3 : out1 ? 2 : 1, per = n / k * 32;
   DevBuf dout(c);
@@ -1397,12 +1398,12 @@
   hipLaunchKernelGGL(ge_compress_kernel, dim3((unsigned)((n + 63) / 64)), dim3(64), 0, c->stream, d_pts, n, (fp*)dout.p, (fp*)nullptr);
   VPIN_HIP_TRY(hipGetLastError());
   for (size_t i = 0; i < k; i++) VPIN_HIP_TRY(hipMemcpyAsync(outs[i], (uint8_t*)dout.p + i * per, per, hipMemcpyDeviceToHost, c->stream));
-  VPIN_HIP_TRY(hipStreamSynchronize(c->stream));
+  if (!no_wait) VPIN_HIP_TRY(hipStreamSynchronize(c->stream));
   return VPIN_OK;
 }
 
 static int commit_rows(vpin_ctx* c, const vpin_gens* g, const fq* z, size_t rows, size_t stride, size_t R, const uint8_t* blinds,
-                       size_t blind_base, bool buckets, int c_bits, uint8_t* out_compressed, bool walk_only = false) {
+                       size_t blind_base, bool buckets, int c_bits, uint8_t* out_compressed, bool walk_only = false, bool no_wait = false) {
   (void)hipSetDevice(c->device);
   const int n_extra = blinds ? 1 : 0;
   DevBuf dbl(c), dpts(c);
@@ -1411,7 +1412,7 @@
   const int rc = buckets ? msm_rows_pip(c, g, z, rows, stride, R, (const fq*)dbl.p, n_extra, blind_base, c_bits, (ge_ext*)dpts.p)
                          : msm_rows(c, g, z, rows, stride, R, (const fq*)dbl.p, n_extra, blind_base, (ge_ext*)dpts.p, walk_only);
   if (rc) return rc;
-  return compress_to_host(c, (const ge_ext*)dpts.p, rows, out_compressed);
+  return compress_to_host(c, (const ge_ext*)dpts.p, rows, out_compressed, nullptr, nullptr, no_wait);
 }
 
 int vpin_hyrax_commit(vpin_ctx* c, const vpin_gens* g, const vpin_table* Z, const uint8_t* blinds, size_t L,
@@ -1447,8 +1448,8 @@
 
 int hyrax_commit_derefs_hot(vpin_ctx* c, const vpin_gens* g, const vpin_table* Z, size_t L, size_t N, const uint32_t* const col_idx[3],
                             const uint32_t hot[3], const fq* e_ry, uint8_t* out_compressed, size_t row0, size_t nrows, size_t row_step,
-                            const fq* z_rows) {
-  if (!c || !g || !Z || (!Z->d && !z_rows) || !col_idx || !hot || !e_ry || !out_compressed || L == 0 || Z->len % L) return VPIN_EINVAL;
+                            const fq* z_rows, bool no_wait) {
+  if (!c || !g || !Z || (!Z->d && !z_rows) || !col_idx || !hot || !out_compressed || L == 0 || Z->len % L) return VPIN_EINVAL;
   const size_t R = Z->len / L;
   if (R > g->nb || N % R || Z->len < 6 * N) return VPIN_ESHAPE;
   const fq* zbase = z_rows ? z_rows : (const fq*)Z->d;
@@ -1456,7 +1457,9 @@
   if (nrows == (size_t)-1) { row0 = 0; nrows = L; row_step = 1; }
   if (row_step == 0 || (nrows && row0 + (nrows - 1) * row_step >= L)) return VPIN_ESHAPE;
   if (nrows == 0) return VPIN_OK;
-  if (pip_mode()) return hyrax_commit_rows_strided(c, g, Z, L, row0, nrows, row_step, out_compressed, z_rows);
+  const bool hot_rows = row0 + (nrows - 1) * row_step >= 3 * (N / R) && row0 < 6 * (N / R);
+  if (hot_rows && !e_ry) return VPIN_EINVAL;
+  if (pip_mode()) return hyrax_commit_rows_strided(c, g, Z, L, row0, nrows, row_step, out_compressed, z_rows, no_wait);
   (void)hipSetDevice(c->device);
   DevBuf dpts(c), dT(c);
   if (dpts.alloc(nrows * sizeof(ge_ext))) return VPIN_ENOMEM;
@@ -1468,7 +1471,7 @@
   for (int m = 0; m < 3; m++) {
     hr.idx[m] = col_idx[m];
     hr.hot[m] = hot[m];
-    if (hot[m] == 0xffffffffu) continue;
+    if (hot[m] == 0xffffffffu || !hot_rows) continue;
     bool seen = false;
     for (int k = 0; k < nd; k++) seen = seen || distinct[k] == hot[m];
     if (!seen) distinct[nd++] = hot[m];
@@ -1480,10 +1483,11 @@
     for (int m = 0; m < 3; m++)
       if (hot[m] == distinct[k]) hr.T[m] = Tk;
   }
+  if (!hot_rows) hr.rows_per_vec = 0;
   if (const int rc = msm_rows_launch(c, g, RowArgs{zbase, R, R, nullptr, 0, 0, row0, row_step, z_compact}, nrows, hr,
                                      RowPolicy{false, false, true}, (ge_ext*)dpts.p))
     return rc;
-  return compress_to_host(c, (const ge_ext*)dpts.p, nrows, out_compressed);
+  return compress_to_host(c, (const ge_ext*)dpts.p, nrows, out_compressed, nullptr, nullptr, no_wait);
 }
 
 int hyrax_commit_walk(vpin_ctx* c, const vpin_gens* g, const vpin_table* Z, const uint8_t* blinds, size_t L, size_t blind_base,
@@ -1500,14 +1504,14 @@
 }
 
 int hyrax_commit_rows_strided(vpin_ctx* c, const vpin_gens* g, const vpin_table* Z, size_t L, size_t row0, size_t nrows, size_t row_step,
-                              uint8_t* out_compressed, const fq* z_rows) {
+                              uint8_t* out_compressed, const fq* z_rows, bool no_wait) {
   if (!c || !g || !Z || (!Z->d && !z_rows) || !out_compressed || L == 0 || row_step == 0) return VPIN_EINVAL;
   if (nrows == 0) return VPIN_OK;
   if (Z->len % L != 0 || row0 + (nrows - 1) * row_step >= L) return VPIN_ESHAPE;
   const size_t R = Z->len / L;
   if (R > g->nb) return VPIN_ESHAPE;
-  if (z_rows) return commit_rows(c, g, z_rows, nrows, R, R, nullptr, 0, false, 0, out_compressed);
-  return commit_rows(c, g, Z->d + row0 * R, nrows, row_step * R, R, nullptr, 0, false, 0, out_compressed);
+  if (z_rows) return commit_rows(c, g, z_rows, nrows, R, R, nullptr, 0, false, 0, out_compressed, false, no_wait);
+  return commit_rows(c, g, Z->d + row0 * R, nrows, row_step * R, R, nullptr, 0, false, 0, out_compressed, false, no_wait);
 }
 
 }
diff --git a/vpin_amd/csrc/prover.cpp b/vpin_amd/csrc/prover.cpp
--- a/vpin_amd/csrc/prover.cpp
+++ b/vpin_amd/csrc/prover.cpp
@@ -475,7 +475,7 @@
                    const vpin_table* d_para, const vpin_table* d_input, const vpin_table* d_vars, const uint8_t* inputs,
                    const uint8_t seed_commit64[64], const uint8_t seed_proof64[64], uint8_t* proof_out, size_t proof_cap,
                    size_t* proof_len, uint8_t* comm_para_out, uint8_t* comm_input_out, uint8_t inst_evals_out[96],
-                   uint8_t* rx_out, uint8_t* ry_out, vpin_host::Transcript* tr_out, vpin_host::Transcript* tape_out) {
+                   uint8_t* rx_out, uint8_t* ry_out, vpin_host::Transcript* tr_out, vpin_host::Transcript* tape_out, SatHooks* hooks) {
   auto t_begin = Clock::now();
   memset(g_timings, 0, sizeof g_timings);
   (void)hipSetDevice(c->device);
@@ -573,6 +573,7 @@
   if ((rc = vpin::comm_mark(c, "sat_phase1_rest"))) return rc;
   vpin::ctx_enter_alt(c);
   if (c->progress_flag) *c->progress_flag = 1;
+  if (hooks && (rc = hooks->on_rx(rx))) return rc;
   g_timings[1] = secs(t0, Clock::now());
 
   const Fq tau_claim = claims1[0], Az_claim = claims1[1], Bz_claim = claims1[2], Cz_claim = claims1[3];
@@ -621,6 +622,7 @@
                    nullptr, lw);
   if (rc) return rc;
   if ((rc = vpin::comm_mark(c, "sat_phase2_rest"))) return rc;
+  if (hooks && (rc = hooks->on_ry(ry))) return rc;
   g_timings[2] = secs(t0, Clock::now());
 
   t0 = Clock::now();
diff --git a/vpin_amd/csrc/spark.cpp b/vpin_amd/csrc/spark.cpp
--- a/vpin_amd/csrc/spark.cpp
+++ b/vpin_amd/csrc/spark.cpp
@@ -87,6 +87,100 @@
   if (short_scalars) return vpin::hyrax_commit_walk(c, pc->dev, Z, zeros.data(), pc->L, pc->R + 1, out[0].b);
   return vpin_hyrax_commit(c, pc->dev, Z, zeros.data(), pc->L, pc->R + 1, out[0].b);
 }
+
+static int spark_views(vpin_ctx* c, const vpin_spark_decomm* d, const PcGens** g_ops, const PcGens** g_mem, const PcGens** g_derefs) {
+  const size_t lgN = log2z(d->N);
+  const Shape sh{d->nx, d->ny, d->N, d->M, lgN + 4, std::max(d->nx, d->ny) + 1, lgN + 3};
+  int rc;
+  if ((rc = get_view(c, std::max(sh.v_ops, sh.v_mem), g_ops)) || (rc = get_view(c, sh.v_ops, g_ops)) || (rc = get_view(c, sh.v_mem, g_mem)) ||
+      (rc = get_view(c, sh.v_derefs, g_derefs)))
+    return rc;
+  return VPIN_OK;
+}
+
+static size_t early_derefs_min() {
+  const char* e = getenv("VPIN_EARLY_DEREFS_MIN");
+  if (e) return (size_t)strtoull(e, nullptr, 10);
+  return ~(size_t)0;
+}
+
+struct EarlyDerefs : SatHooks {
+  vpin_ctx* c;
+  const vpin_spark_decomm* d;
+  const PcGens *g_ops = nullptr, *g_mem = nullptr, *g = nullptr;
+  vpin::DeferredFree parked;
+  vpin::DeferredJoin joiner;
+  vpin_table *mem_rx = nullptr, *mem_ry = nullptr, *comb = nullptr;
+  uint8_t* h_out = nullptr;
+  bool on = false, done = false;
+
+  EarlyDerefs(vpin_ctx* c_, const vpin_spark_decomm* d_)
+      : c(c_), d(d_), joiner(&parked, [](void* a) { vpin::side_wait(static_cast<vpin_ctx*>(a)); }, c_) {
+    parked.owner = c_;
+    parked.release = [](void* owner, void* p) { vpin::dev_free(static_cast<vpin_ctx*>(owner), p); };
+  }
+  ~EarlyDerefs() override {
+    if (on) joiner.join();
+    joiner.joined = true;
+    if (mem_rx) vpin_table_free(c, mem_rx);
+    if (mem_ry) vpin_table_free(c, mem_ry);
+    if (comb) vpin_table_free(c, comb);
+  }
+  bool hot() const { return d->hot_col[0] != 0xffffffffu || d->hot_col[1] != 0xffffffffu || d->hot_col[2] != 0xffffffffu; }
+  int commit(size_t row0, size_t nrows, const vpin::fq* e_ry) {
+    const uint32_t* col_idx[3] = {d->idx + 6 * d->N, d->idx + 7 * d->N, d->idx + 8 * d->N};
+    uint8_t* out = h_out + 32 * row0;
+    if (hot()) return vpin::hyrax_commit_derefs_hot(c, g->dev, comb, g->L, d->N, col_idx, d->hot_col, e_ry, out, row0, nrows, 1, nullptr, true);
+    return vpin::hyrax_commit_rows_strided(c, g->dev, comb, g->L, row0, nrows, 1, out, nullptr, true);
+  }
+  int eq_ext(const std::vector<Fq>& r, vpin_table** out) {
+    const size_t nm = std::max(d->nx, d->ny);
+    std::vector<Fq> ext(nm, Fq::zero());
+    std::copy(r.begin(), r.end(), ext.begin() + (nm - r.size()));
+    return vpin_eq_table(c, B(ext.data()), (int)nm, out);
+  }
+
+  int on_rx(const std::vector<Fq>& rx) override {
+    if (c->comm || d->N < 4 || d->M < 4 || rx.size() != d->nx) return VPIN_OK;
+    if (8 * d->N < early_derefs_min()) return VPIN_OK;
+    int rc;
+    if ((rc = spark_views(c, d, &g_ops, &g_mem, &g))) return rc;
+    if (g->L < 8) return VPIN_OK;
+    if (!(h_out = static_cast<uint8_t*>(vpin::side_pinned(c, g->L * 32)))) return VPIN_ENOMEM;
+    vpin::SideScope side(c, &parked);
+    if (!side.ok()) return side.rc;
+    on = true;
+    if ((rc = eq_ext(rx, &mem_rx)) || (rc = vpin::table_alloc_uninit(c, 8 * d->N, &comb)) ||
+        (rc = vpin::spark_gather_derefs_slices(c, d, 0, 3, mem_rx->d, nullptr, comb->d)))
+      return rc;
+    return commit(0, 3 * (g->L / 8), nullptr);
+  }
+  int on_ry(const std::vector<Fq>& ry) override {
+    if (!on) return VPIN_OK;
+    if (ry.size() != d->ny) return VPIN_ESHAPE;
+    int rc;
+    vpin::SideScope side(c, &parked);
+    if (!side.ok()) return side.rc;
+    if ((rc = eq_ext(ry, &mem_ry)) || (rc = vpin::spark_gather_derefs_slices(c, d, 3, 5, nullptr, mem_ry->d, comb->d))) return rc;
+    if ((rc = commit(3 * (g->L / 8), g->L - 3 * (g->L / 8), mem_ry->d))) return rc;
+    c->early_derefs_rows += 6 * (g->L / 8);
+    done = true;
+    return VPIN_OK;
+  }
+  int take(TableGuard& tg, vpin_table** o_rx, vpin_table** o_ry, vpin_table** o_comb, std::vector<CG>& out) {
+    if (!done) return VPIN_EINVAL;
+    (void)hipSetDevice(c->device);
+    const hipError_t e = hipStreamSynchronize(c->stream_side);
+    joiner.join();
+    if (e != hipSuccess) { vpin::set_last_error("early derefs commitment", e); return VPIN_EHIP; }
+    out.resize(g->L);
+    memcpy(out[0].b, h_out, g->L * 32);
+    *o_rx = tg.add(mem_rx); *o_ry = tg.add(mem_ry); *o_comb = tg.add(comb);
+    mem_rx = mem_ry = comb = nullptr;
+    on = false;
+    return VPIN_OK;
+  }
+};
 
 static void append_polycomm(Transcript& tr, const char* label, const std::vector<CG>& C) {
   tr.append_message(label, "poly_commitment_begin");
@@ -650,6 +744,7 @@
   std::vector<Fq> rand_ops, rand_mem;
   Fq ev_derefs[6], ev_ops[15], ev_mem[2];
   DpLog pe_derefs, pe_ops, pe_mem;
+  EarlyDerefs* early = nullptr;
 
   SparkProof(vpin_ctx* c_, const vpin_spark_decomm* d_, const std::vector<Fq>& rx_, const std::vector<Fq>& ry_, const Fq* evals_,
              Transcript& tr_, Transcript& tape_)
@@ -681,6 +776,15 @@
   const size_t N = S.N;
   int rc;
   S.tr.append_protocol_name("Sparse polynomial evaluation proof");
+  if (S.early && S.early->done) {
+    if ((rc = S.early->take(S.tg, &S.mem_rx, &S.mem_ry, &S.comb, S.comm_derefs))) return rc;
+    S.Nf = N; S.Mf = S.M;
+    S.derefs = S.comb->d; S.vals = d->vals;
+    S.tr.append_message("derefs_commitment", "begin_derefs_commitment");
+    append_polycomm(S.tr, "comm_poly_row_col_ops_val", S.comm_derefs);
+    S.tr.append_message("derefs_commitment", "end_derefs_commitment");
+    return VPIN_OK;
+  }
   const size_t nm = std::max(d->nx, d->ny);
   std::vector<Fq> rx_ext(nm, Fq::zero()), ry_ext(nm, Fq::zero());
   std::copy(S.rx.begin(), S.rx.end(), rx_ext.begin() + (nm - d->nx));
@@ -1049,14 +1153,12 @@
 }
 
 static int spark_prove(vpin_ctx* c, const vpin_spark_decomm* d, const std::vector<Fq>& rx, const std::vector<Fq>& ry,
-                       const Fq evals[3], Transcript& tr, Transcript& tape, Writer& w) {
+                       const Fq evals[3], Transcript& tr, Transcript& tape, Writer& w, EarlyDerefs* early = nullptr) {
   if (d->N < 4 || d->M < 4 || rx.size() != d->nx || ry.size() != d->ny) return VPIN_ESHAPE;
   int rc;
   SparkProof S(c, d, rx, ry, evals, tr, tape);
-  const Shape sh{d->nx, d->ny, S.N, S.M, S.lgN + 4, std::max(d->nx, d->ny) + 1, S.lgN + 3};
-  if ((rc = get_view(c, std::max(sh.v_ops, sh.v_mem), &S.g_ops)) || (rc = get_view(c, sh.v_ops, &S.g_ops)) ||
-      (rc = get_view(c, sh.v_mem, &S.g_mem)) || (rc = get_view(c, sh.v_derefs, &S.g_derefs)))
-    return rc;
+  S.early = early;
+  if ((rc = spark_views(c, d, &S.g_ops, &S.g_mem, &S.g_derefs))) return rc;
   auto t0 = Clock::now();
   auto lap = [&](int slot) { g_spark_timings[slot] = secs(t0, Clock::now()); t0 = Clock::now(); };
   if ((rc = split_plan(S)) || (rc = stage_derefs(S))) return rc;
@@ -1334,8 +1436,9 @@
   uint8_t ie[96];
   std::vector<Fq> rx(log2z(ncons)), ry(log2z(2 * nv));
   size_t sat_len = 0;
+  EarlyDerefs early(c, decomm);
   int rc = sat_prove_core(c, dinst, nv, ncons, ni, vars_para, vars_input, vars, inputs, seed_commit64, seed_proof64, proof_out,
-                          proof_cap, &sat_len, comm_para_out, comm_input_out, ie, B(rx.data()), B(ry.data()), &tr, &tape);
+                          proof_cap, &sat_len, comm_para_out, comm_input_out, ie, B(rx.data()), B(ry.data()), &tr, &tape, &early);
   if (rc) return vpin::comm_leave(c->comm, rc);
   if (c->progress_flag) *c->progress_flag = 1;
   g_spark_timings[5] = secs(t0, Clock::now());
@@ -1343,7 +1446,7 @@
   w.bytes(ie, 96);
   Fq evals[3];
   memcpy(evals, ie, 96);
-  if ((rc = spark_prove(c, decomm, rx, ry, evals, tr, tape, w))) return vpin::comm_leave(c->comm, rc);
+  if ((rc = spark_prove(c, decomm, rx, ry, evals, tr, tape, w, &early))) return vpin::comm_leave(c->comm, rc);
   if (sat_len + w.buf.size() > proof_cap) return VPIN_ESHAPE;
   memcpy(proof_out + sat_len, w.buf.data(), w.buf.size());
   *proof_len = sat_len + w.buf.size();
diff --git a/vpin_amd/csrc/spark.hip b/vpin_amd/csrc/spark.hip
--- a/vpin_amd/csrc/spark.hip
+++ b/vpin_amd/csrc/spark.hip
@@ -36,8 +36,8 @@
 template <bool kStrided>
 __global__ __launch_bounds__(kBlock) void gather_derefs_kernel(const uint32_t* __restrict__ idx, size_t N,
                                                                const fq* __restrict__ mem_rx, const fq* __restrict__ mem_ry,
-                                                               fq* __restrict__ comb, SparkLeaves lv) {
-  const int s = blockIdx.y;
+                                                               fq* __restrict__ comb, SparkLeaves lv, int s0) {
+  const int s = s0 + (int)blockIdx.y;
   const size_t n = kStrided ? N / lv.step : N;
   fq* dst = comb + (size_t)s * n;
   if (!kStrided && s >= 6) {
@@ -621,12 +621,23 @@
   ProfScope ps(c, VPIN_K_SPARK_BUILD, strided ? (double)d->N * 6 * 68.0 + (double)nrows_loc * R * 68.0 : (double)d->N * (6 * 68.0 + 2 * 32.0));
   const dim3 grid(grid_for(d->N / lv.step), strided ? 6 : 8);
   if (strided)
-    hipLaunchKernelGGL(gather_derefs_kernel<true>, grid, dim3(kBlock), 0, c->stream, (const uint32_t*)d->idx, d->N, mem_rx, mem_ry, comb, lv);
+    hipLaunchKernelGGL(gather_derefs_kernel<true>, grid, dim3(kBlock), 0, c->stream, (const uint32_t*)d->idx, d->N, mem_rx, mem_ry, comb, lv, 0);
   else
-    hipLaunchKernelGGL(gather_derefs_kernel<false>, grid, dim3(kBlock), 0, c->stream, (const uint32_t*)d->idx, d->N, mem_rx, mem_ry, comb, lv);
+    hipLaunchKernelGGL(gather_derefs_kernel<false>, grid, dim3(kBlock), 0, c->stream, (const uint32_t*)d->idx, d->N, mem_rx, mem_ry, comb, lv, 0);
   if (strided && nrows_loc)
     hipLaunchKernelGGL(gather_derefs_rows_kernel, dim3(grid_for(nrows_loc * R)), dim3(kBlock), 0, c->stream, (const uint32_t*)d->idx, d->N,
                        R, mem_rx, mem_ry, comb_rows, lv.r0, lv.step, nrows_loc);
+  VPIN_HIP_TRY(hipGetLastError());
+  return VPIN_OK;
+}
+
+int spark_gather_derefs_slices(vpin_ctx* c, const vpin_spark_decomm* d, int s0, int ns, const fq* mem_rx, const fq* mem_ry, fq* comb) {
+  if (!c || !d || !comb || s0 < 0 || ns < 1 || s0 + ns > 8 || (s0 < 3 && !mem_rx) || (s0 + ns > 3 && s0 < 6 && !mem_ry)) return VPIN_EINVAL;
+  (void)hipSetDevice(c->device);
+  const int gathered = std::max(0, std::min(s0 + ns, 6) - s0);
+  ProfScope ps(c, VPIN_K_SPARK_BUILD, (double)d->N * (gathered * 68.0 + (ns - gathered) * 32.0));
+  hipLaunchKernelGGL(gather_derefs_kernel<false>, dim3(grid_for(d->N), (unsigned)ns), dim3(kBlock), 0, c->stream, (const uint32_t*)d->idx, d->N,
+                     mem_rx, mem_ry, comb, SparkLeaves{}, s0);
   VPIN_HIP_TRY(hipGetLastError());
   return VPIN_OK;
 }
diff --git a/vpin_amd/csrc/spark_dev.h b/vpin_amd/csrc/spark_dev.h
--- a/vpin_amd/csrc/spark_dev.h
+++ b/vpin_amd/csrc/spark_dev.h
@@ -39,6 +39,7 @@
 
 int spark_gather_derefs(vpin_ctx* c, const vpin_spark_decomm* d, const SparkLeaves& lv, const fq* mem_rx, const fq* mem_ry, fq* comb,
                         fq* comb_rows = nullptr, size_t R = 0, size_t nrows_loc = 0);
+int spark_gather_derefs_slices(vpin_ctx* c, const vpin_spark_decomm* d, int s0, int ns, const fq* mem_rx, const fq* mem_ry, fq* comb);
 int spark_find_hot_cols(vpin_ctx* c, vpin_spark_decomm* d);
 
 struct SparkForest {
```
